# yangjames/Calico

Measured on AMD Instinct MI355X. Metric: LM iterations/sec on the 4-cam+IMU ~100k-observation problem, higher is better.
Workload: dtype f64

## Files before the change

### calico_amd/_capi.py

```python
import ctypes as C
import os

import numpy as np

OK, INVALID_ARGUMENT, FAILED_PRECONDITION, UNIMPLEMENTED, INTERNAL = 0, 3, 9, 12, 13
MANIFOLD_EUCLIDEAN, MANIFOLD_EIGEN_QUATERNION = 0, 1
SENSOR_CAMERA, SENSOR_GYROSCOPE, SENSOR_ACCELEROMETER = 0, 1, 2
CONVERGENCE, NO_CONVERGENCE, FAILURE = 0, 1, 2


class SolverOptions(C.Structure):
    _fields_ = [
        ("max_num_iterations", C.c_int32),
        ("num_threads", C.c_int32),
        ("minimizer_progress_to_stdout", C.c_int32),
        ("jacobi_scaling", C.c_int32),
        ("max_num_consecutive_invalid_steps", C.c_int32),
        ("sync_every", C.c_int32),
        ("function_tolerance", C.c_double),
        ("gradient_tolerance", C.c_double),
        ("parameter_tolerance", C.c_double),
        ("initial_trust_region_radius", C.c_double),
        ("max_trust_region_radius", C.c_double),
        ("min_trust_region_radius", C.c_double),
# ... 247 lines not shown
        ids = _i32(block_ids)
        per = np.broadcast_to(np.asarray(sizes, np.int64), (ids.size,))
        for i, n in zip(ids, per):
            known = self._sizes.get(int(i))
            if known is not None and known != int(n):
                raise ValueError("block %d has %d values, not %d" % (int(i), known, int(n)))
        total = int(per.sum())
        out = np.zeros(total)
        self._check(self.api.get_param_blocks(self.h, ids.size, _ip(ids), _dp(out)))
        return out

    def set_param_block(self, block_id, values):
        v = _f64(values).ravel()
        self._check(self.api.set_param_block(self.h, block_id, _dp(v)))

    def set_param_blocks(self, block_ids, values_concat):
        ids, v = _i32(block_ids), _f64(values_concat)
        self._check(self.api.set_param_blocks(self.h, ids.size, _ip(ids), _dp(v)))

    def set_spline(self, order, knots, basis, ctrl_block_ids):
        k, b, c = _f64(knots), _f64(basis), _i32(ctrl_block_ids)
        assert c.size == k.size - order
        self._check(self.api.problem_set_spline(self.h, order, k.size, _dp(k), _dp(b), _ip(c)))

    def add_rigid_body(self, q_block, t_block):
        out = C.c_int32(-1)
        self._check(self.api.problem_add_rigid_body(self.h, q_block, t_block, C.byref(out)))
        return out.value

    def add_sensor(self, kind, model, intr, q, t, lat, grav=-1, sigma=1.0, loss=0, loss_scale=1.0):
        out = C.c_int32(-1)
        self._check(self.api.problem_add_sensor(self.h, kind, model, intr, q, t, lat, grav, float(sigma), loss,
                                                float(loss_scale), C.byref(out)))
        return out.value

    def add_camera_residuals(self, sensor, pixels, stamps, body_ids, point_blocks):
        px, st, b, p = _f64(pixels), _f64(stamps), _i32(body_ids), _i32(point_blocks)
        self._check(self.api.problem_add_camera_residuals(self.h, sensor, st.size, _dp(px), _dp(st), _ip(b), _ip(p)))

    def add_imu_residuals(self, sensor, meas, stamps):
        m, st = _f64(meas), _f64(stamps)
        self._check(self.api.problem_add_imu_residuals(self.h, sensor, st.size, _dp(m), _dp(st)))

    def solve(self, options=None):
        o = options if options is not None else self.api.default_options()
        s = Summary()
        self._check(self.api.solve(self.h, C.byref(o), C.byref(s)))
        return s

    def iterations(self, max_rows=4096):
        buf = (Iteration * max_rows)()
        n = C.c_int32(0)
        self._check(self.api.get_iterations(self.h, buf, max_rows, C.byref(n)))
        return [buf[i] for i in range(n.value)]

    def residuals(self, sensor, n, dim, check=True):
        out = np.zeros((n, dim))
        valid = np.zeros(n, dtype=np.uint8)
        st = self.api.get_residuals(self.h, sensor, _dp(out), valid.ctypes.data_as(C.POINTER(C.c_uint8)))
        if check:
            self._check(st)
        return out, valid

    def project(self, sensor, n, dim):
        out = np.zeros((n, dim))
        valid = np.zeros(n, dtype=np.uint8)
        self._check(self.api.project(self.h, sensor, _dp(out), valid.ctypes.data_as(C.POINTER(C.c_uint8))))
        return out, valid

    def set_outlier_mask(self, sensor, is_outlier=None):
        if is_outlier is None:
            self._check(self.api.problem_set_outlier_mask(self.h, sensor, None))
        else:
            m = np.ascontiguousarray(is_outlier, dtype=np.uint8)
            self._check(self.api.problem_set_outlier_mask(self.h, sensor, m.ctypes.data_as(C.POINTER(C.c_uint8))))

    def mark_outliers(self, sensor, threshold):
        n = C.c_int64(0)
        self._check(self.api.mark_outliers(self.h, sensor, float(threshold), C.byref(n)))
        return n.value

    def residual_heatmap(self, sensor, image_width, image_height, num_rows=8, num_cols=12):
        rmse = np.zeros((num_rows, num_cols))
        count = np.zeros((num_rows, num_cols), dtype=np.int64)
        self._check(self.api.residual_heatmap(self.h, sensor, int(image_width), int(image_height), int(num_rows), int(num_cols),
                                              _dp(rmse), count.ctypes.data_as(C.POINTER(C.c_int64))))
        return rmse, count

    def inlier_mask(self, sensor, n, threshold):
        mask = np.zeros(n, dtype=np.uint8)
        self._check(self.api.get_inlier_mask(self.h, sensor, float(threshold),
                                             mask.ctypes.data_as(C.POINTER(C.c_uint8))))
        return mask

    def num_effective_parameters(self):
        n = C.c_int32(0)
        self._check(self.api.num_effective_parameters(self.h, C.byref(n)))
        return n.value

    def evaluate(self, want_jtj=True):
        n = self.num_effective_parameters()
        cost = C.c_double(0)
        g = np.zeros(n)
        H = np.zeros((n, n)) if want_jtj else None
        self._check(self.api.evaluate(self.h, C.byref(cost), _dp(g), _dp(H) if want_jtj else None))
        return cost.value, g, H

    def covariance_compute(self, min_relative_pivot=None):
        o = CovarianceOptions()
        self.api.default_covariance_options(C.byref(o))
        if min_relative_pivot is not None:
            o.min_relative_pivot = float(min_relative_pivot)
        self._check(self.api.covariance_compute(self.h, C.byref(o)))
        return self.covariance_info()

    def covariance_info(self):
        dim, nu, piv = C.c_int32(0), C.c_int32(0), C.c_double(0)
        self._check(self.api.covariance_info(self.h, C.byref(dim), C.byref(nu), C.byref(piv)))
        return dim.value, nu.value, piv.value

    def covariance_dense(self):
        dim = self.covariance_info()[0]
        out = np.zeros((dim, dim))
        self._check(self.api.covariance_get_dense(self.h, _dp(out)))
        return out

    def covariance(self, blocks, tangent=False, min_relative_pivot=None):
        self.covariance_compute(min_relative_pivot)
        res = {}
        for i, a in enumerate(blocks):
            for b in blocks[i:]:
                res[(a, b)] = self.covariance_block(a, b, tangent)
        return res

    def covariance_block(self, block_a, block_b, tangent=False, sizes=None):
        if sizes is None:
            def sz(b):
                n = self._sizes[b]
                return 3 if (tangent and n == 4 and self._manifolds.get(b) == MANIFOLD_EIGEN_QUATERNION) else n
            sizes = (sz(block_a), sz(block_b))
        out = np.zeros(sizes)
        self._check(self.api.covariance_get_block(self.h, int(block_a), int(block_b), int(bool(tangent)), _dp(out)))
        return out

    def set_allreduce(self, pyfunc):
        cb = ALLREDUCE_FN(pyfunc)
        self._keep.append(cb)
        self._check(self.api.problem_set_allreduce(self.h, cb, None))

    def finalize(self):
        self._check(self.api.problem_finalize(self.h))

    def plan_info(self):
        out = np.zeros(9, np.int32)
        self._check(self.api.debug_plan_info(self.h, out.ctypes.data_as(C.POINTER(C.c_int32)), 9))
        keys = ("fuse_expand", "frames", "items", "cells", "max_frames_per_cell", "max_items_per_cell", "tree_solver", "m",
                "all_control_points_observed")
        return dict(zip(keys, (int(v) for v in out)))

    def comm_init_rccl(self, unique_id, rank, world_size):
        buf = (C.c_uint8 * 128).from_buffer_copy(bytes(unique_id))
        self._check(self.api.comm_init_rccl(self.h, buf, int(rank), int(world_size)))

    def comm_info(self):
        r, w = C.c_int32(0), C.c_int32(0)
        nl, nt = C.c_int64(0), C.c_int64(0)
        self._check(self.api.comm_info(self.h, C.byref(r), C.byref(w), C.byref(nl), C.byref(nt)))
        return r.value, w.value, nl.value, nt.value

    def set_shard(self, rank, world_size):
        self._check(self.api.problem_set_shard(self.h, int(rank), int(world_size)))

    def set_stream(self, stream_ptr):
        self._check(self.api.problem_set_stream(self.h, C.c_void_p(stream_ptr)))

    def set_phase_timing(self, mask):
        self._check(self.api.set_phase_timing(self.h, int(mask)))

    def phase_time(self, phase):
        ms = C.c_double(0)
        n = C.c_int64(0)
        self._check(self.api.get_phase_time(self.h, phase, C.byref(ms), C.byref(n)))
        return ms.value, n.value


_HIP_LIB_NAME = "libcalico_hip.so"
_hip_api = None


def hip_library_path():
    other = os.environ.get("CALICO_HIP_LIB") if os.environ.get("CALICO_DEV") == "1" else None
    return other or os.path.join(os.path.dirname(os.path.abspath(__file__)), _HIP_LIB_NAME)


def load_hip():
    global _hip_api
    if _hip_api is None:
        path = hip_library_path()
        if not os.path.exists(path):
            raise RuntimeError("%s not found: run `python -c 'import __graft_entry__ as g; g.build()'` "
                               "(the HIP library is the only backend; there is no CPU fallback)" % path)
        _hip_api = CApi(C.CDLL(path), "calico_", has_device=True)
    return _hip_api
```

### calico_amd/csrc/calico_hip.cpp

```cpp
#include <hip/hip_runtime.h>
#include <rccl/rccl.h>
#include <dlfcn.h>
#include <link.h>

#include <algorithm>
#include <chrono>
#include <cmath>
#include <cstdio>
#include <cstdlib>
#include <cstring>
#include <limits>
#include <array>
#include <atomic>
#include <map>
#include <memory>
#include <mutex>
#include <string>
#include <unordered_map>
#include <vector>

#include "../../include/calico_hip.h"
#include "calico_hip_testing.h"
#include "problem_dev.hpp"
#include "shard.hpp"

namespace cal {

void launch_eval(const EvalArgs& a, bool jac, hipStream_t stream);
void launch_eval_frames(const EvalArgs& a, hipStream_t stream);
void launch_eval_jacobian(const EvalArgs& a, hipStream_t stream);
void launch_expand_cells(const EvalArgs& a, hipStream_t stream);
void launch_residual_heatmap(const double* res, const uint8_t* valid, const uint8_t* active, const double* px, const double* py,
                             int begin, int end, int width, int height, int num_rows, int num_cols, double* rmse, long long* count,
                             hipStream_t s);
void launch_inlier_mask(const double* res, uint8_t* valid_then_mask, const uint8_t* active, int begin, int end, int dim, double threshold,
                        hipStream_t s);
void launch_mark_outliers(const double* res, const uint8_t* valid, uint8_t* active, int begin, int end, int dim,
                          double threshold, int* n_marked, hipStream_t s);
hipError_t configure_eval_kernels(size_t max_lds_bytes);

void launch_gather(double* R, const double* src, const int* out_idx_thin, const int64_t* ptr_thin, const int* idx_thin,
                   int n_thin, int n_thin8, int n_thin4, int thin_per_lane, const int* out_idx_fat, const int64_t* ptr_fat, const int* idx_fat, int n_fat,
                   const double* cost_src, int n_cost, const LmState* st, int need_flag, size_t other_stride, hipStream_t s, const ControlTail* tail = nullptr);
void launch_gather_lists(const GatherStruct& gs, int n_out, int* cnt, int* out_idx, int64_t* ptr, int* idx, int zero_slot, long long* scratch,
                         hipStream_t s);
size_t gather_fixed_entries(int n_thin, int n_thin8, int n_thin4, int thin_per_lane);
void launch_gather_pack_fixed(const int64_t* ptr, const int* idx, int n_thin, int n_thin8, int n_thin4, int thin_per_lane, int zero_slot, int* out,
                              hipStream_t s);
void launch_post_eval(const SolveArgs& a, const double* x, const BlockDev* blocks, int n_blocks, const LmOptionsDev& o,
                      IterLog* log, int log_cap, int first, int jacobi, hipStream_t s);
size_t band_cholesky_lds_bytes(const SolveArgs& a);
size_t reduced_solve_lds_bytes(const SolveArgs& a);
size_t frame_lds_doubles(int Ps, int P1e, int n1);
size_t band_backsolve_lds_bytes(const SolveArgs& a);
hipError_t configure_solve_kernels(size_t band_lds, size_t reduced_lds, size_t back_lds);
void launch_solve(const SolveArgs& a, const LmOptionsDev& o, const double* x, double* x_cand, const BlockDev* blocks,
                  int n_blocks, bool dense_in_lds, hipStream_t s, bool with_post_eval, IterLog* log, int log_cap, int jacobi);
void launch_cost_reduce(const double* item_cost, int n_items, double* R2, const LmState* st, hipStream_t s);
void launch_control(LmState* st, const LmOptionsDev& o, double* R2, double* x, const double* x_cand, int n_amb,
                    IterLog* log, int log_cap, const double* item_cost, int n_items, const double* Rbase, size_t r_stride,
                    hipStream_t s, bool commit_by_copy = false);
void launch_init_state(LmState* st, double radius, double x_norm, hipStream_t s, const double* upd_ext = nullptr, int upd_ext_n = 0);
void launch_begin_solve(LmState* st, double radius, double x_norm, const double* upd_ext, int upd_ext_n, const ResultSink& sink, double* x,
                        double* x_cand, const double* h_x, int n_amb, hipStream_t s);
void launch_publish_results(const LmState* st, const IterLog* log, int log_rows, const double* x, int n_amb, LmState* h_state,
                            IterLog* h_log, double* h_x, hipStream_t s);
void launch_seed_x(double* x, const double* h_x, int n_amb, hipStream_t s);
void launch_debug_control_replay(LmState* st, const LmOptionsDev& o, const double* rho, const int* infinite, int n, double* R2,
                                 double* radius_out, int* accepted_out, double* cost_out, IterLog* log, int log_cap, hipStream_t s);
size_t bcr_level_lds_bytes();
size_t bcr_back_lds_bytes(int q_max, int m1p);
hipError_t configure_bcr_kernels(int q_max, int m1p);
void roll_table_row(int k, int lane, unsigned* out);
hipError_t configure_dense_block_solve();
hipError_t configure_reduced_block_step();
size_t dense_block_solve_lds_bytes();
void launch_bcr_level(const SolveArgs& a, const BcrArgs& b, int node0, int n_nodes, int level, int keep0, int n_keep, const LmOptionsDev& o,
                      const double* x, const BlockDev* blocks, int n_blocks, int with_post_eval, IterLog* log, int log_cap, int jacobi,
                      hipStream_t s, int schur_ks, int* fan_word, const BcrInlineNodes& inl);
void launch_bcr_schur(const SolveArgs& a, const BcrArgs& b, int ks, const LmOptionsDev& o, hipStream_t s);
void launch_bcr_back(const SolveArgs& a, const BcrArgs& b, int node0, int n_nodes, bool top, bool extras, bool border_rows, int q_max,
                     const double* x, double* x_cand, const BlockDev* blocks, int n_blocks, const BcrTopSeps& ts, hipStream_t s);

void launch_reduced_solve(const SolveArgs& a, bool reduced_in_lds, int ks, hipStream_t s);
bool dense_back_fusable(const SolveArgs& a, int ks, int q_max, bool border_rows);
size_t dense_back_lds_bytes(int q_max, int m1p);
hipError_t configure_dense_back_bytes(size_t lds);
void launch_dense_back(const SolveArgs& a, const BcrArgs& b, int ks, int node0, int n_nodes, int q_max, const double* x, double* x_cand,
                       const BlockDev* blocks, int n_blocks, const BcrTopSeps& ts, int* word, int seq, hipStream_t s);
int reduced_schur_slices(const SolveArgs& a);
void launch_band_reduction(const SolveArgs& a, const LmOptionsDev& o, const double* x, const BlockDev* blocks, int n_blocks, hipStream_t s,
                           bool with_post_eval, IterLog* log, int log_cap, int jacobi);
int covariance_max_dim();
int covariance_ld(int n);
bool covariance_in_lds(int n);
void launch_covariance(const double* Spart, int ks, int m, int mc, const double* Cdiag, const LmState* st, double* work, double* out,
                       double* info, hipStream_t s);
hipError_t configure_covariance_kernel();

}

using namespace cal;

namespace {

constexpr size_t kMaxLds = 160 * 1024;
constexpr int kLogCap = 4096;
constexpr int kNumPhases = 7;

struct RcclApi {
  void* lib = nullptr;
  ncclResult_t (*GetUniqueId)(ncclUniqueId*) = nullptr;
  ncclResult_t (*CommInitRank)(ncclComm_t*, int, ncclUniqueId, int) = nullptr;
  ncclResult_t (*CommDestroy)(ncclComm_t) = nullptr;
  ncclResult_t (*CommCount)(const ncclComm_t, int*) = nullptr;
  ncclResult_t (*AllReduce)(const void*, void*, size_t, ncclDataType_t, ncclRedOp_t, ncclComm_t, hipStream_t) = nullptr;
  const char* (*GetErrorString)(ncclResult_t) = nullptr;
  std::string error;
  bool ok() const { return lib != nullptr; }
};
RcclApi& rccl() {
  static RcclApi api = [] {
    RcclApi a;
    std::vector<std::string> names;
    if (const char* one = std::getenv("CALICO_RCCL_LIB")) names.push_back(one);
    else {
      names = {"librccl.so.1", "librccl.so"};
      for (const char* env : {"ROCM_PATH", "ROCM_HOME"})
        if (const char* r = std::getenv(env)) { names.push_back(std::string(r) + "/lib/librccl.so.1"); names.push_back(std::string(r) + "/lib/librccl.so"); }
      names.push_back("/opt/rocm/lib/librccl.so.1"); names.push_back("/opt/rocm/lib/librccl.so");
    }
    std::string why;
    for (const std::string& n : names) {
      a.lib = dlopen(n.c_str(), RTLD_NOW | RTLD_NOLOAD);
      if (a.lib) break;
    }
    for (const std::string& n : names) {
      if (a.lib) break;
      a.lib = dlopen(n.c_str(), RTLD_NOW | RTLD_LOCAL);
      if (a.lib) break;
      const char* e = dlerror();
      if (e) why = e;
    }
    if (!a.lib) { a.error = "librccl not found: " + why; return a; }
    auto sym = [&](const char* n) { void* f = dlsym(a.lib, n); if (!f && a.error.empty()) a.error = std::string("librccl lacks ") + n; return f; };
    a.GetUniqueId = reinterpret_cast<decltype(a.GetUniqueId)>(sym("ncclGetUniqueId"));
    a.CommInitRank = reinterpret_cast<decltype(a.CommInitRank)>(sym("ncclCommInitRank"));
    a.CommDestroy = reinterpret_cast<decltype(a.CommDestroy)>(sym("ncclCommDestroy"));
    a.CommCount = reinterpret_cast<decltype(a.CommCount)>(sym("ncclCommCount"));
    a.AllReduce = reinterpret_cast<decltype(a.AllReduce)>(sym("ncclAllReduce"));
    a.GetErrorString = reinterpret_cast<decltype(a.GetErrorString)>(sym("ncclGetErrorString"));
    if (!a.error.empty()) { dlclose(a.lib); a.lib = nullptr; }
    return a;
  }();
  return api;
}

struct HBlock {
  std::vector<double> v;
  int size = 0, manifold = 0;
  bool constant = false, used = false;
  int amb_off = 0;
  int tan = -1;
  int eff = -1;
  int tangent_size() const { return manifold == CALICO_MANIFOLD_EIGEN_QUATERNION ? 3 : size; }
};
struct HBody { int q, t; };
struct HSensor {
  int kind, model, K;
  int intr, q, t, lat, grav;
  double sigma, info;
  int loss; double loss_scale;
  std::vector<double> meas, stamps;
  std::vector<int> body, point, seg;
  std::vector<int64_t> sorted_pos;
  std::vector<uint8_t> active;
  int64_t n_active = -1;
  int64_t sorted_begin = 0, sorted_end = 0;
  int dim() const { return kind == CALICO_SENSOR_CAMERA ? 2 : 3; }
  int64_t n() const { return int64_t(stamps.size()); }
};

class DeviceArena {
 public:
  static DeviceArena& get() { static DeviceArena* a = new DeviceArena; return *a; }
  hipError_t alloc(void** out, size_t bytes) {
    if (!enabled_ || bytes > kSlab) return hipMalloc(out, bytes);
    bytes = (bytes + kAlign - 1) / kAlign * kAlign;
    std::lock_guard<std::mutex> g(mu_);
    int dev = 0; (void)hipGetDevice(&dev);
    for (int pass = 0; pass < 2; ++pass) {
      for (Slab& sl : slabs_) {
        if (sl.device != dev) continue;
        for (auto it = sl.free.begin(); it != sl.free.end(); ++it) {
          if (it->second < bytes) continue;
          const size_t off = it->first, len = it->second;
          sl.free.erase(it);
          if (len > bytes) sl.free.emplace(off + bytes, len - bytes);
          *out = sl.base + off;
// ... 34 lines not shown
      if (next != sl.free.begin()) {
        auto prev = std::prev(next);
        if (prev->first + prev->second == off) { off = prev->first; len += prev->second; sl.free.erase(prev); }
      }
      sl.free.emplace(off, len);
      return;
    }
  }
  struct Batch {
    explicit Batch(int device) : prev_(batch_device()) { if (DeviceArena::get().enabled_) { sync_device(device); batch_device() = device; } }
    ~Batch() { batch_device() = prev_; }
    Batch(const Batch&) = delete;
    Batch& operator=(const Batch&) = delete;
   private:
    int prev_;
  };
  size_t trim(int keep_per_device) {
    std::vector<Slab> drop;
    {
      std::lock_guard<std::mutex> g(mu_);
      std::map<int, int> kept;
      for (size_t i = 0; i < slabs_.size();) {
        Slab& sl = slabs_[i];
        const bool idle = sl.free.size() == 1 && sl.free.begin()->first == 0 && sl.free.begin()->second == sl.size;
        if (idle && kept[sl.device]++ >= keep_per_device) { drop.push_back(std::move(sl)); slabs_.erase(slabs_.begin() + long(i)); }
        else ++i;
      }
    }
    size_t bytes = 0;
    for (Slab& sl : drop) { (void)hipFree(sl.base); bytes += sl.size; }
    return bytes;
  }
  size_t slab_bytes() { std::lock_guard<std::mutex> g(mu_); size_t b = 0; for (const Slab& sl : slabs_) b += sl.size; return b; }
 private:
  static constexpr size_t kAlign = 4096, kSlab = size_t(64) << 20;
  struct Slab { char* base = nullptr; size_t size = 0; int device = 0; std::map<size_t, size_t> free; };
  DeviceArena() { enabled_ = env_flag("CALICO_ARENA", true); }
  static int& batch_device() { static thread_local int d = -1; return d; }
  static void sync_device(int device) {
    int cur = device;
    (void)hipGetDevice(&cur);
    if (cur != device) (void)hipSetDevice(device);
    (void)hipDeviceSynchronize();
    if (cur != device) (void)hipSetDevice(cur);
  }
  std::mutex mu_;
  std::vector<Slab> slabs_;
  std::unordered_map<void*, size_t> used_;
  bool enabled_ = true;
};

template <class T> struct DevBuf {
  T* p = nullptr; size_t n = 0;
  bool owner = true;
  DevBuf() = default;
  DevBuf(const DevBuf&) = delete;
  DevBuf& operator=(const DevBuf&) = delete;
  ~DevBuf() { release(); }
  void release() { if (p && owner) DeviceArena::get().release(p); p = nullptr; n = 0; owner = true; }
  void alias(const DevBuf& o) { release(); p = o.p; n = o.n; owner = false; }
  void take(DevBuf& o) { release(); p = o.p; n = o.n; owner = o.owner; o.p = nullptr; o.n = 0; o.owner = true; }
  void swap(DevBuf& o) { std::swap(p, o.p); std::swap(n, o.n); std::swap(owner, o.owner); }
  hipError_t alloc(size_t count) {
    if (count == 0) count = 1;
    if (count == n && p && owner) return hipSuccess;
    release();
    hipError_t e = DeviceArena::get().alloc(reinterpret_cast<void**>(&p), count * sizeof(T));
    if (e == hipSuccess) n = count;
    return e;
  }
  hipError_t upload(const std::vector<T>& h, hipStream_t s) {
    hipError_t e = alloc(h.size());
    if (e != hipSuccess || h.empty()) return e;
    return hipMemcpyAsync(p, h.data(), h.size() * sizeof(T), hipMemcpyHostToDevice, s);
  }
};

struct PhaseTimer {
  std::vector<hipEvent_t> pool;
  struct Rec { int phase; hipEvent_t a, b; };
  std::vector<Rec> pending;
  size_t next = 0;
  double ms[kNumPhases] = {0, 0, 0, 0, 0, 0};
  int64_t count[kNumPhases] = {0, 0, 0, 0, 0, 0};
  double ms_working[kNumPhases] = {0, 0, 0, 0, 0, 0};
  int64_t count_working[kNumPhases] = {0, 0, 0, 0, 0, 0};
  std::vector<float> samples[kNumPhases];
  hipEvent_t get() {
    if (next == pool.size()) { hipEvent_t e; (void)hipEventCreate(&e); pool.push_back(e); }
    return pool[next++];
  }
  int mask = 0;
  int every = 1;
  int64_t seen[kNumPhases] = {0, 0, 0, 0, 0, 0};
  bool open_rec = false;
  int nested = 0;
  void begin(int phase, hipStream_t s) {
    if (open_rec) { ++nested; return; }
    open_rec = (mask >> phase) & 1;
    if (open_rec && phase != 5 && every > 1) open_rec = (seen[phase]++ % every) == 0;
    if (!open_rec) return;
    Rec r; r.phase = phase; r.a = get(); r.b = nullptr; (void)hipEventRecord(r.a, s); pending.push_back(r);
  }
  void end(hipStream_t s) { if (nested) { --nested; return; } if (!open_rec) return; Rec& r = pending.back(); r.b = get(); (void)hipEventRecord(r.b, s); open_rec = false; }
  void resolve() {
    for (const Rec& r : pending) {
      float t = 0;
      if (r.b && hipEventElapsedTime(&t, r.a, r.b) == hipSuccess) { ms[r.phase] += t; count[r.phase]++; samples[r.phase].push_back(t); }
    }
    pending.clear(); next = 0;
    for (int ph = 0; ph < kNumPhases; ++ph) {
      float mx = 0; for (float t : samples[ph]) mx = std::max(mx, t);
      ms_working[ph] = 0; count_working[ph] = 0;
      for (float t : samples[ph]) if (t >= 0.25f * mx) { ms_working[ph] += t; count_working[ph]++; }
    }
  }
  void reset() { for (int i = 0; i < kNumPhases; ++i) { ms[i] = 0; count[i] = 0; seen[i] = 0; ms_working[i] = 0; count_working[i] = 0; samples[i].clear(); } }
  ~PhaseTimer() { for (hipEvent_t e : pool) (void)hipEventDestroy(e); }
};

}

struct BcrLevel { int node0, n_nodes, keep0, n_keep, q_max; };
struct PlanHost {
  bool speculative = true;
  size_t r_size = 0;
  int sep_s = 0, sep_n = 0;
  bool use_bcr = false, bcr_all_active = false;
  int bcr_N = 0, bcr_m1p = 16, bcr_root = -1, bcr_root_pend = 0, bcr_root_par = 0, bcr_br = 0, bcr_q_max = 1, bcr_slots = 1, bcr_q0 = 1;
  std::vector<BcrLevel> bcr_levels;
  std::vector<BcrNodeDev> h_bcr_nodes;
  std::vector<int> h_bcr_keep, h_cp_block;
  int border_extra() const { return use_bcr ? bcr_br : 6 * sep_n; }
  int n_cp = 0, m = 0, n_amb = 0, n_eff = 0, n_items = 0, n_items_all = 0, lds_cols = 0, row_pad = kRowPad;
  int64_t n_obs = 0;
  size_t partial_doubles = 0, partials_alloc = 0;
  std::vector<int> eff_to_tan;
  std::vector<BlockDev> h_blocks;
  std::vector<ItemDev> h_items, h_items_all, h_jac_items;
  std::vector<FrameItemDev> h_fitems;
  std::vector<CellDev> h_cells;
  int cell_chunk = 1, cell_rec_max = 1, row_cell_chunk = 1;
  int frame_lds_doubles = 0;
  int n_fitems = 0, n_jac_items = 0;
  bool fuse_expand = false;
  int pair_wave_lds_doubles = 0;
  int n_thin = 0, n_fat = 0;
  int n_thin8 = 0, n_thin4 = 0;
  int thin_per_lane = 6;
  bool gather_fixed = false;
  bool dense_in_lds = true;
  int gather_owner_block = 0;
  bool gs_lists_on_device = false;
};
struct PlanDev {
  DevBuf<double> d_knots, d_basis, d_stamp;
  DevBuf<int> d_ctrl_off, d_point_off, d_out_thin, d_idx_thin, d_idx_fixed, d_out_fat, d_idx_fat, d_prim_tab, d_bkeep, d_cp_block, d_gs_tab;
  DevBuf<int64_t> d_ptr_thin, d_ptr_fat;
  DevBuf<uint8_t> d_cp_active;
  DevBuf<SensorDev> d_sensors;
  DevBuf<LayoutDev> d_layouts;
  DevBuf<ItemDev> d_items, d_items_all, d_jac_items;
  DevBuf<FrameItemDev> d_fitems;
  DevBuf<CellDev> d_cells;
  DevBuf<BlockDev> d_blocks;
  DevBuf<BcrNodeDev> d_bnodes;
#define PLAN_DEV_BUFS(X) X(d_knots) X(d_basis) X(d_stamp) X(d_ctrl_off) X(d_point_off) X(d_out_thin) X(d_idx_thin) X(d_idx_fixed) X(d_out_fat) X(d_idx_fat) \
  X(d_prim_tab) X(d_bkeep) X(d_cp_block) X(d_gs_tab) X(d_ptr_thin) X(d_ptr_fat) X(d_cp_active) X(d_sensors) X(d_layouts) X(d_items) X(d_items_all)     \
  X(d_jac_items) X(d_fitems) X(d_cells) X(d_blocks) X(d_bnodes)
  void take_from(PlanDev& o) {
#define X(n) n.take(o.n);
    PLAN_DEV_BUFS(X)
#undef X
  }
  void alias_from(const PlanDev& o) {
#define X(n) n.alias(o.n);
    PLAN_DEV_BUFS(X)
#undef X
  }
};
struct Workspace {
  DevBuf<unsigned long long> d_wave_log;
  DevBuf<double> d_x, d_xc, d_m0, d_m1, d_m2, d_partials, d_R, d_R2, d_Lb, d_Linv, d_Y, d_S, d_Spart, d_Swork, d_zbuf, d_y, d_dadd, d_scale, d_res;
  DevBuf<double> d_bD, d_bG, d_bF, d_bpD, d_bpF, d_bM, d_bZA, d_bZB, d_bY, d_bysol, d_bzb, d_bupd;
  DevBuf<uint8_t> d_valid, d_active;
  DevBuf<int> d_counter;
  DevBuf<int> d_handoff;
  DevBuf<LmState> d_state;
  DevBuf<IterLog> d_log;
  int handoff_seq = 0;
  LmState* h_state = nullptr;
  int* h_progress = nullptr;
  int solve_epoch = 0;
  int* d_progress = nullptr;
  double* h_xpin = nullptr;
  size_t h_xpin_n = 0;
  IterLog* h_log = nullptr;
  bool ws_ready = false;
#define WS_BUFS(X) X(d_wave_log) X(d_x) X(d_xc) X(d_m0) X(d_m1) X(d_m2) X(d_partials) X(d_R) X(d_R2) X(d_Lb) X(d_Linv) X(d_Y) X(d_S) X(d_Spart)      \
  X(d_Swork) X(d_zbuf) X(d_y) X(d_dadd) X(d_scale) X(d_res) X(d_bD) X(d_bG) X(d_bF) X(d_bpD) X(d_bpF) X(d_bM) X(d_bZA) X(d_bZB) X(d_bY) X(d_bysol) \
  X(d_bzb) X(d_bupd) X(d_valid) X(d_active) X(d_counter) X(d_handoff) X(d_state) X(d_log)
  void swap_ws(Workspace& o) {
#define X(n) n.swap(o.n);
    WS_BUFS(X)
#undef X
    std::swap(handoff_seq, o.handoff_seq); std::swap(h_state, o.h_state); std::swap(h_progress, o.h_progress);
    std::swap(solve_epoch, o.solve_epoch); std::swap(d_progress, o.d_progress); std::swap(h_xpin, o.h_xpin);
    std::swap(h_xpin_n, o.h_xpin_n); std::swap(h_log, o.h_log); std::swap(ws_ready, o.ws_ready);
  }
  void free_pinned() {
    if (h_state) (void)hipHostFree(h_state);
    if (h_progress) (void)hipHostFree(h_progress);
    if (h_xpin) (void)hipHostFree(h_xpin);
    if (h_log) (void)hipHostFree(h_log);
    h_state = nullptr; h_progress = nullptr; d_progress = nullptr; h_xpin = nullptr; h_xpin_n = 0; h_log = nullptr;
  }
  Workspace() = default;
  Workspace(const Workspace&) = delete;
  Workspace& operator=(const Workspace&) = delete;
  ~Workspace() { free_pinned(); }
};

struct PlanEntry;

struct calico_problem : PlanHost, PlanDev, Workspace {
  int device = 0;
  hipStream_t stream = nullptr;
  bool own_stream = false;
  std::string error;
  std::vector<HBlock> blocks;
  std::vector<HBody> bodies;
  std::vector<HSensor> sensors;
  int order = 0;
  std::vector<double> knots, valid_knots, basis;
  std::vector<int> ctrl;
  bool dirty = true;
  calico_allreduce_fn allreduce = nullptr;
  void* allreduce_ctx = nullptr;
  ncclComm_t comm = nullptr;
  bool has_exchange() const { return allreduce != nullptr || comm != nullptr; }
  int rank = 0, world = 1;
  std::shared_ptr<PlanEntry> plan;

  std::vector<double> h_x;
  double* h_mpin = nullptr;
  size_t h_mpin_n = 0;
  bool active_dirty = true;
  bool any_tagged = false;
  bool xc_stale = true;
  struct ResCache { bool valid = false, predict = false; std::vector<double> x, r; std::vector<uint8_t> v; } res_cache;
  std::vector<calico_iteration> iterations;
  PhaseTimer timer;
  struct Covariance {
    DevBuf<LmState> st;
    DevBuf<double> scale, dadd, y, zbuf, work, out, info;
    bool valid = false;
    int dim = 0, n_unobserved = 0;
    double min_relative_pivot = 0.0;
    std::vector<double> sigma;
    struct Blk { int off, size, manifold; std::vector<double> v; };
    std::vector<Blk> blocks;
  } cov;

  int set_error(int code, const std::string& msg) { error = msg; return code; }
  int hip_error(hipError_t e, const char* what) {
    return set_error(CALICO_INTERNAL, std::string(what) + ": " + hipGetErrorString(e));
  }
};

#define HIP_TRY(p, expr)                                    \
  do {                                                      \
    hipError_t _e = (expr);                                 \
    if (_e != hipSuccess) return (p)->hip_error(_e, #expr); \
  } while (0)

namespace {

int spline_index(const calico_problem* p, double t) {
  const std::vector<double>& vk = p->valid_knots;
  if (t == vk.back()) return int(vk.size()) - 2;
  if (!(t < vk.back())) return -1;
  const int n = int(vk.size());
  if (t < vk.front()) return -1;
  const double dt = (vk.back() - vk.front()) / double(n - 1);
  int i = dt > 0.0 ? int((t - vk.front()) / dt) : 0;
  i = std::max(0, std::min(n - 2, i));
  while (i > 0 && t < vk[size_t(i)]) --i;
  while (i + 1 < n && !(t < vk[size_t(i) + 1])) ++i;
  return i;
}
int camera_num_params(int model) {
  switch (model) { case 1: return 8; case 2: return 11; case 3: return 7; case 4: return 5; case 5: return 4; case 6: return 4;
    case 7: return 5; default: return -1; }
}
int imu_num_params(int model) { return model == 1 ? 1 : (model == 2 ? 4 : (model == 3 ? 12 : -1)); }

struct PlanSwitches {
  bool band_solver = env_is("CALICO_SOLVER", "band");
  bool speculative = env_flag("CALICO_SPECULATIVE", true);
  bool band_split = env_flag("CALICO_BAND_SPLIT", true);
  bool fuse_expand = env_flag("CALICO_FUSE_EXPAND", true);
  bool gather_struct = env_flag("CALICO_GATHER_STRUCT", true);
  int bcr_leaf = env_int("CALICO_BCR_LEAF", 0, 1, kBcrMaxChain);
};

SolveArgs make_solve_args(calico_problem* p) {
  SolveArgs a;
  a.R = p->d_R.p; a.r_stride = p->speculative ? p->r_size : 0; a.Lb = p->d_Lb.p; a.Linv = p->d_Linv.p; a.Y = p->d_Y.p; a.S = p->d_S.p; a.Spart = p->d_Spart.p;
  a.Swork = p->d_Swork.p; a.y = p->d_y.p; a.zbuf = p->d_zbuf.p; a.dadd = p->d_dadd.p;
  a.scale = p->d_scale.p; a.cp_active = p->d_cp_active.p; a.st = p->d_state.p; a.n_cp = p->n_cp; a.k = p->order; a.mc = p->m; a.sep_s = p->sep_s; a.sep_n = p->sep_n; a.m = p->m + p->border_extra();
  static const int dbg = [] {
    const int v = env_int("CALICO_KERNEL_TIMING", 0, 0);
#ifndef CALICO_DEV_TIMING
    if (v) std::fprintf(stderr, "[calico] CALICO_KERNEL_TIMING is set, but this library was built without the kernels' development "
                                "instrumentation (rebuild with CALICO_DEV_TIMING=1 in the environment of __graft_entry__.build())\n");
#endif
    return v;
  }();
  a.debug = dbg;
  a.progress = nullptr;
  return a;
}

BcrArgs make_bcr_args(calico_problem* p) {
  BcrArgs b;
  b.D = p->d_bD.p; b.G = p->d_bG.p; b.F = p->d_bF.p; b.pendD = p->d_bpD.p; b.pendF = p->d_bpF.p; b.M = p->d_bM.p; b.ZA = p->d_bZA.p;
  b.ZB = p->d_bZB.p; b.Y = p->d_bY.p; b.ysol = p->d_bysol.p; b.zb = p->d_bzb.p; b.upd = p->d_bupd.p; b.nodes = p->d_bnodes.p; b.keep = p->d_bkeep.p;
  b.cp_block = p->d_cp_block.p; b.ctrl_off = p->d_ctrl_off.p; b.all_active = p->bcr_all_active ? 1 : 0; b.pad0 = 0; b.N = p->bcr_N; b.m1p = p->bcr_m1p; b.root = p->bcr_root; b.root_pend = p->bcr_root_pend;
  b.root_par = p->bcr_root_par; b.n_slots = p->bcr_slots;
  return b;
}

void build_bcr_plan(calico_problem* p, const PlanSwitches& sw) {
  const int N = (p->n_cp + kBcrCps - 1) / kBcrCps;
  p->bcr_N = N;
  auto levels_after = [](int n_sep) { int l = 0; while (n_sep > 1) { n_sep /= 2; ++l; } return l; };
  int q = 1;
  {
    double best = 1e300;
    for (int c = 1; c <= kBcrMaxChain; ++c) {
      const int n_sep = N > c ? N / (c + 1) : 0;
      const int L = 1 + levels_after(n_sep);
      double cost = 6.0 * L + 4.0 * (c + L - 1);
      const int per = 1 + p->bcr_m1p / 16, nodes = n_sep + 1;
      if (8 * ((nodes + 7) / 8) * per + 9 > 256) cost += 5.0;
      if (cost < best) { best = cost; q = c; }
    }
    if (sw.bcr_leaf > 0) q = sw.bcr_leaf;
  }
  p->bcr_levels.clear(); p->h_bcr_nodes.clear(); p->h_bcr_keep.clear();
  std::vector<int> alive(static_cast<size_t>(N), 0), mask(static_cast<size_t>(N), 0);
  for (int i = 0; i < N; ++i) alive[size_t(i)] = i;
  int level = 0, q_max_all = 1;
  while (!alive.empty() && (level == 0 || alive.size() > 1)) {
    const int chain = level == 0 ? q : 1;
    BcrLevel L;
    L.node0 = int(p->h_bcr_nodes.size()); L.keep0 = int(p->h_bcr_keep.size() / 2); L.q_max = 1;
    std::vector<int> kept, new_mask(size_t(N), 0);
    const size_t n = alive.size();
    size_t pos = 0;
    while (pos < n) {
      BcrNodeDev nd = {};
      nd.left = kept.empty() ? -1 : kept.back();
      nd.q = 0;
      nd.blk0 = alive[pos]; nd.pend = mask[size_t(alive[pos])];
      while (pos < n && nd.q < chain) { ++nd.q; ++pos; }
      nd.right = pos < n ? alive[pos] : -1;
      nd.slot = int(p->h_bcr_nodes.size());
      L.q_max = std::max(L.q_max, nd.q);
      if (nd.left >= 0) new_mask[size_t(nd.left)] |= 2;
      if (nd.right >= 0) new_mask[size_t(nd.right)] |= 1;
      p->h_bcr_nodes.push_back(nd);
      if (pos < n) { kept.push_back(alive[pos]); ++pos; }
    }
    for (int kb : kept)
      if (level == 0 || mask[size_t(kb)]) { p->h_bcr_keep.push_back(kb); p->h_bcr_keep.push_back(mask[size_t(kb)]); }
    L.n_nodes = int(p->h_bcr_nodes.size()) - L.node0;
    L.n_keep = int(p->h_bcr_keep.size() / 2) - L.keep0;
    q_max_all = std::max(q_max_all, L.q_max);
    p->bcr_levels.push_back(L);
    alive = kept; mask = new_mask;
    ++level;
  }
  p->bcr_root = alive.empty() ? -1 : alive[0];
  p->bcr_root_pend = alive.empty() ? 0 : mask[size_t(alive[0])];
  p->bcr_root_par = (level - 1) & 1;
  p->bcr_br = alive.empty() ? 0 : 6 * kBcrCps;
  p->bcr_q_max = q_max_all;
  p->bcr_q0 = q;
  p->bcr_slots = int(p->h_bcr_nodes.size()) + 1;
}

EvalArgs make_eval_args(calico_problem* p, const double* x, int apply_loss, bool want_res) {
  EvalArgs a;
  static const int dbg = env_int("CALICO_KERNEL_TIMING", 0, 0);
  a.debug = dbg;
  a.x = x; a.sensors = p->d_sensors.p; a.layouts = p->d_layouts.p; a.items = p->d_items.p;
  a.knots = p->d_knots.p; a.basis = p->d_basis.p; a.ctrl_off = p->d_ctrl_off.p;
  a.m0 = p->d_m0.p; a.m1 = p->d_m1.p; a.m2 = p->d_m2.p; a.stamp = p->d_stamp.p; a.point_off = p->d_point_off.p;
  a.partials = p->d_partials.p; a.item_cost = p->d_partials.p + p->partial_doubles;
  a.res_out = want_res ? p->d_res.p : nullptr; a.valid_out = want_res ? p->d_valid.p : nullptr;
  a.order = p->order; a.n_items = p->n_items; a.lds_cols = p->lds_cols; a.row_pad = p->row_pad; a.n_cells = int(p->h_cells.size()); a.cells = p->d_cells.p; a.prim_tab = p->d_prim_tab.p;
  a.cell_chunk = p->cell_chunk; a.cell_rec_max = p->cell_rec_max; a.project = 0; a.row_cell_chunk = p->row_cell_chunk; a.frame_lds_doubles = p->frame_lds_doubles; a.pad5 = 0; a.wave_log = p->d_wave_log.p; a.active = p->any_tagged ? p->d_active.p : nullptr; a.apply_loss = apply_loss;
  a.st = nullptr; a.need_flag = 0; a.cost_index_base = 0;
  a.fitems = p->d_fitems.p; a.n_fitems = p->n_fitems;
  a.hint_progress = nullptr; a.hint_seq = 0; a.hint_ftol = a.hint_ptol = 0.0;
  a.pair_mode = 0; a.wave_lds_doubles = 0;
  return a;
}

constexpr int kImuChunkItems = 21;

struct SetupTimer {
  std::chrono::steady_clock::time_point t = std::chrono::steady_clock::now();
  void section(const char* name) {
    static const bool on = env_flag("CALICO_SETUP_TIMING", false);
    if (!on) return;
    const auto now = std::chrono::steady_clock::now();
    std::fprintf(stderr, "[calico] finalize %-28s %8.3f ms\n", name, std::chrono::duration<double, std::milli>(now - t).count());
    t = now;
  }
};

int build_plan(calico_problem* p, const PlanSwitches& sw, SetupTimer& setup) {
  const int k = p->order;
  const int n_cp = int(p->ctrl.size());
  p->n_cp = n_cp;
  int off = 0;
  for (HBlock& b : p->blocks) { b.amb_off = off; off += b.size; b.used = false; b.tan = -1; b.eff = -1; }
  p->n_amb = off;
  std::vector<char> is_ctrl(p->blocks.size(), 0);
  for (int id : p->ctrl) is_ctrl[id] = 1;
  std::vector<uint8_t> cp_active(n_cp, 0);
  for (HSensor& s : p->sensors) {
    if (s.n() == 0) continue;
    p->blocks[s.intr].used = p->blocks[s.q].used = p->blocks[s.t].used = p->blocks[s.lat].used = true;
    if (s.kind == CALICO_SENSOR_ACCELEROMETER) p->blocks[s.grav].used = true;
    for (int64_t i = 0; i < s.n(); ++i) {
      for (int j = 0; j < k; ++j) cp_active[s.seg[i] + j] = 1;
      if (s.kind == CALICO_SENSOR_CAMERA) {
        p->blocks[s.point[i]].used = true;
        p->blocks[p->bodies[s.body[i]].q].used = p->blocks[p->bodies[s.body[i]].t].used = true;
      }
    }
  }
  for (int i = 0; i < n_cp; ++i) {
    HBlock& b = p->blocks[p->ctrl[i]];
    b.used = cp_active[i] != 0;
    if (b.constant && b.used) return p->set_error(CALICO_UNIMPLEMENTED, "constant control points are not supported");
    b.tan = 6 * i;
  }
  p->h_blocks.clear(); p->eff_to_tan.clear();
  int eff = 0;
  for (int i = 0; i < n_cp; ++i) {
    if (!cp_active[i]) continue;
// ... 258 lines not shown
        p->h_cells.push_back(c);
        it.rows_off = -2;
        it.partial_off = int64_t(poff);
        poff += size_t(tri_size(n1));
      } else if (hs.kind != CALICO_SENSOR_CAMERA && n1 <= 112) {
        it.partial_off = 0; it.rows_off = 0;
        if (p->h_cells.empty() || p->h_cells.back().prim_off >= 0 || p->h_cells.back().layout != it.layout ||
            p->h_cells.back().seg != it.seg) {
          CellDev c;
          c.layout = it.layout; c.seg = it.seg; c.frame_begin = int(p->h_jac_items.size()); c.frame_count = 0;
          c.partial_off = int64_t(poff); c.src_off = 0; c.n1 = n1; c.PE = hs.dim() * kImuChunkItems; c.prim_off = -1; c.pad0 = 0;
          poff += size_t(tri_size(n1));
          p->h_cells.push_back(c);
        }
        p->h_cells.back().frame_count += 1;
        p->h_cells.back().pad0 += hs.dim() * it.obs_count;
      } else {
        it.rows_off = -1;
        it.partial_off = int64_t(poff);
        poff += size_t(tri_size(n1));
      }
      p->h_jac_items.push_back(it);
    }
  }
  p->n_fitems = int(p->h_fitems.size());
  p->n_jac_items = int(p->h_jac_items.size());
  const size_t n_cost_slots = 2 * size_t(std::max(std::max(int(p->h_items.size()), int(p->h_items_all.size())), p->n_fitems + p->n_jac_items));
  const size_t comp_base = poff + n_cost_slots;
  p->cell_rec_max = 1;
  p->frame_lds_doubles = 0;
  for (FrameItemDev& f : p->h_fitems) {
    {
      const LayoutDev& L = layouts[size_t(f.layout)];
      const HSensor& hs = p->sensors[size_t(L.sensor)];
      const int P1 = 7 + (L.c_intr >= 0 ? hs.K : 0) + 3 * (L.c_q >= 0) + 3 * (L.c_t >= 0) + 3 * (L.c_bq >= 0) + 3 * (L.c_bt >= 0);
      const int Ps = 7 + (L.c_intr >= 0 ? hs.K : 0) + 3 * (L.c_bq >= 0);
      p->frame_lds_doubles = std::max(p->frame_lds_doubles, int(frame_lds_doubles(Ps, P1, L.ncols + 1)));
    }
    f.partial_off += int64_t(comp_base);
    p->cell_rec_max = std::max(p->cell_rec_max, int(frame_rec(layouts[size_t(f.layout)])));
  }
  p->cell_chunk = std::max(1, int((56 * 1024 / sizeof(double)) / size_t(p->cell_rec_max)));
  {
    int most = 1;
    for (const CellDev& c : p->h_cells) if (c.prim_off >= 0) most = std::max(most, c.frame_count);
    p->cell_chunk = std::min(p->cell_chunk, most);
  }
  std::vector<int> prim_tab;
  {
    std::vector<int> tab_off(layouts.size(), -1);
    for (CellDev& c : p->h_cells) {
      if (c.prim_off < 0) continue;
      const LayoutDev& L = layouts[size_t(c.layout)];
      const HSensor& hs = p->sensors[size_t(L.sensor)];
      int pc = 6;
      const int p_intr = pc; if (L.c_intr >= 0) pc += hs.K;
      const int p_q = pc; if (L.c_q >= 0) pc += 3;
      const int p_t = pc; if (L.c_t >= 0) pc += 3;
      const int p_bq = pc; if (L.c_bq >= 0) pc += 3;
      const int p_bt = pc; if (L.c_bt >= 0) pc += 3;
      const int p_r = pc, PT = pc + 1;
      if (tab_off[size_t(c.layout)] < 0) {
        tab_off[size_t(c.layout)] = int(prim_tab.size());
        std::vector<int> prim;
        for (int lc = 0; lc <= L.ncols; ++lc) {
          int pr;
          if (lc < 36) pr = lc % 6;
          else if (lc == L.c_lat) pr = PT;
          else if (lc == L.ncols) pr = p_r;
          else if (L.c_intr >= 0 && lc >= L.c_intr && lc < L.c_intr + hs.K) pr = p_intr + (lc - L.c_intr);
          else if (L.c_q >= 0 && lc >= L.c_q && lc < L.c_q + 3) pr = p_q + (lc - L.c_q);
          else if (L.c_t >= 0 && lc >= L.c_t && lc < L.c_t + 3) pr = p_t + (lc - L.c_t);
          else if (L.c_bq >= 0 && lc >= L.c_bq && lc < L.c_bq + 3) pr = p_bq + (lc - L.c_bq);
          else pr = p_bt + (lc - L.c_bt);
          prim.push_back(pr);
        }
        const int n1 = L.ncols + 1, PEc = PT + 1;
        for (int i = 0; i < n1; ++i)
          for (int j = i; j < n1; ++j) prim_tab.push_back(i | (j << 8) | ((prim[size_t(i)] * PEc + prim[size_t(j)]) << 16));
      }
      c.prim_off = tab_off[size_t(c.layout)]; c.pad0 = 0;
      c.n1 = L.ncols + 1; c.PE = PT + 1;
      c.src_off = c.frame_begin >= 0 ? p->h_fitems[size_t(c.frame_begin)].partial_off : 0;
    }
    for (FrameItemDev& fi : p->h_fitems) {
      const CellDev& c = p->h_cells[size_t(fi.cell)];
      fi.cell_frames = c.frame_count; fi.cell_prim_off = c.prim_off; fi.cell_partial_off = c.partial_off; fi.cell_src_off = c.src_off;
    }
  }
  for (HSensor& s : p->sensors) { s.sorted_begin = n_obs; s.sorted_end = 0; }
  for (int64_t q = 0; q < n_obs; ++q) {
    HSensor& s = p->sensors[keys[q].sensor];
    const int64_t i = keys[q].idx;
    s.sorted_pos[size_t(i)] = q;
    s.sorted_begin = std::min(s.sorted_begin, q); s.sorted_end = std::max(s.sorted_end, q + 1);
    st[q] = s.stamps[i];
    if (s.kind == CALICO_SENSOR_CAMERA) point_off[q] = p->blocks[s.point[i]].amb_off;
  }
  p->n_items = int(p->h_items.size());
  p->n_items_all = int(p->h_items_all.size());
  p->partial_doubles = poff;
  if (poff + 2 * size_t(std::max(p->n_items, p->n_fitems + p->n_jac_items)) >= size_t(0x7fffffff))
    return p->set_error(CALICO_UNIMPLEMENTED, "problem too large for 32-bit gather indices");
  {
    int jc = 4, jr = 2;
    for (const ItemDev& it : p->h_jac_items) {
      const LayoutDev& L = layouts[size_t(it.layout)];
      jc = std::max(jc, L.ncols + 1);
      jr = std::max(jr, p->sensors[size_t(L.sensor)].dim() * it.obs_count);
    }
    (void)max_cols;
    p->lds_cols = (jc + 15) & ~15;
    p->row_pad = (((jr + 3) & ~3) + 1) | 1;
  }
  if (size_t(p->lds_cols) * p->row_pad * sizeof(double) > kMaxLds)
    return p->set_error(CALICO_UNIMPLEMENTED, "too many Jacobian columns per residual block for the LDS staging area");
  size_t row_store = 0;
  {
    const size_t stride = (size_t(p->lds_cols) * p->row_pad + 1) & ~size_t(1);
    row_store = (comp_base + comp_off) & 1;
    for (size_t i = 0; i < p->h_jac_items.size(); ++i) {
      ItemDev& it = p->h_jac_items[i];
      if (it.rows_off < 0) continue;
      it.rows_off = int64_t(comp_base + comp_off + row_store);
      row_store += stride;
    }
    for (CellDev& c : p->h_cells)
      if (c.prim_off == -1) c.src_off = p->h_jac_items[size_t(c.frame_begin)].rows_off;
    p->row_cell_chunk = std::max(1, int((56 * 1024 / sizeof(double)) / std::max<size_t>(1, stride)));
    int most = 1;
    for (const CellDev& c : p->h_cells) if (c.prim_off == -1) most = std::max(most, c.frame_count);
    p->row_cell_chunk = std::min(p->row_cell_chunk, most);
  }
  setup.section("sort + work items");
  SolveArgs sa; sa.n_cp = n_cp; sa.k = k; sa.mc = m; sa.sep_s = p->sep_s; sa.sep_n = p->sep_n; sa.m = m + p->border_extra(); sa.debug = 0; sa.progress = nullptr;
  const size_t r_size = sa.r_size();
  if (r_size >= size_t(0x7fffffff)) return p->set_error(CALICO_UNIMPLEMENTED, "normal-equation buffer too large");
  struct Pair { int dst, src; };
  std::vector<Pair> pairs;
  const int n_cells = int(p->h_cells.size());
  const int n_part = n_cells + p->n_jac_items;
  bool gs_ok = sw.gather_struct && int(layouts.size()) * k <= 96 && int(layouts.size()) >= 1 && m >= 1 && n_cells > 0;
  for (int itn = n_cells; gs_ok && itn < n_part; ++itn) {
    const int64_t ro = p->h_jac_items[size_t(itn - n_cells)].rows_off;
    gs_ok = ro >= 0 || ro == -2;
  }
  const int64_t gs_n_out = int64_t(NS) * m + int64_t(n_cp) * k * 36 + NS;
  gs_ok = gs_ok && gs_n_out * 96 < int64_t(0x7fffffff);
  p->gs_lists_on_device = gs_ok;
  std::vector<int> gs_tab;
  GatherStruct gsd = {};
  if (gs_ok) {
    const int n_lay = int(layouts.size()), nsg = int(p->valid_knots.size()) - 1;
    gs_tab.assign(size_t(n_lay) * nsg + size_t(n_lay) * m + size_t(n_lay), -1);
    for (const CellDev& c : p->h_cells) gs_tab[size_t(c.layout) * nsg + size_t(c.seg)] = int(c.partial_off);
    for (int l = 0; l < n_lay; ++l) {
      const std::vector<int>& gmap = layout_gmap[size_t(l)];
      for (size_t q = 0; q < gmap.size(); ++q) gs_tab[size_t(n_lay) * nsg + size_t(l) * m + size_t(gmap[q] - NS)] = 6 * k + int(q);
      gs_tab[size_t(n_lay) * nsg + size_t(n_lay) * m + size_t(l)] = layouts[size_t(l)].ncols + 1;
    }
    gsd.n_lay = n_lay; gsd.nseg = nsg; gsd.n_cp = n_cp; gsd.k = k; gsd.m = m;
    {
      int d4 = k;
      while (d4 > 0 && (k - (d4 - 1)) * n_lay <= 24) --d4;
      gsd.d_split = d4;
    }
    gsd.off_g = sa.off_g(); gsd.off_B = sa.off_B(); gsd.off_E = sa.off_E();
  }
  pairs.reserve(gs_ok ? size_t(n_part) * 256 : poff / 2 + 4 * size_t(p->n_items));
  for (int itn = 0; itn < n_part; ++itn) {
    const bool is_cell = itn < n_cells;
    if (!is_cell && (p->h_jac_items[size_t(itn - n_cells)].rows_off >= 0 || p->h_jac_items[size_t(itn - n_cells)].rows_off == -2)) continue;
    const int it_layout = is_cell ? p->h_cells[size_t(itn)].layout : p->h_jac_items[size_t(itn - n_cells)].layout;
    const int it_seg = is_cell ? p->h_cells[size_t(itn)].seg : p->h_jac_items[size_t(itn - n_cells)].seg;
    const int64_t it_poff = is_cell ? p->h_cells[size_t(itn)].partial_off : p->h_jac_items[size_t(itn - n_cells)].partial_off;
    const LayoutDev& L = layouts[size_t(it_layout)];
    const std::vector<int>& gmap = layout_gmap[size_t(it_layout)];
    const int nc = L.ncols, n1 = nc + 1;
    auto tan_of = [&](int c) { return c < 6 * k ? 6 * (it_seg + c / 6) + c % 6 : gmap[size_t(c - 6 * k)]; };
    for (int i = gs_ok ? 6 * k : 0; i < nc; ++i) {
      const int ti = tan_of(i);
      pairs.push_back({int(sa.off_g()) + ti, int(it_poff) + tri_off(i, nc, n1)});
      for (int j = i; j < nc; ++j) {
        const int tj = tan_of(j);
        const int src = int(it_poff) + tri_off(i, j, n1);
        if (ti < NS && tj < NS) {
          const int a = ti / 6, b = tj / 6;
          pairs.push_back({int(sa.off_B()) + (a * k + (b - a)) * 36 + (ti % 6) * 6 + (tj % 6), src});
          if (a == b && ti != tj) pairs.push_back({int(sa.off_B()) + (a * k) * 36 + (tj % 6) * 6 + (ti % 6), src});
        } else if (ti < NS) {
          pairs.push_back({int(sa.off_E() + size_t(ti) * m + (tj - NS)), src});
        } else {
          const int a = ti - NS, b = tj - NS;
          pairs.push_back({int(sa.off_C() + size_t(a) * m + b), src});
          if (a != b) pairs.push_back({int(sa.off_C() + size_t(b) * m + a), src});
        }
      }
    }
  }
  std::vector<int> out_thin, idx_thin, out_fat, idx_fat;
  std::vector<int64_t> ptr_thin(1, 0), ptr_fat(1, 0);
  {
    std::vector<int64_t> start(r_size + 1, 0);
    for (const Pair& pr : pairs) ++start[size_t(pr.dst) + 1];
    for (size_t d = 0; d < r_size; ++d) start[d + 1] += start[d];
    std::vector<int> sorted_src(pairs.size());
    {
      std::vector<int64_t> fill(start.begin(), start.end() - 1);
      for (const Pair& pr : pairs) sorted_src[size_t(fill[size_t(pr.dst)]++)] = pr.src;
    }
    int thin_cap = 48;
    if (gs_ok) thin_cap = int(layouts.size()) * k <= 48 ? 48 : 96;
    else {
      size_t n_mid = 0;
      for (size_t d = 0; d < r_size; ++d) { const int64_t c = start[d + 1] - start[d]; if (c > 48 && c <= 96) ++n_mid; }
      if (n_mid > 0) thin_cap = 96;
    }
    p->thin_per_lane = thin_cap / 8;
    size_t n_thin_src = 0, n_fat_src = 0;
    for (size_t d = 0; d < r_size; ++d) {
      const int64_t c = start[d + 1] - start[d];
      if (gs_ok || c > thin_cap) n_fat_src += size_t(c); else n_thin_src += size_t(c);
    }
    idx_thin.reserve(n_thin_src); idx_fat.reserve(n_fat_src);
    for (size_t d = 0; d < r_size; ++d) {
      const int64_t q0 = start[d], q1 = start[d + 1];
      if (q1 == q0) continue;
      const bool fat = gs_ok || (q1 - q0) > thin_cap;
      std::vector<int>& out = fat ? out_fat : out_thin;
      std::vector<int>& idx = fat ? idx_fat : idx_thin;
      std::vector<int64_t>& ptr = fat ? ptr_fat : ptr_thin;
      out.push_back(int(d));
      idx.insert(idx.end(), sorted_src.begin() + q0, sorted_src.begin() + q1);
      ptr.push_back(int64_t(idx.size()));
    }
  }
  p->n_thin = int(out_thin.size()); p->n_fat = int(out_fat.size());
  p->n_thin8 = p->n_thin; p->n_thin4 = p->n_thin;
  p->gather_owner_block = 0;
  setup.section("gather lists");
  hipStream_t s = p->stream;
  std::vector<int> ctrl_off(n_cp);
  for (int i = 0; i < n_cp; ++i) ctrl_off[i] = p->blocks[p->ctrl[i]].amb_off;
  {
    auto fill = [&](auto& it) {
      it.L = layouts[size_t(it.layout)];
      it.S = sd[size_t(it.L.sensor)];
      for (int i = 0; i < 8; ++i) it.ctrl_off[i] = (i < k && it.seg + i < n_cp) ? ctrl_off[size_t(it.seg + i)] : 0;
    };
    for (ItemDev& it : p->h_items) fill(it);
    for (ItemDev& it : p->h_items_all) fill(it);
    for (ItemDev& it : p->h_jac_items) fill(it);
    for (FrameItemDev& it : p->h_fitems) fill(it);
  }
  HIP_TRY(p, p->d_knots.upload(p->knots, s)); HIP_TRY(p, p->d_basis.upload(p->basis, s));
  HIP_TRY(p, p->d_ctrl_off.upload(ctrl_off, s));
  HIP_TRY(p, p->d_stamp.upload(st, s)); HIP_TRY(p, p->d_point_off.upload(point_off, s));
  HIP_TRY(p, p->d_sensors.upload(sd, s)); HIP_TRY(p, p->d_layouts.upload(layouts, s));
  HIP_TRY(p, p->d_items.upload(p->h_items, s)); HIP_TRY(p, p->d_items_all.upload(p->h_items_all, s));
  HIP_TRY(p, p->d_jac_items.upload(p->h_jac_items, s)); HIP_TRY(p, p->d_fitems.upload(p->h_fitems, s));
  HIP_TRY(p, p->d_blocks.upload(p->h_blocks, s));
  HIP_TRY(p, p->d_cp_active.upload(cp_active, s));
  DevBuf<int> d_cnt;
  DevBuf<long long> d_scan;
  if (comp_base + comp_off + row_store + 2 >= size_t(0x7fffffff)) return p->set_error(CALICO_UNIMPLEMENTED, "problem too large for 32-bit gather indices");
  const int zero_slot = int(comp_base + comp_off + row_store);
  if (gs_ok) {
    HIP_TRY(p, p->d_gs_tab.upload(gs_tab, s));
    gsd.tab = p->d_gs_tab.p;
    const int per_out = int(layouts.size()) * k;
    HIP_TRY(p, p->d_out_thin.alloc(size_t(gs_n_out))); HIP_TRY(p, p->d_ptr_thin.alloc(size_t(gs_n_out) + 1));
    HIP_TRY(p, p->d_idx_thin.alloc(size_t(gs_n_out) * per_out)); HIP_TRY(p, d_cnt.alloc(size_t(gs_n_out)));
    HIP_TRY(p, d_scan.alloc(size_t(gs_n_out) / 1024 + 2));
    launch_gather_lists(gsd, int(gs_n_out), d_cnt.p, p->d_out_thin.p, p->d_ptr_thin.p, p->d_idx_thin.p, zero_slot, d_scan.p, s);
    p->n_thin = int(gs_n_out);
    bool one_layout = k <= 8;
    for (int tc = 0; one_layout && tc < m; ++tc) {
      int holders = 0;
      for (int l = 0; l < gsd.n_lay; ++l) holders += gs_tab[size_t(gsd.n_lay) * gsd.nseg + size_t(l) * m + size_t(tc)] >= 0 ? 1 : 0;
      one_layout = holders <= 1;
    }
    const int n_border0 = NS + n_cp * k * 36;
    p->n_thin4 = one_layout ? n_border0 : p->n_thin;
    const int d4 = gsd.d_split;
    p->n_thin8 = one_layout ? std::min(n_border0, NS + d4 * n_cp * 36) : p->n_thin;
  } else {
    HIP_TRY(p, p->d_out_thin.upload(out_thin, s)); HIP_TRY(p, p->d_idx_thin.upload(idx_thin, s));
    HIP_TRY(p, p->d_ptr_thin.upload(ptr_thin, s));
  }
  HIP_TRY(p, p->d_out_fat.upload(out_fat, s)); HIP_TRY(p, p->d_idx_fat.upload(idx_fat, s));
  HIP_TRY(p, p->d_ptr_fat.upload(ptr_fat, s));
  p->gather_fixed = p->n_thin > 0 && gs_ok;
  if (p->gather_fixed) {
    HIP_TRY(p, p->d_idx_fixed.alloc(gather_fixed_entries(p->n_thin, p->n_thin8, p->n_thin4, p->thin_per_lane) + 8));
    launch_gather_pack_fixed(p->d_ptr_thin.p, p->d_idx_thin.p, p->n_thin, p->n_thin8, p->n_thin4, p->thin_per_lane, zero_slot, p->d_idx_fixed.p, s);
  }
  HIP_TRY(p, p->d_cells.upload(p->h_cells, s)); HIP_TRY(p, p->d_prim_tab.upload(prim_tab, s));
  p->partials_alloc = comp_base + comp_off + row_store + 2;
  p->r_size = r_size;
  p->speculative = sw.speculative;
  {
    sa = make_solve_args(p);
    if (band_cholesky_lds_bytes(sa) > kMaxLds) return p->set_error(CALICO_UNIMPLEMENTED, "spline order too high for the banded factorisation window");
    p->dense_in_lds = reduced_solve_lds_bytes(sa) <= kMaxLds - 1024;
    if (band_backsolve_lds_bytes(sa) > kMaxLds) return p->set_error(CALICO_UNIMPLEMENTED, "trajectory too long for the back-substitution window");
  }
  if (p->use_bcr) {
    HIP_TRY(p, p->d_bnodes.upload(p->h_bcr_nodes, s)); HIP_TRY(p, p->d_bkeep.upload(p->h_bcr_keep, s));
    p->h_cp_block.assign(size_t(n_cp), -1);
    for (size_t bi = 0; bi < p->h_blocks.size(); ++bi)
      if (p->h_blocks[bi].tan_off < NS) p->h_cp_block[size_t(p->h_blocks[bi].tan_off / 6)] = int(bi);
    HIP_TRY(p, p->d_cp_block.upload(p->h_cp_block, s));
    if (bcr_level_lds_bytes() > kMaxLds || bcr_back_lds_bytes(p->bcr_q_max, p->bcr_m1p) > kMaxLds)
      return p->set_error(CALICO_UNIMPLEMENTED, "tree solver workspace exceeds the LDS");
  }
  HIP_TRY(p, hipStreamSynchronize(s));
  setup.section("structure uploads");
  return CALICO_OK;
}

struct PlanKey {
  uint64_t h1 = 0, h2 = 0; size_t n_blocks = 0, n_obs = 0; int device = 0;
  bool operator==(const PlanKey& o) const { return h1 == o.h1 && h2 == o.h2 && n_blocks == o.n_blocks && n_obs == o.n_obs && device == o.device; }
};
}
struct PlanEntry {
  PlanKey key;
  PlanHost host;
  PlanDev dev;
  struct BlockMeta { int amb_off, tan, eff; bool used; };
  std::vector<BlockMeta> block_meta;
  struct SensorMeta { std::vector<int64_t> sorted_pos; int64_t sorted_begin, sorted_end; };
  std::vector<SensorMeta> sensor_meta;
  std::vector<std::unique_ptr<Workspace>> pool;
  uint64_t last_use = 0;
};
namespace {
struct PlanCache {
  std::mutex mu;
  std::vector<std::shared_ptr<PlanEntry>> entries;
  uint64_t tick = 0;
  int64_t hits = 0, misses = 0;
  static constexpr size_t kMaxEntries = 8, kMaxPool = 2;
};
PlanCache& plan_cache() { static PlanCache* c = new PlanCache; return *c; }
bool plan_cache_enabled() {
  static const bool on = env_flag("CALICO_PLAN_CACHE", true);
  return on;
}
struct Hasher {
  uint64_t a = 0x9E3779B97F4A7C15ull, b = 0xC2B2AE3D27D4EB4Full;
  void word(uint64_t w) {
    a = (a ^ w) * 0xff51afd7ed558ccdull; a ^= a >> 32;
    b = (b + w) * 0xc4ceb9fe1a85ec53ull; b ^= b >> 29;
  }
  void bytes(const void* p, size_t n) {
    const unsigned char* c = static_cast<const unsigned char*>(p);
    size_t i = 0;
    if (n >= 256) {
      uint64_t l0 = 0x243F6A8885A308D3ull, l1 = 0x13198A2E03707344ull, l2 = 0xA4093822299F31D0ull, l3 = 0x082EFA98EC4E6C89ull;
      for (; i + 32 <= n; i += 32) {
        uint64_t w[4];
        std::memcpy(w, c + i, 32);
        l0 = (l0 ^ w[0]) * 0xff51afd7ed558ccdull; l0 ^= l0 >> 32;
        l1 = (l1 ^ w[1]) * 0xc4ceb9fe1a85ec53ull; l1 ^= l1 >> 29;
        l2 = (l2 ^ w[2]) * 0x9E3779B97F4A7C15ull; l2 ^= l2 >> 31;
        l3 = (l3 ^ w[3]) * 0xD6E8FEB86659FD93ull; l3 ^= l3 >> 30;
      }
      word(l0); word(l1); word(l2); word(l3);
    }
    for (; i + 8 <= n; i += 8) { uint64_t w; std::memcpy(&w, c + i, 8); word(w); }
    if (i < n) { uint64_t w = 0; std::memcpy(&w, c + i, n - i); word(w ^ (uint64_t(n - i) << 56)); }
  }
  template <class T> void vec(const std::vector<T>& v) { word(v.size()); bytes(v.data(), v.size() * sizeof(T)); }
  void dbl(double d) { uint64_t w; std::memcpy(&w, &d, 8); word(w); }
};
PlanKey structure_key(const calico_problem* p, const PlanSwitches& sw) {
  Hasher h;
  h.word(uint64_t(p->order)); h.vec(p->knots); h.vec(p->basis); h.vec(p->ctrl);
  h.word(uint64_t(p->rank)); h.word(uint64_t(p->world));
  h.word(p->blocks.size());
  for (const HBlock& b : p->blocks) h.word(uint64_t(b.size) | (uint64_t(b.manifold) << 32) | (uint64_t(b.constant) << 40));
  h.word(p->bodies.size());
  for (const HBody& b : p->bodies) h.word(uint64_t(uint32_t(b.q)) | (uint64_t(uint32_t(b.t)) << 32));
  h.word(p->sensors.size());
  size_t n_obs = 0;
  for (const HSensor& s : p->sensors) {
    h.word(uint64_t(s.kind) | (uint64_t(s.model) << 8) | (uint64_t(s.K) << 16) | (uint64_t(s.loss) << 32));
    h.word(uint64_t(uint32_t(s.intr)) | (uint64_t(uint32_t(s.q)) << 32)); h.word(uint64_t(uint32_t(s.t)) | (uint64_t(uint32_t(s.lat)) << 32));
    h.word(uint64_t(uint32_t(s.grav)));
    h.dbl(s.sigma); h.dbl(s.info); h.dbl(s.loss_scale);
    h.vec(s.stamps); h.vec(s.body); h.vec(s.point);
    n_obs += s.stamps.size();
  }
  h.word(uint64_t(sw.band_solver) | (uint64_t(sw.speculative) << 1) | (uint64_t(sw.band_split) << 2) | (uint64_t(sw.fuse_expand) << 3) |
         (uint64_t(sw.gather_struct) << 4) | (uint64_t(sw.bcr_leaf) << 8));
  PlanKey k; k.h1 = h.a; k.h2 = h.b; k.n_blocks = p->blocks.size(); k.n_obs = n_obs; k.device = p->device;
  return k;
}

void adopt_plan(calico_problem* p, const std::shared_ptr<PlanEntry>& e) {
  static_cast<PlanHost&>(*p) = e->host;
  static_cast<PlanDev&>(*p).alias_from(e->dev);
  for (size_t i = 0; i < p->blocks.size(); ++i) {
    const PlanEntry::BlockMeta& bm = e->block_meta[i];
    p->blocks[i].amb_off = bm.amb_off; p->blocks[i].tan = bm.tan; p->blocks[i].eff = bm.eff; p->blocks[i].used = bm.used;
  }
  for (size_t i = 0; i < p->sensors.size(); ++i) {
    p->sensors[i].sorted_pos = e->sensor_meta[i].sorted_pos;
    p->sensors[i].sorted_begin = e->sensor_meta[i].sorted_begin; p->sensors[i].sorted_end = e->sensor_meta[i].sorted_end;
  }
  p->plan = e;
}

int prepare_workspace(calico_problem* p) {
  hipStream_t s = p->stream;
  if (p->plan) {
    std::unique_ptr<Workspace> w;
    {
      std::lock_guard<std::mutex> lock(plan_cache().mu);
      if (!p->plan->pool.empty()) { w = std::move(p->plan->pool.back()); p->plan->pool.pop_back(); }
    }
    if (w) { static_cast<Workspace&>(*p).swap_ws(*w); p->active_dirty = true; p->xc_stale = true; return CALICO_OK; }
  }
  const int n_cp = p->n_cp, m = p->m, k = p->order, NS = 6 * n_cp;
  const int64_t n_obs = p->n_obs;
  const size_t r_size = p->r_size;
  HIP_TRY(p, p->d_x.alloc(size_t(p->n_amb))); HIP_TRY(p, p->d_xc.alloc(size_t(p->n_amb)));
  HIP_TRY(p, p->d_m0.alloc(size_t(n_obs))); HIP_TRY(p, p->d_m1.alloc(size_t(n_obs))); HIP_TRY(p, p->d_m2.alloc(size_t(n_obs)));
  HIP_TRY(p, p->d_partials.alloc(p->partials_alloc));
  HIP_TRY(p, hipMemsetAsync(p->d_partials.p + (p->partials_alloc - 2), 0, 2 * sizeof(double), s));
  if (env_int("CALICO_KERNEL_TIMING", 0, 0) >= 3) HIP_TRY(p, p->d_wave_log.alloc(2 * size_t(p->n_jac_items + p->n_fitems) + 8));
  HIP_TRY(p, p->d_R.alloc(2 * r_size)); HIP_TRY(p, hipMemsetAsync(p->d_R.p, 0, 2 * r_size * sizeof(double), s));
  HIP_TRY(p, p->d_R2.alloc(2));
  const int NT = 6 * n_cp + m;
  const int mw = m + p->border_extra();
  HIP_TRY(p, p->d_Lb.alloc(size_t(NS) * 6 * k)); HIP_TRY(p, p->d_Linv.alloc(size_t(n_cp) * 36));
  HIP_TRY(p, p->d_Y.alloc(size_t(NS) * (mw + 1)));
  HIP_TRY(p, p->d_S.alloc(size_t(mw + 1) * (mw + 1)));
  HIP_TRY(p, p->d_y.alloc(size_t(NT) + p->border_extra() + 64)); HIP_TRY(p, p->d_zbuf.alloc(size_t(NS) + 64)); HIP_TRY(p, p->d_dadd.alloc(NT)); HIP_TRY(p, p->d_scale.alloc(2 * size_t(NT)));
  HIP_TRY(p, p->d_res.alloc(size_t(n_obs) * 3)); HIP_TRY(p, p->d_valid.alloc(size_t(n_obs)));
  HIP_TRY(p, p->d_active.alloc(size_t(n_obs))); HIP_TRY(p, p->d_counter.alloc(1));
  p->active_dirty = true; p->xc_stale = true;
  HIP_TRY(p, p->d_state.alloc(1)); HIP_TRY(p, p->d_log.alloc(kLogCap));
  if (!p->h_state) {
    HIP_TRY(p, hipHostMalloc(reinterpret_cast<void**>(&p->h_state), sizeof(LmState), hipHostMallocMapped | hipHostMallocCoherent));
    std::memset(p->h_state, 0, sizeof(LmState));
  }
  if (!p->h_log) HIP_TRY(p, hipHostMalloc(reinterpret_cast<void**>(&p->h_log), size_t(kLogCap) * sizeof(IterLog), hipHostMallocMapped | hipHostMallocCoherent));
  if (p->h_xpin_n < size_t(p->n_amb)) {
    if (p->h_xpin) (void)hipHostFree(p->h_xpin);
    p->h_xpin = nullptr; p->h_xpin_n = 0;
    HIP_TRY(p, hipHostMalloc(reinterpret_cast<void**>(&p->h_xpin), std::max<size_t>(1, size_t(p->n_amb)) * sizeof(double), hipHostMallocMapped | hipHostMallocCoherent));
    p->h_xpin_n = size_t(p->n_amb);
  }
  if (!p->h_progress) {
    HIP_TRY(p, hipHostMalloc(reinterpret_cast<void**>(&p->h_progress), 64, hipHostMallocMapped | hipHostMallocCoherent));
    HIP_TRY(p, hipHostGetDevicePointer(reinterpret_cast<void**>(&p->d_progress), p->h_progress, 0));
    std::memset(p->h_progress, 0, 64);
  }
  const SolveArgs sa = make_solve_args(p);
  const size_t reduced_lds = reduced_solve_lds_bytes(sa);
  HIP_TRY(p, p->d_Spart.alloc(size_t(mw + 1 <= 128 ? 8 : 4) * size_t(mw + 1) * (mw + 1) + 64));
  HIP_TRY(p, p->d_Swork.alloc(std::max<size_t>(reduced_lds / sizeof(double) + 8, size_t(mw + 1) * 16 * 13 + 8)));
  if (p->use_bcr) {
    const size_t N = size_t(p->bcr_N), bb = size_t(kBcrBP) * kBcrBP, fb = size_t(kBcrBP) * p->bcr_m1p;
    HIP_TRY(p, p->d_bD.alloc(N * bb)); HIP_TRY(p, p->d_bG.alloc(2 * N * bb)); HIP_TRY(p, p->d_bF.alloc(N * fb));
    HIP_TRY(p, p->d_bpD.alloc(4 * N * bb)); HIP_TRY(p, p->d_bpF.alloc(4 * N * fb));
    HIP_TRY(p, p->d_bM.alloc(N * bb)); HIP_TRY(p, p->d_bZA.alloc(N * bb)); HIP_TRY(p, p->d_bZB.alloc(N * bb));
    HIP_TRY(p, p->d_bY.alloc(N * fb)); HIP_TRY(p, p->d_bysol.alloc(N * kBcrBP)); HIP_TRY(p, p->d_bzb.alloc(N * kBcrBP)); HIP_TRY(p, p->d_bupd.alloc(size_t(p->bcr_slots) * 4));
    HIP_TRY(p, hipMemsetAsync(p->d_bY.p, 0, N * fb * sizeof(double), s));
    HIP_TRY(p, hipMemsetAsync(p->d_bG.p, 0, 2 * N * bb * sizeof(double), s));
    HIP_TRY(p, hipMemsetAsync(p->d_bpD.p, 0, 4 * N * bb * sizeof(double), s)); HIP_TRY(p, hipMemsetAsync(p->d_bpF.p, 0, 4 * N * fb * sizeof(double), s));
    HIP_TRY(p, hipMemsetAsync(p->d_bupd.p, 0, size_t(p->bcr_slots) * 4 * sizeof(double), s));
    HIP_TRY(p, p->d_handoff.alloc(8)); HIP_TRY(p, hipMemsetAsync(p->d_handoff.p, 0, 8 * sizeof(int), s));
    p->handoff_seq = 0;
  }
  p->ws_ready = true;
  return CALICO_OK;
}

struct PinnedPool {
  std::mutex mu;
  std::vector<std::pair<double*, size_t>> idle;
  double* acquire(size_t n, size_t* cap) {
    {
      std::lock_guard<std::mutex> lock(mu);
      for (size_t i = 0; i < idle.size(); ++i)
        if (idle[i].second >= n) { double* q = idle[i].first; *cap = idle[i].second; idle.erase(idle.begin() + long(i)); return q; }
    }
    double* q = nullptr;
    const size_t c = n + n / 4;
    if (hipHostMalloc(reinterpret_cast<void**>(&q), c * sizeof(double), hipHostMallocDefault) != hipSuccess) return nullptr;
    *cap = c;
    return q;
  }
  void release(double* q, size_t cap) {
    if (!q) return;
    std::lock_guard<std::mutex> lock(mu);
    if (idle.size() < 2) { idle.emplace_back(q, cap); return; }
    size_t small = 0;
    for (size_t i = 1; i < idle.size(); ++i) if (idle[i].second < idle[small].second) small = i;
    if (idle[small].second < cap) { (void)hipHostFree(idle[small].first); idle[small] = {q, cap}; }
    else (void)hipHostFree(q);
  }
};
PinnedPool& pinned_pool() { static PinnedPool* pp = new PinnedPool(); return *pp; }

int upload_values(calico_problem* p) {
  hipStream_t s = p->stream;
  const size_t n = size_t(std::max<int64_t>(p->n_obs, 1));
  if (p->h_mpin && p->h_mpin_n < 3 * n) { pinned_pool().release(p->h_mpin, p->h_mpin_n); p->h_mpin = nullptr; p->h_mpin_n = 0; }
  if (!p->h_mpin) {
    p->h_mpin = pinned_pool().acquire(3 * n, &p->h_mpin_n);
    if (!p->h_mpin) return p->set_error(CALICO_INTERNAL, "hipHostMalloc (measurement staging) failed");
  }
  double* m0 = p->h_mpin; double* m1 = m0 + n; double* m2 = m1 + n;
  for (const HSensor& sn : p->sensors) {
    const int dim = sn.dim();
    const int64_t ns = sn.n();
    const double* me = sn.meas.data();
    const int64_t* sp = sn.sorted_pos.data();
    if (dim == 2) for (int64_t i = 0; i < ns; ++i) { const size_t q = size_t(sp[i]); m0[q] = me[2 * i]; m1[q] = me[2 * i + 1]; m2[q] = 0.0; }
    else for (int64_t i = 0; i < ns; ++i) { const size_t q = size_t(sp[i]); m0[q] = me[3 * i]; m1[q] = me[3 * i + 1]; m2[q] = me[3 * i + 2]; }
  }
  if (p->n_obs > 0) {
    HIP_TRY(p, hipMemcpyAsync(p->d_m0.p, m0, size_t(p->n_obs) * sizeof(double), hipMemcpyHostToDevice, s));
    HIP_TRY(p, hipMemcpyAsync(p->d_m1.p, m1, size_t(p->n_obs) * sizeof(double), hipMemcpyHostToDevice, s));
    HIP_TRY(p, hipMemcpyAsync(p->d_m2.p, m2, size_t(p->n_obs) * sizeof(double), hipMemcpyHostToDevice, s));
  }
  p->h_x.assign(size_t(p->n_amb), 0.0);
  for (const HBlock& b : p->blocks) std::copy(b.v.begin(), b.v.end(), p->h_x.begin() + b.amb_off);
  if (p->n_amb > 0) {
    HIP_TRY(p, hipMemcpyAsync(p->d_x.p, p->h_x.data(), p->h_x.size() * sizeof(double), hipMemcpyHostToDevice, s));
    HIP_TRY(p, hipMemcpyAsync(p->d_xc.p, p->h_x.data(), p->h_x.size() * sizeof(double), hipMemcpyHostToDevice, s));
  }
  return CALICO_OK;
}

int configure_kernels(calico_problem* p) {
  const SolveArgs sa = make_solve_args(p);
  const size_t reduced_lds = reduced_solve_lds_bytes(sa);
  const bool db_fits = p->use_bcr && std::max(dense_block_solve_lds_bytes(), bcr_back_lds_bytes(std::min(p->bcr_q_max, 4), p->bcr_m1p)) + 1024 <= kMaxLds;
  const std::array<size_t, 8> want = {size_t(p->lds_cols) * p->row_pad * sizeof(double), band_cholesky_lds_bytes(sa),
                                      p->dense_in_lds ? reduced_lds : 0, band_backsolve_lds_bytes(sa), size_t(p->use_bcr ? 1 : 0),
                                      size_t(p->use_bcr ? p->bcr_q_max : 0), size_t(p->use_bcr ? p->bcr_m1p : 0),
                                      db_fits ? dense_back_lds_bytes(std::min(p->bcr_q_max, 4), p->bcr_m1p) : 0};
  static std::mutex mu;
  static std::map<int, std::array<size_t, 8>> allowed;
// ... 7 lines not shown
  HIP_TRY(p, configure_dense_block_solve());
  HIP_TRY(p, configure_reduced_block_step());
  if (nw[4]) HIP_TRY(p, configure_bcr_kernels(int(nw[5]), int(nw[6])));
  if (nw[7]) HIP_TRY(p, configure_dense_back_bytes(nw[7]));
  cur = nw;
  return CALICO_OK;
}

int finalize(calico_problem* p) {
  if (!p->dirty) return CALICO_OK;
  p->res_cache.valid = false;
  p->cov.valid = false;
  if (p->order <= 0) return p->set_error(CALICO_FAILED_PRECONDITION, "spline not set");
  if (p->order > 8) return p->set_error(CALICO_UNIMPLEMENTED, "spline order > 8 is not supported by the HIP kernels");
  HIP_TRY(p, hipSetDevice(p->device));
  const PlanSwitches sw{};
  SetupTimer setup;
  const bool use_cache = plan_cache_enabled();
  PlanKey key;
  std::shared_ptr<PlanEntry> hit;
  if (use_cache) {
    key = structure_key(p, sw);
    PlanCache& c = plan_cache();
    std::lock_guard<std::mutex> lock(c.mu);
    for (const std::shared_ptr<PlanEntry>& e : c.entries) if (e->key == key) { hit = e; break; }
    if (hit) { hit->last_use = ++c.tick; ++c.hits; } else ++c.misses;
  }
  setup.section("structure key + look-up");
  if (hit && p->plan == hit && p->ws_ready) {
  } else {
    if (p->plan && p->ws_ready) {
      HIP_TRY(p, hipStreamSynchronize(p->stream));
      auto w = std::make_unique<Workspace>();
      w->swap_ws(static_cast<Workspace&>(*p));
      std::lock_guard<std::mutex> lock(plan_cache().mu);
      if (p->plan->pool.size() < PlanCache::kMaxPool) p->plan->pool.push_back(std::move(w));
    }
    p->plan.reset();
    p->ws_ready = false;
    if (hit) adopt_plan(p, hit);
    else {
      const int rc = build_plan(p, sw, setup);
      if (rc != CALICO_OK) return rc;
      if (use_cache) {
        auto e = std::make_shared<PlanEntry>();
        e->key = key;
        e->host = static_cast<const PlanHost&>(*p);
        e->block_meta.resize(p->blocks.size());
        for (size_t i = 0; i < p->blocks.size(); ++i) e->block_meta[i] = {p->blocks[i].amb_off, p->blocks[i].tan, p->blocks[i].eff, p->blocks[i].used};
        e->sensor_meta.resize(p->sensors.size());
        for (size_t i = 0; i < p->sensors.size(); ++i)
          e->sensor_meta[i] = {p->sensors[i].sorted_pos, p->sensors[i].sorted_begin, p->sensors[i].sorted_end};
        e->dev.take_from(static_cast<PlanDev&>(*p));
        static_cast<PlanDev&>(*p).alias_from(e->dev);
        p->plan = e;
        PlanCache& c = plan_cache();
        std::shared_ptr<PlanEntry> evicted;
        {
          std::lock_guard<std::mutex> lock(c.mu);
          e->last_use = ++c.tick;
          if (c.entries.size() >= PlanCache::kMaxEntries) {
            size_t old = 0;
            for (size_t i = 1; i < c.entries.size(); ++i) if (c.entries[i]->last_use < c.entries[old]->last_use) old = i;
            evicted = std::move(c.entries[old]);
            c.entries.erase(c.entries.begin() + long(old));
          }
          c.entries.push_back(e);
        }
        if (evicted && evicted.use_count() == 1) {
          DeviceArena::Batch batch(evicted->key.device);
          evicted.reset();
        }
      }
    }
    setup.section(hit ? "plan adopted" : "plan cached");
    const int rc = prepare_workspace(p);
    if (rc != CALICO_OK) return rc;
    setup.section("workspace");
  }
  int rc = upload_values(p);
  if (rc != CALICO_OK) return rc;
  rc = configure_kernels(p);
  if (rc != CALICO_OK) return rc;
  HIP_TRY(p, hipStreamSynchronize(p->stream));
  pinned_pool().release(p->h_mpin, p->h_mpin_n); p->h_mpin = nullptr; p->h_mpin_n = 0;
  setup.section("values + kernel attributes");
  p->dirty = false;
  return CALICO_OK;
}

int upload_x(calico_problem* p, bool seed = true) {
  if (p->active_dirty) {
    std::vector<uint8_t> act(size_t(std::max<int64_t>(p->n_obs, 1)), 1);
    bool tagged = false;
    for (const HSensor& s : p->sensors)
      for (int64_t i = 0; i < s.n(); ++i) { act[size_t(s.sorted_pos[size_t(i)])] = s.active[size_t(i)]; tagged = tagged || !s.active[size_t(i)]; }
    p->any_tagged = tagged;
    HIP_TRY(p, hipMemcpyAsync(p->d_active.p, act.data(), size_t(p->n_obs), hipMemcpyHostToDevice, p->stream));
    HIP_TRY(p, hipStreamSynchronize(p->stream));
    p->active_dirty = false;
  }
  for (const HBlock& b : p->blocks) std::copy(b.v.begin(), b.v.end(), p->h_x.begin() + b.amb_off);
  std::copy(p->h_x.begin(), p->h_x.end(), p->h_xpin);
  if (!seed) return CALICO_OK;
  launch_seed_x(p->d_x.p, p->h_xpin, int(p->h_x.size()), p->stream);
  if (p->xc_stale) {
    HIP_TRY(p, hipMemcpyAsync(p->d_xc.p, p->h_xpin, p->h_x.size() * sizeof(double), hipMemcpyHostToDevice, p->stream));
    p->xc_stale = false;
  }
  return CALICO_OK;
}

int do_allreduce(calico_problem* p, double* buf, int64_t n) {
  if (p->comm) {
    const ncclResult_t r = rccl().AllReduce(buf, buf, size_t(n), ncclDouble, ncclSum, p->comm, p->stream);
    if (r != ncclSuccess) return p->set_error(CALICO_INTERNAL, std::string("ncclAllReduce: ") + rccl().GetErrorString(r));
    return CALICO_OK;
  }
  if (!p->allreduce) return CALICO_OK;
  const int st = p->allreduce(p->allreduce_ctx, buf, n, p->stream);
  if (st != 0) return p->set_error(CALICO_INTERNAL, "all-reduce callback failed");
  return CALICO_OK;
}

static bool end_hint_available(const calico_problem* p) { return p->order == 6 && p->n_fitems > 0; }
int enqueue_jacobian_eval(calico_problem* p, const LmState* st, int need_flag, const double* x_at = nullptr, bool spec = false,
                          const ControlTail* tail = nullptr, bool end_hint = false) {
  p->timer.begin(0, p->stream);
  EvalArgs ea = make_eval_args(p, x_at ? x_at : p->d_x.p, 1, false);
  ea.st = st; ea.need_flag = need_flag;
  if (end_hint && tail && st && end_hint_available(p)) {
    ea.hint_progress = tail->progress; ea.hint_seq = tail->seq;
    ea.hint_ftol = tail->o.function_tolerance; ea.hint_ptol = tail->o.parameter_tolerance;
  }
  ea.items = p->d_jac_items.p; ea.n_items = p->n_jac_items; ea.cost_index_base = p->n_fitems;
  if (p->fuse_expand) { ea.pair_mode = 1; ea.wave_lds_doubles = p->pair_wave_lds_doubles; }
  (void)hipGetLastError();
  if (p->order == 6 && p->n_fitems > 0) {
    launch_eval_jacobian(ea, p->stream);
    HIP_TRY(p, hipGetLastError());
  } else {
    launch_eval_frames(ea, p->stream);
    HIP_TRY(p, hipGetLastError());
    launch_eval(ea, true, p->stream);
    HIP_TRY(p, hipGetLastError());
  }
  p->timer.end(p->stream);
  p->timer.begin(1, p->stream);
  double* target = p->d_R.p + ((spec && p->h_state && !p->h_state->rcur) ? p->r_size : 0);
  if (p->has_exchange() && p->world > 1) {
    HIP_TRY(p, hipMemsetAsync(target, 0, p->r_size * sizeof(double), p->stream));
  }
  if (!p->fuse_expand) launch_expand_cells(ea, p->stream);
  launch_gather(p->d_R.p, p->d_partials.p, p->d_out_thin.p, p->gather_fixed ? nullptr : p->d_ptr_thin.p, p->gather_fixed ? p->d_idx_fixed.p : p->d_idx_thin.p, p->n_thin, p->n_thin8, p->n_thin4, p->thin_per_lane, p->d_out_fat.p,
                p->d_ptr_fat.p, p->d_idx_fat.p, p->n_fat, p->d_partials.p + p->partial_doubles, p->n_fitems + p->n_jac_items, st, need_flag,
                spec ? p->r_size : 0, p->stream, tail);
  p->timer.end(p->stream);
  if (!p->has_exchange()) return CALICO_OK;
  return do_allreduce(p, target, int64_t(p->r_size));
}

void enqueue_linear_solve(calico_problem* p, const SolveArgs& sa, const LmOptionsDev& o, int with_post_eval, int jacobi, bool reduce_only = false) {
  hipStream_t s = p->stream;
  const int n_blocks = int(p->h_blocks.size());
  if (reduce_only && !p->use_bcr) {
    launch_band_reduction(sa, o, p->d_x.p, p->d_blocks.p, n_blocks, s, with_post_eval == 1, p->d_log.p, kLogCap, jacobi);
    return;
  }
  if (!p->use_bcr) {
    launch_solve(sa, o, p->d_x.p, p->d_xc.p, p->d_blocks.p, n_blocks, p->dense_in_lds, s, with_post_eval == 1, p->d_log.p, kLogCap, jacobi);
    return;
  }
  const BcrArgs b = make_bcr_args(p);
  const int L = int(p->bcr_levels.size());
  const int ks = reduced_schur_slices(sa);
  const BcrLevel& last = p->bcr_levels[size_t(L - 1)];
  bool schur_rides = L >= 2 && last.n_nodes >= 1 && last.n_nodes <= 2 && p->bcr_root >= 0;
  for (int i = 0; schur_rides && i < last.n_nodes; ++i) schur_rides = p->h_bcr_nodes[size_t(last.node0 + i)].q == 1;
  int* const fan_word = p->d_handoff.p + 4;
  const bool inline_nodes = env_flag("CALICO_INLINE_NODES", true);
  for (int l = 0; l < L; ++l) {
    const BcrLevel& lv = p->bcr_levels[size_t(l)];
    BcrInlineNodes inl = {};
    if (inline_nodes) {
      if (l == 0) inl.q_regular = p->bcr_q0;
      else if (lv.n_nodes <= 4) { inl.n = lv.n_nodes; for (int i = 0; i < lv.n_nodes; ++i) inl.nd[i] = p->h_bcr_nodes[size_t(lv.node0 + i)]; }
    }
    launch_bcr_level(sa, b, lv.node0, lv.n_nodes, l, lv.keep0, lv.n_keep, o, p->d_x.p, p->d_blocks.p, n_blocks, l == 0 ? with_post_eval : 0,
                     p->d_log.p, kLogCap, jacobi, s, schur_rides && l == L - 1 ? ks : 0, schur_rides ? fan_word : nullptr, inl);
  }
  if (!schur_rides) launch_bcr_schur(sa, b, ks, o, s);
  if (reduce_only) return;
  BcrTopSeps ts = {};
  if (L >= 2) {
    const BcrLevel& tl = p->bcr_levels[size_t(L - 1)];
    bool ok = tl.n_nodes <= 2 && p->bcr_levels[size_t(L - 2)].q_max <= 4;
    for (int i = 0; ok && i < tl.n_nodes; ++i) {
      const BcrNodeDev& nd = p->h_bcr_nodes[size_t(tl.node0 + i)];
      ok = nd.q == 1 && (nd.left < 0 || nd.left == p->bcr_root) && (nd.right < 0 || nd.right == p->bcr_root);
      ts.blk[i] = nd.blk0; ts.left[i] = nd.left; ts.right[i] = nd.right;
    }
    ts.n = ok ? tl.n_nodes : 0;
  }
  const int l_first = ts.n > 0 ? L - 2 : L - 1;
  const BcrLevel& lf = p->bcr_levels[size_t(l_first)];
  const bool fused = l_first == 0 && dense_back_fusable(sa, ks, lf.q_max, l_first > 0) &&
                     std::max(dense_block_solve_lds_bytes(), bcr_back_lds_bytes(lf.q_max, p->bcr_m1p)) + 1024 <= kMaxLds;
  p->timer.begin(6, s);
  if (fused) {
    p->handoff_seq = p->handoff_seq % 0x3fffffff + 1;
    launch_dense_back(sa, b, ks, lf.node0, lf.n_nodes, lf.q_max, p->d_x.p, p->d_xc.p, p->d_blocks.p, n_blocks, ts, p->d_handoff.p, p->handoff_seq, s);
  } else {
    launch_reduced_solve(sa, p->dense_in_lds, ks, s);
  }
  p->timer.end(s);
  for (int l = L - 1; l >= 0; --l) {
    const BcrLevel& lv = p->bcr_levels[size_t(l)];
    if (ts.n > 0 && l == L - 1) continue;
    const bool first = l == L - 1 || (ts.n > 0 && l == L - 2);
    if (first && fused) continue;
    const BcrTopSeps none = {};
    launch_bcr_back(sa, b, lv.node0, lv.n_nodes, first, first, l > 0, lv.q_max, p->d_x.p, p->d_xc.p, p->d_blocks.p, n_blocks,
                    first ? ts : none, s);
  }
  static const bool check = env_flag("CALICO_CHECK_FINITE", false);
  if (check) {
    (void)hipStreamSynchronize(s);
    const hipError_t le = hipGetLastError();
    if (le != hipSuccess) std::fprintf(stderr, "[calico] launch error after the tree solve: %s\n", hipGetErrorString(le));
    auto scan = [&](const char* name, const double* d, size_t n) {
      std::vector<double> h(n);
      (void)hipMemcpy(h.data(), d, n * sizeof(double), hipMemcpyDeviceToHost);
      size_t bad = 0, first = 0;
      for (size_t i = 0; i < n; ++i) if (!std::isfinite(h[i])) { if (!bad) first = i; ++bad; }
      if (bad) std::fprintf(stderr, "[calico] %s: %zu of %zu non-finite, first at %zu\n", name, bad, n, first);
    };
    const size_t N = size_t(p->bcr_N), bb = size_t(kBcrBP) * kBcrBP, fb = size_t(kBcrBP) * p->bcr_m1p, m1 = size_t(sa.m) + 1;
    scan("R", p->d_R.p, 2 * p->r_size); scan("D", b.D, N * bb); scan("F", b.F, N * fb); scan("M", b.M, N * bb); scan("ZA", b.ZA, N * bb);
    scan("ZB", b.ZB, N * bb); scan("Y", b.Y, N * fb); scan("Spart", sa.Spart, size_t(ks) * m1 * m1); scan("y", sa.y, size_t(sa.NT()) + p->border_extra());
    scan("dadd", sa.dadd, size_t(sa.NT())); scan("scale", sa.scale, size_t(sa.NT()));
    scan("zb", b.zb, N * kBcrBP); scan("ysol", b.ysol, N * kBcrBP); scan("x", p->d_x.p, size_t(p->n_amb)); scan("x_cand", p->d_xc.p, size_t(p->n_amb));
    {
      std::vector<double> h(N * kBcrBP);
      (void)hipMemcpy(h.data(), b.ysol, h.size() * sizeof(double), hipMemcpyDeviceToHost);
      std::string okb;
      for (size_t I = 0; I < N; ++I) { bool ok = true; for (int r = 0; r < kBcrBP; ++r) ok = ok && std::isfinite(h[I * kBcrBP + r]); okb += ok ? '.' : 'X'; }
      std::fprintf(stderr, "[calico] ysol by superblock (X = non-finite): %s  root %d levels %zu\n", okb.c_str(), p->bcr_root, p->bcr_levels.size());
    }
  }
}

int read_state(calico_problem* p) {
  HIP_TRY(p, hipMemcpyAsync(p->h_state, p->d_state.p, sizeof(LmState), hipMemcpyDeviceToHost, p->stream));
  HIP_TRY(p, hipStreamSynchronize(p->stream));
  p->timer.resolve();
  return CALICO_OK;
}

void fill_counts(calico_problem* p, calico_summary* sm) {
  int nrb = 0, nr = 0;
  for (HSensor& s : p->sensors) {
    if (s.n_active < 0) { int64_t c = 0; for (uint8_t a : s.active) c += a ? 1 : 0; s.n_active = c; }
    const int64_t na = s.n_active;
    nrb += int(na); nr += int(na) * s.dim();
  }
  sm->num_residual_blocks = nrb; sm->num_residuals = nr;
  sm->num_residual_blocks_reduced = nrb; sm->num_residuals_reduced = nr;
  sm->num_parameter_blocks = int(p->blocks.size());
  int np = 0, ne = 0, npr = 0;
  for (const HBlock& b : p->blocks) { np += b.size; ne += b.tangent_size(); }
  sm->num_parameters = np; sm->num_effective_parameters = ne;
  sm->num_parameter_blocks_reduced = int(p->h_blocks.size());
  for (const BlockDev& b : p->h_blocks) npr += b.size;
  sm->num_parameters_reduced = npr;
  sm->num_effective_parameters_reduced = p->n_eff;
}

const char* reason_message(int reason) {
  switch (reason) {
    case 1: return "Maximum number of iterations reached.";
    case 2: return "Gradient tolerance reached.";
    case 3: return "Minimum trust region radius reached.";
    case 4: return "Parameter tolerance reached.";
    case 5: return "Function tolerance reached.";
    case 10: return "Initial residual and Jacobian evaluation failed.";
    case 11: return "Residual and Jacobian evaluation failed.";
    case 12: return "Number of consecutive invalid steps more than Solver::Options::max_num_consecutive_invalid_steps.";
    default: return "";
  }
}

}

namespace {
struct StreamPool {
  std::mutex mu;
  std::map<int, std::vector<hipStream_t>> idle;
  static constexpr size_t kMaxIdle = 4;
};
StreamPool& stream_pool() { static StreamPool* sp = new StreamPool(); return *sp; }
}

extern "C" {

int32_t calico_problem_create(calico_problem** out, int32_t device) {
  if (!out) return CALICO_INVALID_ARGUMENT;
  *out = nullptr;
  int count = 0;
  if (hipGetDeviceCount(&count) != hipSuccess || count <= 0 || device < 0 || device >= count) return CALICO_INTERNAL;
// ... 371 lines not shown
    rc = read_state(p);
    if (rc != CALICO_OK) return rc;
  }
  const bool spec = p->speculative;
  const bool multi = p->has_exchange();
  const bool async = !multi || (spec && env_flag("CALICO_MULTIRANK_ASYNC", true));
  const int batch = async ? std::max(1, opt->sync_every) : 1;
  int batch_now = batch;
  while (!streaming && !p->h_state->terminated) {
    batch_now = batch;
    {
      const LmState& hs = *p->h_state;
      const double tol = opt->function_tolerance * hs.x_cost;
      if (batch > 1 && hs.last_cost_change > 0.0 && hs.prev_cost_change > hs.last_cost_change && tol > 0.0) {
        const double r = hs.last_cost_change / hs.prev_cost_change;
        const double left = hs.last_cost_change <= tol ? 0.0 : std::ceil(std::log(tol / hs.last_cost_change) / std::log(r));
        batch_now = int(std::max(1.0, std::min(double(batch), left + 1.0)));
      }
    }
    for (int b = 0; b < batch_now; ++b) {
      const bool ride = spec && async && b > 0;
      p->timer.begin(2, s);
      enqueue_linear_solve(p, sa, o, ride, opt->jacobi_scaling);
      p->timer.end(s);
      if (spec) {
        rc = enqueue_jacobian_eval(p, p->d_state.p, 0, p->d_xc.p, true);
        if (rc != CALICO_OK) return rc;
        p->timer.begin(4, s);
        launch_control(p->d_state.p, o, p->d_R2.p, p->d_x.p, p->d_xc.p, p->n_amb, p->d_log.p, kLogCap, nullptr, 0, p->d_R.p,
                       p->r_size, s, multi && async);
        if (!async || b == batch_now - 1)
          launch_post_eval(sa, p->d_x.p, p->d_blocks.p, n_blocks, o, p->d_log.p, kLogCap, 0, opt->jacobi_scaling, s);
        p->timer.end(s);
        if (!async) {
          rc = read_state(p);
          if (rc != CALICO_OK) return rc;
          if (p->h_state->terminated) break;
        }
        continue;
      }
      p->timer.begin(3, s);
      {
        EvalArgs ea = make_eval_args(p, p->d_xc.p, 1, false);
        ea.st = p->d_state.p;
        launch_eval(ea, false, s);
      }
      const bool fuse_cost = !p->has_exchange();
      if (!fuse_cost) launch_cost_reduce(p->d_partials.p + p->partial_doubles, p->n_items, p->d_R2.p, p->d_state.p, s);
      p->timer.end(s);
      rc = do_allreduce(p, p->d_R2.p, 2);
      if (rc != CALICO_OK) return rc;
      p->timer.begin(4, s);
      launch_control(p->d_state.p, o, p->d_R2.p, p->d_x.p, p->d_xc.p, p->n_amb, p->d_log.p, kLogCap,
                     fuse_cost ? p->d_partials.p + p->partial_doubles : nullptr, p->n_items, nullptr, 0, s);
      p->timer.end(s);
      if (!async) {
        rc = read_state(p);
        if (rc != CALICO_OK) return rc;
        if (p->h_state->terminated || !p->h_state->need_jacobian) continue;
      }
      rc = enqueue_jacobian_eval(p, p->d_state.p, async ? 1 : 0);
      if (rc != CALICO_OK) return rc;
      p->timer.begin(4, s);
      launch_post_eval(sa, p->d_x.p, p->d_blocks.p, n_blocks, o, p->d_log.p, kLogCap, 0, opt->jacobi_scaling, s);
      p->timer.end(s);
    }
    rc = read_state(p);
    if (rc != CALICO_OK) return rc;
  }
  mark(3);
  if (!streaming) launch_publish_results(p->d_state.p, p->d_log.p, log_rows, p->d_x.p, int(p->h_x.size()), p->h_state, p->h_log, p->h_xpin, s);
  if (!streaming) HIP_TRY(p, hipStreamSynchronize(s));
  sm->num_jacobian_evaluations = p->h_state->n_jac_evals;
  sm->num_cost_evaluations = p->h_state->n_cost_evals;
  const double t_solve = std::chrono::duration<double>(std::chrono::steady_clock::now() - t_loop).count();
  const LmState st = *p->h_state;
  std::copy(p->h_xpin, p->h_xpin + p->h_x.size(), p->h_x.begin());
  for (HBlock& b : p->blocks) std::copy(p->h_x.begin() + b.amb_off, p->h_x.begin() + b.amb_off + b.size, b.v.begin());
  const std::vector<IterLog> log(p->h_log, p->h_log + std::max(0, std::min(st.n_log, log_rows)));
  for (const IterLog& r : log) {
    calico_iteration it;
    it.iteration = r.iteration; it.step_is_valid = r.step_is_valid; it.step_is_successful = r.step_is_successful; it.reserved = 0;
    it.cost = r.cost; it.cost_change = r.cost_change; it.gradient_max_norm = r.gradient_max_norm; it.step_norm = r.step_norm;
    it.relative_decrease = r.relative_decrease; it.trust_region_radius = r.trust_region_radius;
    p->iterations.push_back(it);
    if (opt->minimizer_progress_to_stdout) {
      if (r.iteration == 0) std::printf("iter      cost      cost_change  |gradient|   |step|    tr_ratio  tr_radius\n");
      std::printf("%4d % 8e   % 3.2e   % 3.2e  % 3.2e  % 3.2e % 3.2e\n", r.iteration, r.cost, r.cost_change, r.gradient_max_norm,
                  r.step_norm, r.relative_decrease, r.trust_region_radius);
    }
  }
  if (p->d_wave_log.p && p->d_wave_log.n > 1) {
    std::vector<unsigned long long> wl(p->d_wave_log.n);
    HIP_TRY(p, hipMemcpy(wl.data(), p->d_wave_log.p, wl.size() * sizeof(unsigned long long), hipMemcpyDeviceToHost));
    for (size_t i = 0; i + 1 < wl.size(); i += 2)
      std::fprintf(stderr, "WAVE %zu %s t0 %llu t1 %llu\n", i / 2, int(i / 2) < ((p->n_jac_items + 1) & ~1) ? "item" : "frame", wl[i], wl[i + 1]);
  }
  sm->termination_type = st.termination_type;
  sm->num_successful_steps = st.num_successful; sm->num_unsuccessful_steps = st.num_unsuccessful;
  sm->num_iterations = st.last_logged_iteration;
  sm->initial_cost = st.initial_cost;
  sm->final_cost = st.termination_type == CALICO_FAILURE ? 0.0 : std::min(st.initial_cost, st.min_cost);
  std::snprintf(sm->message, sizeof(sm->message), "%s", reason_message(st.termination_reason));
  sm->solve_time_in_seconds = t_solve;
  sm->total_time_in_seconds = std::chrono::duration<double>(std::chrono::steady_clock::now() - t_start).count();
  if (solve_timing) {
    mark(4);
    std::fprintf(stderr, "solve host us: since last return %.1f | prep %.1f | begin launch %.1f | first evaluation enqueued %.1f | loop %.1f | results %.1f"
                 " | iterations: device %d, enqueued %d (ahead of the device %d, behind a finished iteration %d), reason %d\n",
                 std::chrono::duration<double, std::micro>(t_start - t_last_return).count(), t_mark[0], t_mark[1] - t_mark[0],
                 t_mark[2] - t_mark[1], t_mark[3] - t_mark[2], t_mark[4] - t_mark[3], st.iteration, dbg_enq, dbg_go, dbg_wait,
                 st.termination_reason);
    t_last_return = std::chrono::steady_clock::now();
  }
  return CALICO_OK;
}

int32_t calico_debug_lm_control_replay(int32_t device, int32_t n, const double* rho, const int32_t* infinite,
                                       const calico_solver_options* opt, double* radius_out, int32_t* accepted_out,
                                       double* cost_column_out) {
  if (n <= 0 || n > kLogCap - 2 || !rho || !infinite || !opt || !radius_out || !accepted_out || !cost_column_out)
    return CALICO_INVALID_ARGUMENT;
  if (hipSetDevice(device) != hipSuccess) return CALICO_INTERNAL;
  DevBuf<double> d_rho, d_R2, d_rad, d_cost;
  DevBuf<int> d_inf, d_acc;
  DevBuf<LmState> d_st;
  DevBuf<IterLog> d_log;
  std::vector<double> h_rho(rho, rho + n);
  std::vector<int> h_inf(infinite, infinite + n);
  if (d_rho.upload(h_rho, nullptr) != hipSuccess || d_inf.upload(h_inf, nullptr) != hipSuccess || d_R2.alloc(2) != hipSuccess ||
      d_rad.alloc(size_t(n)) != hipSuccess || d_cost.alloc(size_t(n)) != hipSuccess || d_acc.alloc(size_t(n)) != hipSuccess ||
      d_st.alloc(1) != hipSuccess || d_log.alloc(kLogCap) != hipSuccess)
    return CALICO_INTERNAL;
  LmOptionsDev o;
  o.max_num_iterations = 1 << 30; o.max_num_consecutive_invalid_steps = opt->max_num_consecutive_invalid_steps;
  o.function_tolerance = 0.0; o.gradient_tolerance = 0.0; o.parameter_tolerance = 0.0;
  o.max_radius = opt->max_trust_region_radius; o.min_radius = opt->min_trust_region_radius;
  o.min_relative_decrease = opt->min_relative_decrease; o.min_lm_diagonal = opt->min_lm_diagonal; o.max_lm_diagonal = opt->max_lm_diagonal;
  launch_init_state(d_st.p, opt->initial_trust_region_radius, 1.0, nullptr);
  launch_debug_control_replay(d_st.p, o, d_rho.p, d_inf.p, n, d_R2.p, d_rad.p, d_acc.p, d_cost.p, d_log.p, kLogCap, nullptr);
  if (hipMemcpy(radius_out, d_rad.p, size_t(n) * sizeof(double), hipMemcpyDeviceToHost) != hipSuccess ||
      hipMemcpy(accepted_out, d_acc.p, size_t(n) * sizeof(int), hipMemcpyDeviceToHost) != hipSuccess ||
      hipMemcpy(cost_column_out, d_cost.p, size_t(n) * sizeof(double), hipMemcpyDeviceToHost) != hipSuccess)
    return CALICO_INTERNAL;
  return CALICO_OK;
}

int32_t calico_debug_roll_table(int32_t spline_order, int32_t lane, uint32_t* out48) {
  if (!out48 || spline_order < 1 || spline_order > 6 || lane < 0 || lane > 63) return CALICO_INVALID_ARGUMENT;
  cal::roll_table_row(spline_order, lane, out48);
  return CALICO_OK;
}

int32_t calico_debug_plan_info(calico_problem* p, int32_t* out, int32_t n) {
  if (!p || !out || n < 0 || n > 9) return CALICO_INVALID_ARGUMENT;
  int rc = finalize(p);
  if (rc != CALICO_OK) return rc;
  int max_frames = 0, max_items = 0, run = 0, prev_layout = -1, prev_seg = -1;
  for (const CellDev& c : p->h_cells) if (c.prim_off >= 0) max_frames = std::max(max_frames, c.frame_count);
  for (const ItemDev& it : p->h_jac_items) {
    run = (it.layout == prev_layout && it.seg == prev_seg) ? run + 1 : 1;
    prev_layout = it.layout; prev_seg = it.seg;
    max_items = std::max(max_items, run);
  }
  const int v[9] = {p->fuse_expand ? 1 : 0, p->n_fitems, p->n_jac_items, int(p->h_cells.size()), max_frames, max_items,
                    p->use_bcr ? 1 : 0, p->m, p->bcr_all_active ? 1 : 0};
  for (int i = 0; i < n; ++i) out[i] = v[i];
  return CALICO_OK;
}

int32_t calico_get_iterations(calico_problem* p, calico_iteration* out, int32_t max_rows, int32_t* n_out) {
  if (!p || !out || !n_out) return CALICO_INVALID_ARGUMENT;
  const int n = std::min<int>(max_rows, int(p->iterations.size()));
  for (int i = 0; i < n; ++i) out[i] = p->iterations[size_t(i)];
  *n_out = n;
  return CALICO_OK;
}

static int32_t residuals_or_prediction(calico_problem* p, int32_t sid, double* out, uint8_t* valid, bool predict) {
  if (!p) return CALICO_INVALID_ARGUMENT;
  if (sid < 0 || sid >= int(p->sensors.size())) return p->set_error(CALICO_INVALID_ARGUMENT, "bad sensor id");
  if (p->sensors[size_t(sid)].n() == 0) return CALICO_OK;
  if (!out) return p->set_error(CALICO_INVALID_ARGUMENT, "null output buffer");
  int rc = finalize(p);
  if (rc != CALICO_OK) return rc;
  HIP_TRY(p, hipSetDevice(p->device));
  calico_problem::ResCache& rc_ = p->res_cache;
  std::vector<double> xnow(size_t(p->n_amb), 0.0);
  for (const HBlock& b : p->blocks) std::copy(b.v.begin(), b.v.end(), xnow.begin() + b.amb_off);
  if (!(rc_.valid && rc_.predict == predict && !p->active_dirty && rc_.x == xnow)) {
    rc_.valid = false;
    rc = upload_x(p);
    if (rc != CALICO_OK) return rc;
    {
      EvalArgs ea = make_eval_args(p, p->d_x.p, 0, true);
      ea.items = p->d_items_all.p; ea.n_items = p->n_items_all;
      ea.project = predict ? 1 : 0;
      launch_eval(ea, false, p->stream);
    }
    rc_.r.resize(size_t(p->n_obs) * 3);
    rc_.v.resize(size_t(p->n_obs));
    HIP_TRY(p, hipMemcpyAsync(rc_.r.data(), p->d_res.p, rc_.r.size() * sizeof(double), hipMemcpyDeviceToHost, p->stream));
    HIP_TRY(p, hipMemcpyAsync(rc_.v.data(), p->d_valid.p, rc_.v.size(), hipMemcpyDeviceToHost, p->stream));
    HIP_TRY(p, hipStreamSynchronize(p->stream));
    rc_.x.swap(xnow); rc_.predict = predict; rc_.valid = true;
  }
  const std::vector<double>& r = rc_.r;
  const std::vector<uint8_t>& v = rc_.v;
  const HSensor& s = p->sensors[sid];
  const int dim = s.dim();
  bool all = true;
  for (int64_t i = 0; i < s.n(); ++i) {
    const int64_t q = s.sorted_pos[size_t(i)];
    for (int c = 0; c < dim; ++c) out[i * dim + c] = v[size_t(q)] ? r[size_t(q) * 3 + c] : 0.0;
    if (valid) valid[i] = v[size_t(q)];
    if (!v[size_t(q)] && s.active[size_t(i)]) all = false;
  }
  if (predict) return CALICO_OK;
  return all ? CALICO_OK : p->set_error(CALICO_INTERNAL, "Failed to update residual");
}

int32_t calico_get_residuals(calico_problem* p, int32_t sid, double* out, uint8_t* valid) {
  return residuals_or_prediction(p, sid, out, valid, false);
}

int32_t calico_project(calico_problem* p, int32_t sid, double* out, uint8_t* valid) {
  return residuals_or_prediction(p, sid, out, valid, true);
}

int32_t calico_get_inlier_mask(calico_problem* p, int32_t sid, double threshold, uint8_t* mask) {
  if (!p) return CALICO_INVALID_ARGUMENT;
  if (sid < 0 || sid >= int(p->sensors.size()) || !mask) return p->set_error(CALICO_INVALID_ARGUMENT, "bad sensor id");
  int rc = finalize(p);
  if (rc != CALICO_OK) return rc;
  HIP_TRY(p, hipSetDevice(p->device));
  rc = upload_x(p);
  if (rc != CALICO_OK) return rc;
  const HSensor& s = p->sensors[sid];
  if (s.n() == 0) return CALICO_OK;
  {
    EvalArgs ea = make_eval_args(p, p->d_x.p, 0, true);
    ea.items = p->d_items_all.p; ea.n_items = p->n_items_all;
    launch_eval(ea, false, p->stream);
  }
  launch_inlier_mask(p->d_res.p, p->d_valid.p, p->d_active.p, int(s.sorted_begin), int(s.sorted_end), s.dim(), threshold, p->stream);
  const int64_t nrange = std::max<int64_t>(0, s.sorted_end - s.sorted_begin);
  std::vector<uint8_t> m(size_t(std::max<int64_t>(nrange, 1)));
  if (nrange > 0) HIP_TRY(p, hipMemcpyAsync(m.data(), p->d_valid.p + s.sorted_begin, size_t(nrange), hipMemcpyDeviceToHost, p->stream));
  HIP_TRY(p, hipStreamSynchronize(p->stream));
  for (int64_t i = 0; i < s.n(); ++i) mask[i] = m[size_t(s.sorted_pos[size_t(i)] - s.sorted_begin)];
  return CALICO_OK;
}

int32_t calico_problem_set_outlier_mask(calico_problem* p, int32_t sid, const uint8_t* is_outlier) {
  if (!p) return CALICO_INVALID_ARGUMENT;
  if (sid < 0 || sid >= int(p->sensors.size())) return p->set_error(CALICO_INVALID_ARGUMENT, "bad sensor id");
  HSensor& s = p->sensors[sid];
  for (int64_t i = 0; i < s.n(); ++i) s.active[size_t(i)] = (is_outlier && is_outlier[i]) ? 0 : 1;
  s.n_active = -1;
  p->active_dirty = true;
  p->res_cache.valid = false;
  return CALICO_OK;
}

int32_t calico_mark_outliers(calico_problem* p, int32_t sid, double threshold, int64_t* n_marked) {
  if (!p) return CALICO_INVALID_ARGUMENT;
  if (sid < 0 || sid >= int(p->sensors.size())) return p->set_error(CALICO_INVALID_ARGUMENT, "bad sensor id");
  int rc = finalize(p);
  if (rc != CALICO_OK) return rc;
  HIP_TRY(p, hipSetDevice(p->device));
  rc = upload_x(p);
  if (rc != CALICO_OK) return rc;
  HSensor& s = p->sensors[sid];
  {
    EvalArgs ea = make_eval_args(p, p->d_x.p, 0, true);
    ea.items = p->d_items_all.p; ea.n_items = p->n_items_all;
    launch_eval(ea, false, p->stream);
  }
  HIP_TRY(p, hipMemsetAsync(p->d_counter.p, 0, sizeof(int), p->stream));
  launch_mark_outliers(p->d_res.p, p->d_valid.p, p->d_active.p, int(s.sorted_begin), int(s.sorted_end), s.dim(), threshold,
                       p->d_counter.p, p->stream);
  const int64_t nrange = std::max<int64_t>(0, s.sorted_end - s.sorted_begin);
  std::vector<uint8_t> act(size_t(std::max<int64_t>(nrange, 1)));
  int marked = 0;
  if (nrange > 0) HIP_TRY(p, hipMemcpyAsync(act.data(), p->d_active.p + s.sorted_begin, size_t(nrange), hipMemcpyDeviceToHost, p->stream));
  HIP_TRY(p, hipMemcpyAsync(&marked, p->d_counter.p, sizeof(int), hipMemcpyDeviceToHost, p->stream));
  HIP_TRY(p, hipStreamSynchronize(p->stream));
  for (int64_t i = 0; i < s.n(); ++i) s.active[size_t(i)] = act[size_t(s.sorted_pos[size_t(i)] - s.sorted_begin)];
  s.n_active = -1;
  p->res_cache.valid = false;
  if (marked > 0) p->any_tagged = true;
  if (n_marked) *n_marked = marked;
  return CALICO_OK;
}

int32_t calico_residual_heatmap(calico_problem* p, int32_t sid, int32_t image_width, int32_t image_height, int32_t num_rows,
                                int32_t num_cols, double* rmse_out, int64_t* count_out) {
  if (!p) return CALICO_INVALID_ARGUMENT;
  if (sid < 0 || sid >= int(p->sensors.size())) return p->set_error(CALICO_INVALID_ARGUMENT, "bad sensor id");
  if (p->sensors[size_t(sid)].kind != CALICO_SENSOR_CAMERA) return p->set_error(CALICO_INVALID_ARGUMENT, "not a camera");
  if (image_width <= 0 || image_height <= 0 || num_rows <= 0 || num_cols <= 0 || !rmse_out || !count_out)
    return p->set_error(CALICO_INVALID_ARGUMENT, "bad heat-map dimensions");
  int rc = finalize(p);
  if (rc != CALICO_OK) return rc;
  HIP_TRY(p, hipSetDevice(p->device));
  rc = upload_x(p);
  if (rc != CALICO_OK) return rc;
  const HSensor& s = p->sensors[size_t(sid)];
  {
    EvalArgs ea = make_eval_args(p, p->d_x.p, 0, true);
    ea.items = p->d_items_all.p; ea.n_items = p->n_items_all;
    launch_eval(ea, false, p->stream);
  }
  const size_t nb = size_t(num_rows) * num_cols;
  DevBuf<double> d_rmse; DevBuf<long long> d_cnt;
  HIP_TRY(p, d_rmse.alloc(nb)); HIP_TRY(p, d_cnt.alloc(nb));
  launch_residual_heatmap(p->d_res.p, p->d_valid.p, p->d_active.p, p->d_m0.p, p->d_m1.p, int(std::min(s.sorted_begin, s.sorted_end)),
                          int(s.sorted_end), image_width, image_height, num_rows, num_cols, d_rmse.p, d_cnt.p, p->stream);
  std::vector<long long> cnt(nb);
// ... 319 lines not shown
```

### calico_amd/csrc/calico_hip_testing.h

```cpp
#ifndef CALICO_HIP_TESTING_H_
#define CALICO_HIP_TESTING_H_

#include "../../include/calico_hip.h"

#ifdef __cplusplus
extern "C" {
#endif

int32_t calico_debug_lm_control_replay(int32_t device, int32_t n, const double* rho, const int32_t* infinite,
                                       const calico_solver_options* options, double* radius_out, int32_t* accepted_out,
                                       double* cost_column_out);

int32_t calico_debug_plan_info(calico_problem* problem, int32_t* out, int32_t n);

int32_t calico_debug_roll_table(int32_t spline_order, int32_t lane, uint32_t* out48);

#ifdef __cplusplus
}
#endif
#endif
```

### calico_amd/csrc/problem_dev.hpp

```cpp
#pragma once
#include <stddef.h>
#include <stdint.h>
#include <climits>
#include <cstdlib>
#include <cstring>

#ifdef CALICO_DEV_TIMING
#define CAL_DEV_TIMING(expr) (expr)
#else
#define CAL_DEV_TIMING(expr) false
#endif

namespace cal {

inline bool env_flag(const char* name, bool def) {
  const char* e = std::getenv(name);
  return e ? std::atoi(e) != 0 : def;
}
inline int env_int(const char* name, int def, int lo, int hi = INT_MAX) {
  const char* e = std::getenv(name);
  if (!e) return def;
  const int v = std::atoi(e);
  return v < lo ? lo : (v > hi ? hi : v);
}
inline bool env_is(const char* name, const char* value) {
  const char* e = std::getenv(name);
  return e && std::strcmp(e, value) == 0;
}

constexpr int kRowsPerItem = 128;
constexpr int kRowPad = 129;
constexpr size_t kCellsMaxLds = 158 * 1024;
constexpr size_t cells_launch_lds_bytes(size_t wave_lds_doubles) { return (2 * wave_lds_doubles + 2) * sizeof(double); }

struct SensorDev {
  int kind, model, K, loss;
  int intr_off, q_off, t_off, lat_off, grav_off;
  int pad0;
  double info, loss_scale;
};

struct LayoutDev {
  int sensor, ncols;
  int c_intr, c_q, c_t, c_lat, c_bq, c_bt, c_grav;
  int bq_off, bt_off;
  int c_pt;
};

struct ItemDev {
  int layout, seg, obs_begin, obs_count;
  int64_t partial_off;
  int64_t rows_off;
  LayoutDev L;
  SensorDev S;
  int ctrl_off[8];
};

struct FrameItemDev {
  int layout, seg, obs_begin, obs_count;
  double stamp;
  int64_t partial_off;
  LayoutDev L;
  SensorDev S;
  int ctrl_off[8];
  int cell, cell_frames, cell_prim_off, cell_pad;
  int64_t cell_partial_off, cell_src_off;
};

struct CellDev {
  int layout, seg, frame_begin, frame_count;
  int64_t partial_off;
  int64_t src_off;
  int n1, PE;
  int prim_off, pad0;
};

struct EvalArgs {
  const double* x;
  const SensorDev* sensors;
  const LayoutDev* layouts;
  const ItemDev* items;
  const double* knots;
  const double* basis;
  const int* ctrl_off;
  const double* m0; const double* m1; const double* m2; const double* stamp;
  const int* point_off;
  double* partials;
  double* item_cost;
  double* res_out;
  uint8_t* valid_out;
  int order, n_items, lds_cols, apply_loss;
  const struct LmState* st;
  int need_flag, cost_index_base;
  const FrameItemDev* fitems;
  int n_fitems, debug;
  int row_pad, n_cells;
  const CellDev* cells;
  const int* prim_tab;
  int cell_chunk, cell_rec_max;
  int project, row_cell_chunk;
  const uint8_t* active;
  int frame_lds_doubles, pad5;
  unsigned long long* wave_log;
  int* hint_progress;
  int hint_seq;
  double hint_ftol, hint_ptol;
  int pair_mode;
  int wave_lds_doubles;
};

struct IterLog;
struct LmState;
struct ResultSink {
  LmState* state; IterLog* log; double* x;
  const IterLog* src_log; const double* src_x;
  int rows, n_amb, epoch, pad;
};

struct LmState {
  double radius, decrease_factor;
  double x_cost, candidate_cost, model_cost_change;
  double x_norm, cand_norm, step_norm, gradient_max_norm, gradient_norm;
  double relative_decrease, cost_change;
  double prev_cost_change;
  double last_cost_change;
  double initial_cost, min_cost;
  int iteration;
  int need_jacobian;
  int terminated, termination_type, termination_reason;
  int step_valid, step_successful, chol_failed;
  int num_consecutive_invalid, num_successful, num_unsuccessful;
  int invalid_eval;
  int n_log, n_jac_evals, n_cost_evals;
  int rcur;
  int rfill;
  double upd_mcc[2], upd_sn[2], upd_cn[2];
  int upd_bad[2], upd_parts;
  int commit_pending;
  const double* upd_ext;
  int upd_ext_n;
  int last_logged_iteration;
  int published;
  ResultSink sink;
};

struct LmOptionsDev {
  int max_num_iterations, max_num_consecutive_invalid_steps;
  double function_tolerance, gradient_tolerance, parameter_tolerance;
  double max_radius, min_radius, min_relative_decrease, min_lm_diagonal, max_lm_diagonal;
};

struct IterLog {
  int iteration, step_is_valid, step_is_successful, reserved;
  double cost, cost_change, gradient_max_norm, step_norm, relative_decrease, trust_region_radius;
};

struct BlockDev {
  int amb_off, size, manifold, tan_off;
};

struct GatherStruct {
  const int* tab;
  int n_lay, nseg, n_cp, k, m;
  int d_split;
  unsigned long long off_g, off_B, off_E;
};

struct ControlTail {
  int enabled, n_amb, log_cap, seq;
  LmOptionsDev o;
  double* x;
  const double* x_cand;
  IterLog* log;
  const double* Rbase;
  size_t r_stride;
  int* progress;
  int owner_block;
};

#if defined(__HIPCC__)
#define CAL_HD __host__ __device__
#else
#define CAL_HD
#endif
CAL_HD inline int tri_off(int i, int j, int n1) { return i * n1 - ((i * (i - 1)) >> 1) + (j - i); }
CAL_HD inline int tri_size(int n1) { return (n1 * (n1 + 1)) >> 1; }

struct SolveArgs {
  const double* R;
  size_t r_stride;
  double* Lb;
  double* Linv;
  double* Y;
  double* S;
  double* Spart;
  double* Swork;
  double* y;
  double* zbuf;
  double* dadd;
  double* scale;
  const uint8_t* cp_active;
  LmState* st;
  int n_cp, k;
  int m;
  int mc;
  int sep_s, sep_n;
  int debug;
  int* progress;
  CAL_HD int n_s() const { return 6 * n_cp; }
  CAL_HD int W() const { return 6 * k; }
  CAL_HD int NT() const { return 6 * n_cp + mc; }
  CAL_HD size_t off_g() const { return 2; }
  CAL_HD size_t off_B() const { return 2 + size_t(NT()); }
  CAL_HD size_t off_E() const { return off_B() + size_t(n_cp) * k * 36; }
  CAL_HD size_t off_C() const { return off_E() + size_t(n_s()) * mc; }
  CAL_HD size_t r_size() const { return off_C() + size_t(mc) * mc; }
  CAL_HD bool in_sep(int tangent_row) const { return sep_n > 0 && tangent_row >= 6 * sep_s && tangent_row < 6 * (sep_s + sep_n); }
  CAL_HD int seg_begin(int seg) const { return seg == 0 ? 0 : sep_s + sep_n; }
  CAL_HD int seg_end(int seg) const { return sep_n > 0 && seg == 0 ? sep_s : n_cp; }
  CAL_HD int n_seg() const { return sep_n > 0 ? 2 : 1; }
  CAL_HD int border_tangent(int b) const { return b < mc ? n_s() + b : 6 * sep_s + (b - mc); }
  CAL_HD int y_index(int j) const { return in_sep(j) ? n_s() + mc + (j - 6 * sep_s) : j; }
};

constexpr int kBcrCps = 5;
constexpr int kBcrBP = 32;
constexpr int kBcrMaxChain = 8;
constexpr int kBcrFS = 16;

struct BcrNodeDev {
  int q;
  int left, right;
  int slot;
  int blk0;
  int pend;
};

struct BcrInlineNodes {
  int q_regular, n;
  BcrNodeDev nd[4];
};

struct BcrTopSeps {
  int n;
  int blk[2], left[2], right[2];
};

struct BcrArgs {
  double* D;
  double* G;
  double* F;
  double* pendD;
  double* pendF;
  double* M;
  double* ZA;
  double* ZB;
  double* Y;
  double* ysol;
  double* zb;
  double* upd;
  const BcrNodeDev* nodes;
  const int* keep;
  const int* cp_block;
  const int* ctrl_off;
  int all_active, pad0;
  int N, m1p;
  int root, root_pend, root_par;
  int n_slots;
};

template <class T> __device__ __forceinline__ const T* vector_ptr(const T* p) { asm volatile("" : "+v"(p)); return p; }
__device__ __forceinline__ int uniform(int v) { return __builtin_amdgcn_readfirstlane(v); }
__device__ __forceinline__ double uniform(double v) {
  return __hiloint2double(__builtin_amdgcn_readfirstlane(__double2hiint(v)), __builtin_amdgcn_readfirstlane(__double2loint(v)));
}

template <int CTRL> __device__ __forceinline__ double dpp_mov(double v) {
  int lo = __double2loint(v), hi = __double2hiint(v);
  lo = __builtin_amdgcn_update_dpp(0, lo, CTRL, 0xf, 0xf, false);
  hi = __builtin_amdgcn_update_dpp(0, hi, CTRL, 0xf, 0xf, false);
  return __hiloint2double(hi, lo);
}
__device__ __forceinline__ double row4_sum(double v) { v += dpp_mov<0xB1>(v); v += dpp_mov<0x4E>(v); return v; }
__device__ __forceinline__ double row8_sum(double v) { v = row4_sum(v); v += dpp_mov<0x141>(v); return v; }
__device__ __forceinline__ double row16_sum(double v) { v = row8_sum(v); v += dpp_mov<0x140>(v); return v; }
__device__ __forceinline__ double other_half(double v) {
  const int lo = __double2loint(v), hi = __double2hiint(v);
  const auto a = __builtin_amdgcn_permlane32_swap(lo, lo, false, false);
  const auto b = __builtin_amdgcn_permlane32_swap(hi, hi, false, false);
  const bool up = (threadIdx.x & 32) != 0;
  return __hiloint2double(up ? b[0] : b[1], up ? a[0] : a[1]);
}
__device__ __forceinline__ double other_row(double v) {
  const int lo = __double2loint(v), hi = __double2hiint(v);
  const auto a = __builtin_amdgcn_permlane16_swap(lo, lo, false, false);
  const auto b = __builtin_amdgcn_permlane16_swap(hi, hi, false, false);
  const bool odd = (threadIdx.x & 16) != 0;
  return __hiloint2double(odd ? b[0] : b[1], odd ? a[0] : a[1]);
}
__device__ __forceinline__ double wave_sum(double v) { v = row16_sum(v); v += other_half(v); v += other_row(v); return v; }

}
```

### calico_amd/csrc/solve_kernels.hip

```cpp
#include <hip/hip_runtime.h>

#include <algorithm>

#include "problem_dev.hpp"
#include "solve_dev.hpp"

namespace cal {

struct ControlStage { double u0, u1, u2, u3; double xc[4]; const double* c01; };
DEVI void control_prefetch(const LmState* st, const double* x_cand, int n_amb, LmState* s_st, ControlStage& pf);
DEVI void control_body(LmState* st, const LmOptionsDev& o, double* R2, double* x, const double* x_cand, int n_amb, IterLog* log,
                       int log_cap, const double* __restrict__ item_cost, int n_items, const double* Rbase, size_t r_stride,
                       int no_swap, int* progress, int seq, LmState* s_st, const ControlStage* staged = nullptr);
DEVI void publish(int* word, int value);
struct StructOut { int a, b, r, c, tc, rhs; size_t dst; };
DEVI StructOut struct_output(const GatherStruct& gs, int o) {
  const int NS = 6 * gs.n_cp, n_e = NS * gs.m, n_b = gs.n_cp * gs.k * 36;
  StructOut q;
  q.tc = -1; q.rhs = 0; q.c = 0;
  if (o < NS) {
    const int ti = o;
    q.a = q.b = ti / 6; q.r = ti % 6; q.rhs = 1;
    q.dst = size_t(gs.off_g) + size_t(ti);
  } else if (o < NS + n_b) {
    const int e = o - NS, ds = gs.d_split, n_a = gs.n_cp * ds * 36;
    int bd, d;
    if (e < n_a) { bd = e / 36; q.a = bd / ds; d = bd - q.a * ds; }
    else { const int dr = gs.k - ds; bd = (e - n_a) / 36; q.a = bd / dr; d = ds + (bd - q.a * dr); }
    const int w = e - 36 * (e / 36);
    q.b = q.a + d;
    q.r = w / 6; q.c = w % 6;
    q.dst = size_t(gs.off_B) + size_t(q.a * gs.k + d) * 36 + size_t(w);
  } else {
    const int e = o - NS - n_b, ti = e / gs.m;
    q.tc = e - ti * gs.m;
    q.a = q.b = ti / 6; q.r = ti % 6;
    q.dst = size_t(gs.off_E) + size_t(e);
  }
  return q;
}
template <class F>
DEVI int struct_sources(const GatherStruct& gs, const StructOut& q, F f) {
  const int n_lay = gs.n_lay, nseg = gs.nseg, m = gs.m, k = gs.k;
  const int* poff = gs.tab;
  const int* inv = gs.tab + n_lay * nseg;
  const int* n1s = inv + n_lay * m;
  if (q.b >= gs.n_cp) return 0;
  const int lo = max(0, q.b - (k - 1)), hi = min(q.a, nseg - 1);
  int n = 0;
  for (int l = 0; l < n_lay; ++l) {
    const int n1 = n1s[l];
    const int jc = q.tc >= 0 ? inv[l * m + q.tc] : 0;
    if (jc < 0) continue;
    for (int sg = lo; sg <= hi; ++sg) {
      const int po = poff[l * nseg + sg];
      if (po < 0) continue;
      int i = 6 * (q.a - sg) + q.r, j;
      if (q.tc >= 0) j = jc;
      else if (q.rhs) j = n1 - 1;
      else { j = 6 * (q.b - sg) + q.c; if (q.a == q.b && i > j) { const int t = i; i = j; j = t; } }
      f(po + tri_off(i, j, n1));
      ++n;
    }
  }
  return n;
}
__global__ __launch_bounds__(256) void gather_lists_count_kernel(GatherStruct gs, int n_out, int* __restrict__ cnt, int* __restrict__ out_idx) {
  const int o = blockIdx.x * 256 + threadIdx.x;
  if (o >= n_out) return;
  const StructOut q = struct_output(gs, o);
  const int n = struct_sources(gs, q, [](int) {});
  cnt[o] = n > 0 ? n : 1;
  out_idx[o] = int(q.dst);
}
constexpr int kScanBlock = 1024;
__global__ __launch_bounds__(256) void gather_lists_block_sums_kernel(const int* __restrict__ cnt, int n, long long* __restrict__ bsum) {
  __shared__ long long sw[4];
  const int base = blockIdx.x * kScanBlock, tid = threadIdx.x;
  long long s = 0;
#pragma unroll
  for (int u = 0; u < 4; ++u) { const int i = base + tid + 256 * u; s += i < n ? cnt[i] : 0; }
#pragma unroll
  for (int off = 32; off > 0; off >>= 1) s += __shfl_xor(s, off, 64);
  if ((tid & 63) == 0) sw[tid >> 6] = s;
  __syncthreads();
  if (tid == 0) bsum[blockIdx.x] = (sw[0] + sw[1]) + (sw[2] + sw[3]);
}
__global__ __launch_bounds__(1024) void gather_lists_scan_sums_kernel(long long* __restrict__ bsum, int nb, int64_t* __restrict__ ptr_total) {
  __shared__ long long part[1024];
  const int tid = threadIdx.x;
  long long carry = 0;
  for (int b0 = 0; b0 < nb; b0 += 1024) {
    const int b = b0 + tid;
    const long long v = b < nb ? bsum[b] : 0;
    part[tid] = v;
    __syncthreads();
    for (int off = 1; off < 1024; off <<= 1) {
      const long long w = tid >= off ? part[tid - off] : 0;
      __syncthreads();
      part[tid] += w;
      __syncthreads();
    }
    if (b < nb) bsum[b] = carry + part[tid] - v;
    const long long total = part[1023];
    __syncthreads();
    carry += total;
  }
  if (tid == 0) *ptr_total = carry;
}
__global__ __launch_bounds__(256) void gather_lists_block_scan_kernel(const int* __restrict__ cnt, int n, const long long* __restrict__ boff,
                                                                      int64_t* __restrict__ ptr) {
  __shared__ long long sw[4];
  const int base = blockIdx.x * kScanBlock, tid = threadIdx.x, lane = tid & 63, wave = tid >> 6;
  int c[4];
#pragma unroll
  for (int u = 0; u < 4; ++u) { const int i = base + 4 * tid + u; c[u] = i < n ? cnt[i] : 0; }
  const long long mine = (long long)c[0] + c[1] + c[2] + c[3];
  long long incl = mine;
#pragma unroll
  for (int off = 1; off < 64; off <<= 1) { const long long w = __shfl_up(incl, off, 64); if (lane >= off) incl += w; }
  if (lane == 63) sw[wave] = incl;
  __syncthreads();
  long long wave_off = 0;
#pragma unroll
  for (int w = 0; w < 4; ++w) wave_off += w < wave ? sw[w] : 0;
  long long run = boff[blockIdx.x] + wave_off + (incl - mine);
#pragma unroll
  for (int u = 0; u < 4; ++u) { const int i = base + 4 * tid + u; if (i < n) ptr[i] = run; run += c[u]; }
}
__global__ __launch_bounds__(256) void gather_lists_fill_kernel(GatherStruct gs, int n_out, const int64_t* __restrict__ ptr, int* __restrict__ idx,
                                                                int zero_slot) {
  const int o = blockIdx.x * 256 + threadIdx.x;
  if (o >= n_out) return;
  const StructOut q = struct_output(gs, o);
  int64_t w = ptr[o];
  const int n = struct_sources(gs, q, [&](int srci) { idx[w++] = srci; });
  if (n == 0) idx[w] = zero_slot;
}
void launch_gather_lists(const GatherStruct& gs, int n_out, int* cnt, int* out_idx, int64_t* ptr, int* idx, int zero_slot, long long* scratch,
                         hipStream_t s) {
  hipLaunchKernelGGL(gather_lists_count_kernel, dim3((n_out + 255) / 256), dim3(256), 0, s, gs, n_out, cnt, out_idx);
  const int nb = (n_out + kScanBlock - 1) / kScanBlock;
  hipLaunchKernelGGL(gather_lists_block_sums_kernel, dim3(nb), dim3(256), 0, s, cnt, n_out, scratch);
  hipLaunchKernelGGL(gather_lists_scan_sums_kernel, dim3(1), dim3(1024), 0, s, scratch, nb, ptr + n_out);
  hipLaunchKernelGGL(gather_lists_block_scan_kernel, dim3(nb), dim3(256), 0, s, cnt, n_out, scratch, ptr);
  hipLaunchKernelGGL(gather_lists_fill_kernel, dim3((n_out + 255) / 256), dim3(256), 0, s, gs, n_out, ptr, idx, zero_slot);
}

template <int U, bool FIXED>
__global__ __launch_bounds__(256) void gather_kernel(double* __restrict__ R, const double* __restrict__ src,
                                                     const int* __restrict__ out_thin, const int64_t* __restrict__ ptr_thin,
                                                     const int* __restrict__ idx_thin, int n_thin, int n_thin8, int n_thin4,
                                                     const int* __restrict__ out_fat, const int64_t* __restrict__ ptr_fat,
                                                     const int* __restrict__ idx_fat, int n_fat, int nb_fat,
                                                     const double* __restrict__ cost_src, int n_cost,
                                                     const LmState* st, int need_flag, size_t other_stride, ControlTail tail) {
  int64_t pre_q0 = 0, pre_q1 = 0;
  const int nb_thin8 = (n_thin8 + 31) / 32, nb_thin4 = (n_thin4 - n_thin8 + 63) / 64;
  int o_thin = 0;
  int cls = 8;
  int tb_map = 0;
  bool idle = false;
  if (int(blockIdx.x) - 1 >= nb_fat) {
    const int pb = int(blockIdx.x) - ((1 + nb_fat + 7) & ~7);
    const int nb_thin1 = (n_thin - n_thin4 + 255) / 256;
    const int nbp8 = (nb_thin8 + 7) & ~7, nbp4 = (nb_thin4 + 7) & ~7;
    int pbc = pb, nbc = nb_thin8, base_l = 0;
    if (pb >= nbp8 + nbp4) { pbc = pb - nbp8 - nbp4; nbc = nb_thin1; base_l = nb_thin8 + nb_thin4; }
    else if (pb >= nbp8) { pbc = pb - nbp8; nbc = nb_thin4; base_l = nb_thin8; }
    const int j = (pbc & 7) * ((nbc + 7) >> 3) + (pbc >> 3);
    idle = pb < 0 || j >= nbc;
    tb_map = base_l + (idle ? 0 : j);
  }
  {
    const int bidp = int(blockIdx.x) - 1;
    if (bidp >= nb_fat && n_thin > 0) {
      const int tb = tb_map;
      int oc;
      if (tb < nb_thin8) { o_thin = (tb * int(blockDim.x) + int(threadIdx.x)) >> 3; oc = o_thin < n_thin8 ? o_thin : n_thin8 - 1; }
      else if (tb < nb_thin8 + nb_thin4) {
        cls = 4; o_thin = n_thin8 + (((tb - nb_thin8) * int(blockDim.x) + int(threadIdx.x)) >> 2); oc = o_thin < n_thin4 ? o_thin : n_thin4 - 1;
      } else {
        cls = 1; o_thin = n_thin4 + (tb - nb_thin8 - nb_thin4) * int(blockDim.x) + int(threadIdx.x); oc = o_thin < n_thin ? o_thin : n_thin - 1;
      }
      if (!FIXED) { pre_q0 = ptr_thin[oc]; pre_q1 = ptr_thin[oc + 1]; }
    }
  }
  const size_t fbase4 = size_t(n_thin8) * (8 * U), fbase1 = fbase4 + size_t(n_thin4 - n_thin8) * 24;
  int fid[U > 8 ? U : 8];
  if (FIXED && int(blockIdx.x) - 1 >= nb_fat && n_thin > 0) {
    if (cls == 1) {
      const int oc = o_thin < n_thin ? o_thin : n_thin - 1;
#pragma unroll
      for (int u = 0; u < 8; ++u) fid[u] = idx_thin[fbase1 + size_t(oc - n_thin4) * 8 + u];
    } else if (cls == 4) {
      const int oc = o_thin < n_thin4 ? o_thin : n_thin4 - 1, sub = int(threadIdx.x) & 3;
#pragma unroll
      for (int u = 0; u < 6; ++u) fid[u] = idx_thin[fbase4 + size_t(oc - n_thin8) * 24 + sub + 4 * u];
    } else {
      const int oc = o_thin < n_thin8 ? o_thin : n_thin8 - 1, sub = int(threadIdx.x) & 7;
#pragma unroll
      for (int u = 0; u < U; ++u) fid[u] = idx_thin[size_t(oc) * (8 * U) + sub + 8 * u];
    }
  }
  if (st && (st->terminated || (need_flag && !st->need_jacobian))) {
    if (tail.enabled && tail.progress && st->terminated && blockIdx.x == 0 && threadIdx.x == 0) publish_progress(tail.progress, st, tail.seq);
    return;
  }
  if (idle) return;
  __shared__ LmState s_st;
  __shared__ double s_c01[2];
  ControlStage pf;
  const bool owner = blockIdx.x == 0;
  if (owner && tail.enabled) { control_prefetch(st, tail.x_cand, tail.n_amb, &s_st, pf); pf.c01 = s_c01; }
  if (other_stride && st && st->rfill) R += other_stride;
  if (owner) {
    const int tid = threadIdx.x;
    double c = 0.0, v = 0.0;
    for (int i = tid; i < n_cost; i += 256 * 4) {
      double cc[4], vv[4];
#pragma unroll
      for (int u = 0; u < 4; ++u) { const int j = min(i + 256 * u, n_cost - 1); cc[u] = cost_src[2 * j]; vv[u] = cost_src[2 * j + 1]; }
#pragma unroll
      for (int u = 0; u < 4; ++u) if (i + 256 * u < n_cost) { c += cc[u]; v += vv[u]; }
    }
    c = wave_sum(c); v = wave_sum(v);
    __shared__ double s_w[2][4];
    if ((tid & 63) == 0) { s_w[0][tid >> 6] = c; s_w[1][tid >> 6] = v; }
    __syncthreads();
    if (tid == 0) {
      const double ct = ((s_w[0][0] + s_w[0][1]) + s_w[0][2]) + s_w[0][3], vt = ((s_w[1][0] + s_w[1][1]) + s_w[1][2]) + s_w[1][3];
      R[0] = ct; R[1] = vt; s_c01[0] = ct; s_c01[1] = vt;
    }
    if (tail.enabled) {
      __syncthreads();
      control_body(const_cast<LmState*>(st), tail.o, nullptr, tail.x, tail.x_cand, tail.n_amb, tail.log, tail.log_cap, nullptr, 0,
                   tail.Rbase, tail.r_stride, 0, tail.progress, tail.seq, &s_st, &pf);
    }
    return;
  }
  const int bid = int(blockIdx.x) - 1;
  if (bid < nb_fat) {
    const int wave_raw = (bid * blockDim.x + threadIdx.x) >> 6;
    const int lane = threadIdx.x & 63;
    const bool live = wave_raw < n_fat;
    const int wave = live ? wave_raw : n_fat - 1;
    const int64_t q0 = ptr_fat[wave], q1 = ptr_fat[wave + 1];
    double s = 0.0;
    for (int64_t qb = q0; qb < q1; qb += 256) {
      int id[4];
#pragma unroll
      for (int u = 0; u < 4; ++u) { const int64_t q = qb + lane + 64 * u; id[u] = idx_fat[q < q1 ? q : q1 - 1]; }
      double v[4];
#pragma unroll
      for (int u = 0; u < 4; ++u) v[u] = src[id[u]];
#pragma unroll
      for (int u = 0; u < 4; ++u) s += qb + lane + 64 * u < q1 ? v[u] : 0.0;
    }
    s = wave_sum(s);
    if (live && lane == 0) R[out_fat[wave]] = s;
  } else {
    if (FIXED) {
      if (cls == 1) {
        const int o = o_thin;
        const int dst = out_thin[o < n_thin ? o : n_thin - 1];
        double v[8];
#pragma unroll
        for (int u = 0; u < 8; ++u) v[u] = src[fid[u]];
        double s = 0.0;
#pragma unroll
        for (int u = 0; u < 8; ++u) s += v[u];
        if (o < n_thin) R[dst] = s;
        return;
      }
      if (cls == 4) {
        const int o = o_thin, sub = int(threadIdx.x) & 3;
        double v[6];
#pragma unroll
        for (int u = 0; u < 6; ++u) v[u] = src[fid[u]];
        double s = 0.0;
#pragma unroll
        for (int u = 0; u < 6; ++u) s += v[u];
        s = row4_sum(s);
        if (o < n_thin4 && sub == 0) R[out_thin[o]] = s;
        return;
      }
      const int o = o_thin, sub = int(threadIdx.x) & 7;
      double v[U];
#pragma unroll
      for (int u = 0; u < U; ++u) v[u] = src[fid[u]];
      double s = 0.0, s2 = 0.0;
#pragma unroll
      for (int u = 0; u < 6; ++u) s += v[u];
#pragma unroll
      for (int u = 6; u < U; ++u) s2 += v[u];
      s += s2;
      s = row8_sum(s);
      if (o < n_thin8 && sub == 0) R[out_thin[o]] = s;
      return;
    }
    if (cls == 1) {
      const int o = o_thin;
      const int64_t q0 = pre_q0, q1 = pre_q1;
      int id[8];
#pragma unroll
      for (int u = 0; u < 8; ++u) { const int64_t q = q0 + u; id[u] = idx_thin[q < q1 ? q : q1 - 1]; }
      const int dst = out_thin[o < n_thin ? o : n_thin - 1];
      double v[8];
#pragma unroll
      for (int u = 0; u < 8; ++u) v[u] = src[id[u]];
      double s = 0.0;
#pragma unroll
      for (int u = 0; u < 8; ++u) s += q0 + u < q1 ? v[u] : 0.0;
      if (o < n_thin) R[dst] = s;
      return;
    }
    if (cls == 4) {
      const int o = o_thin, sub = int(threadIdx.x) & 3;
      const int64_t q0 = pre_q0, q1 = pre_q1;
      int id[6];
#pragma unroll
      for (int u = 0; u < 6; ++u) { const int64_t q = q0 + sub + 4 * u; id[u] = idx_thin[q < q1 ? q : q1 - 1]; }
      double v[6];
#pragma unroll
      for (int u = 0; u < 6; ++u) v[u] = src[id[u]];
      double s = 0.0;
#pragma unroll
      for (int u = 0; u < 6; ++u) s += q0 + sub + 4 * u < q1 ? v[u] : 0.0;
      s = row4_sum(s);
      if (o < n_thin4 && sub == 0) R[out_thin[o]] = s;
      return;
    }
    const int o = o_thin, sub = int(threadIdx.x) & 7;
    const bool live = o < n_thin8;
    const int64_t q0 = pre_q0, q1 = pre_q1;
    int id[6];
#pragma unroll
    for (int u = 0; u < 6; ++u) { const int64_t q = q0 + sub + 8 * u; id[u] = idx_thin[q < q1 ? q : q1 - 1]; }
    double v[6];
#pragma unroll
    for (int u = 0; u < 6; ++u) v[u] = src[id[u]];
    double s2 = 0.0;
    if constexpr (U > 6) {
      if (q1 - q0 > 48) {
        int id2[U - 6];
#pragma unroll
        for (int u = 6; u < U; ++u) { const int64_t q = q0 + sub + 8 * u; id2[u - 6] = idx_thin[q < q1 ? q : q1 - 1]; }
        double v2[U - 6];
#pragma unroll
        for (int u = 6; u < U; ++u) v2[u - 6] = src[id2[u - 6]];
#pragma unroll
        for (int u = 6; u < U; ++u) s2 += q0 + sub + 8 * u < q1 ? v2[u - 6] : 0.0;
      }
    }
    double s = 0.0;
#pragma unroll
    for (int u = 0; u < 6; ++u) s += q0 + sub + 8 * u < q1 ? v[u] : 0.0;
    s += s2;
    s = row8_sum(s);
    if (live && sub == 0) R[out_thin[o]] = s;
  }
}

__global__ __launch_bounds__(256) void post_eval_kernel(SolveArgs a, const double* __restrict__ x,
                                                        const BlockDev* __restrict__ blocks, int n_blocks,
                                                        LmOptionsDev o, IterLog* log, int log_cap, int first,
                                                        int jacobi_scaling) {
  if (threadIdx.x == 0 && a.st->commit_pending) a.st->commit_pending = 0;
  post_eval_body(a, x, blocks, n_blocks, o, log, log_cap, first, jacobi_scaling);
}

__global__ __launch_bounds__(256) void prepare_kernel(SolveArgs a, LmOptionsDev o, int with_post, const double* __restrict__ x,
                                                      const BlockDev* __restrict__ blocks, int n_blocks, IterLog* log, int log_cap,
                                                      int jacobi_scaling) {
  const LmState* st = a.st;
  if (st->terminated) return;
  if (with_post && blockIdx.x == gridDim.x - 1) {
    if (threadIdx.x == 0 && a.st->commit_pending) a.st->commit_pending = 0;
    post_eval_body(a, x, blocks, n_blocks, o, log, log_cap, 0, jacobi_scaling);
    return;
  }
  const size_t n_prep_blocks = gridDim.x - (with_post ? 1 : 0);
  use_current_R(a);
  const int n_s = a.n_s(), W = a.W(), m = a.m, mc = a.mc, m1 = a.m + 1;
  const double radius = st->radius;
  const size_t nL = size_t(a.n_cp) * W * 6, nY = size_t(n_s) * m1, nS = size_t(m1) * m1;
  const size_t total = nL + nY + nS;
  auto hss = [&](int r, int c) { return r >= c ? band_entry(a, r, c) : band_entry(a, c, r); };
  auto band_act = [&](int J) { return a.cp_active[J] != 0 && !a.in_sep(6 * J); };
  for (size_t i = size_t(blockIdx.x) * blockDim.x + threadIdx.x; i < total; i += n_prep_blocks * blockDim.x) {
    if (i < nL) {
      const int J = int(i / (size_t(W) * 6)), rem = int(i % (size_t(W) * 6));
      const int r = rem / 6, cc = rem % 6;
      const int col = 6 * J + cc, row = 6 * J + r;
      const bool act = band_act(J);
      double v = 0.0;
      if (row < n_s) v = hss(row, col);
      if (row == col) {
        if (!act) { v = 1.0; if (!a.in_sep(col)) a.dadd[col] = 0.0; }
        else {
          const double s = a.scale[col];
          const double d = fmin(fmax(v * s * s, o.min_lm_diagonal), o.max_lm_diagonal) / (radius * s * s);
          a.dadd[col] = d; v += d;
        }
      } else if (!act || (row < n_s && !band_act(row / 6))) v = 0.0;
      a.Lb[i] = v;
    } else if (i < nL + nY) {
      const size_t q = i - nL;
      const int c = int(q / m1), j = int(q % m1);
      double v = 0.0;
      if (band_act(c / 6)) {
        if (j < mc) v = a.R[a.off_E() + size_t(c) * mc + j];
        else if (j < m) v = hss(c, 6 * a.sep_s + (j - mc));
        else v = a.R[a.off_g() + c];
      }
      a.Y[q] = v;
    } else {
      const size_t q = i - nL - nY;
      const int r = int(q / m1), cc = int(q % m1);
      double v = 0.0;
      if (r < m && cc < m) {
        if (r < mc && cc < mc) v = a.R[a.off_C() + size_t(r) * mc + cc];
        else if (r >= mc && cc >= mc) v = hss(6 * a.sep_s + (r - mc), 6 * a.sep_s + (cc - mc));
        else {
          const int t = 6 * a.sep_s + ((r >= mc ? r : cc) - mc), j = r >= mc ? cc : r;
          v = a.R[a.off_E() + size_t(t) * mc + j];
        }
        if (r == cc) {
          const int tj = a.border_tangent(r);
          const double s = a.scale[tj];
          const double d = fmin(fmax(v * s * s, o.min_lm_diagonal), o.max_lm_diagonal) / (radius * s * s);
          a.dadd[tj] = d; v += d;
        }
      } else if (r == m && cc < m) v = a.R[a.off_g() + a.border_tangent(cc)];
      else if (r < m && cc == m) v = a.R[a.off_g() + a.border_tangent(r)];
      a.S[q] = v;
    }
  }
}

constexpr int kSlotPad = 16;

DEVI void chol6(const double* A, double L[6][6], double dinv[6], double* dmin) {
  double a[6][6];
#pragma unroll
  for (int i = 0; i < 6; ++i)
#pragma unroll
    for (int k = 0; k <= i; ++k) a[i][k] = A[i * 6 + k];
#pragma unroll
  for (int j = 0; j < 6; ++j) {
    const double d = a[j][j];
    *dmin = fmin(*dmin, d);
    const double inv = rsqrt_nr(d);
    L[j][j] = d * inv; dinv[j] = inv;
#pragma unroll
    for (int i = j + 1; i < 6; ++i) L[i][j] = a[i][j] * inv;
#pragma unroll
    for (int i = j + 1; i < 6; ++i)
#pragma unroll
      for (int k = j + 1; k <= i; ++k) a[i][k] -= L[i][j] * L[k][j];
  }
}

__global__ __launch_bounds__(256) __attribute__((amdgpu_waves_per_eu(2))) void band_cholesky_kernel(SolveArgs a, int bs ) {
  LmState* st = a.st;
  if (st->terminated) return;
  extern __shared__ double lds[];
  const int jb = a.seg_begin(blockIdx.y);
  const int k = a.k, W = 6 * k, ncp = a.seg_end(blockIdx.y) - jb, m1 = a.m + 1;
  if (ncp <= 0) return;
  double* const Lb0 = a.Lb + size_t(jb) * W * 6;
  double* const Y0 = a.Y + size_t(6 * jb) * m1;
  double* const Linv0 = a.Linv + size_t(jb) * 36;
  const int j0 = blockIdx.x * bs;
  const int nb = max(1, min(bs, m1 - j0));
  const int nband = W * 6;
  const int SLP = nband + bs * 6;
  const int ZERO = SLP, DUMP = SLP + 8, LINV = SLP + kSlotPad;
  const int SL = SLP + kSlotPad + 40;
  const int NSL = k + 2;
  const int tid = threadIdx.x, lane = tid & 63, wave = tid >> 6;
  const int lc16 = lane & 15, lk = lane >> 4;
  const int nelem = nband + nb * 6;
  constexpr int NE = 3;
  double* Xbuf = lds + NSL * SL;
  double* Lpiv = Xbuf + 2 * SL;
  double* W3 = Lpiv + 144;
  for (int i = tid; i < (NSL + 2) * SL + 224; i += 256) lds[i] = 0.0;
  int l_off[NE], wb_l[NE];
  bool wb_piv[NE];
  const double* g_base[NE];
  double* wb_base[NE];
  size_t g_stride[NE], wb_stride[NE];
  const int stid = tid >= 64 && tid < 192 ? tid - 64 : 0;
#pragma unroll
  for (int u = 0; u < NE; ++u) {
    const int e = stid + 128 * u;
    auto describe = [&](int ee, int* lo, size_t* goff, size_t* stride, bool* isy) {
      if (ee < nband) { *lo = ee; *goff = size_t(ee); *stride = size_t(nband); *isy = false; }
      else { const int q = ee - nband; const int c = q / nb, j = q % nb; *lo = nband + j * 6 + c; *goff = size_t(c) * m1 + j0 + j; *stride = size_t(6) * m1; *isy = true; }
    };
    size_t goff; bool isy;
    describe(e < nelem ? e : 0, &l_off[u], &goff, &g_stride[u], &isy);
    if (e >= nelem) l_off[u] = DUMP;
    g_base[u] = (isy ? Y0 : Lb0) + goff;
    const int ew = blockIdx.x == 0 ? e % nelem : nband + e % (nb * 6);
    describe(ew, &wb_l[u], &goff, &wb_stride[u], &isy);
    wb_base[u] = (isy ? Y0 : Lb0) + goff;
    wb_piv[u] = ew < 36;
  }
  auto gload = [&](int J, double regs[NE]) {
    const int Jc = J < ncp ? J : ncp - 1;
#pragma unroll
    for (int u = 0; u < NE; ++u) regs[u] = g_base[u][size_t(Jc) * g_stride[u]];
// ... 683 lines not shown
      st->invalid_eval = ev_invalid > 0.0;
      if (st->step_norm <= o.parameter_tolerance * (st->x_norm + o.parameter_tolerance)) {
        st->terminated = 1; st->termination_type = 0; st->termination_reason = 4;
      } else {
        st->cost_change = st->x_cost - candidate_cost;
        if (fabs(st->cost_change) <= o.function_tolerance * st->x_cost) {
          st->terminated = 1; st->termination_type = 0; st->termination_reason = 5;
        } else {
          st->relative_decrease = (candidate_cost >= 1.7976931348623157e308)
                                      ? -1.7976931348623157e308
                                      : (st->x_cost - candidate_cost) / st->model_cost_change;
          if (st->relative_decrease > o.min_relative_decrease) {
            s_accept = 1;
            st->step_successful = 1;
            st->prev_cost_change = st->last_cost_change; st->last_cost_change = st->cost_change;
            st->need_jacobian = 1;
            if (r_stride) { if (no_swap) st->commit_pending = 1; else st->rcur ^= 1; }
            st->x_norm = cand_norm;
            const double t = 2.0 * st->relative_decrease - 1.0;
            st->radius = st->radius / fmax(1.0 / 3.0, 1.0 - t * t * t);
            st->radius = fmin(o.max_radius, st->radius);
            st->decrease_factor = 2.0;
          } else {
            st->radius = st->radius / st->decrease_factor;
            st->decrease_factor *= 2.0;
            log_and_finalize(st, o, log, log_cap);
          }
        }
      }
    }
  }
  __syncthreads();
  {
    constexpr int n_int = int(sizeof(LmState) / sizeof(int));
    for (int i = tid; i < n_int; i += 256) reinterpret_cast<int*>(st_g)[i] = reinterpret_cast<const int*>(st)[i];
  }
  if (s_accept) {
#pragma unroll
    for (int k = 0; k < 4; ++k) if (tid + 256 * k < n_amb) x[tid + 256 * k] = pf.xc[k];
    for (int i = tid + 1024; i < n_amb; i += 256) x[i] = x_cand[i];
  }
  if (st->terminated) {
    __syncthreads();
    publish_results_block(st_g, tid, 256);
    __syncthreads();
    if (tid == 0) st_g->published = 1;
  }
  if (progress && tid == 0) publish_progress(progress, st, seq);
}
__global__ __launch_bounds__(256) void lm_control_kernel(LmState* st, LmOptionsDev o, double* R2, double* x,
                                                         const double* x_cand, int n_amb, IterLog* log, int log_cap,
                                                         const double* __restrict__ item_cost, int n_items,
                                                         const double* Rbase, size_t r_stride, int no_swap, int* progress,
                                                         int seq) {
  __shared__ LmState s_st;
  control_body(st, o, R2, x, x_cand, n_amb, log, log_cap, item_cost, n_items, Rbase, r_stride, no_swap, progress, seq, &s_st);
}

__global__ __launch_bounds__(256) void commit_kernel(const LmState* st, double* R, size_t n) {
  if (!st->commit_pending) return;
  for (size_t i = size_t(blockIdx.x) * 256 + threadIdx.x; i < n; i += size_t(gridDim.x) * 256) R[i] = R[n + i];
}

__global__ __launch_bounds__(256) void debug_control_replay_kernel(LmState* st, LmOptionsDev o, const double* rho, const int* infinite,
                                                                    int n, double* R2, double* radius_out, int* accepted_out,
                                                                    double* cost_out, IterLog* log, int log_cap) {
  __shared__ LmState s_st;
  for (int i = 0; i < n; ++i) {
    if (threadIdx.x == 0) {
      st->terminated = 0; st->x_cost = 1.0; st->x_norm = 1.0; st->chol_failed = 0;
      st->upd_parts = 1; st->upd_mcc[0] = 1.0; st->upd_sn[0] = 1.0; st->upd_cn[0] = 1.0; st->upd_bad[0] = 0;
      R2[0] = 1.0 - rho[i]; R2[1] = infinite[i] ? 1.0 : 0.0;
    }
    __syncthreads();
    control_body(st, o, R2, nullptr, nullptr, 0, log, log_cap, nullptr, 0, nullptr, 0, 0, nullptr, 0, &s_st);
    __syncthreads();
    if (threadIdx.x == 0) {
      radius_out[i] = st->radius; accepted_out[i] = st->step_successful;
      cost_out[i] = st->step_successful ? st->candidate_cost : log[st->n_log - 1].cost;
    }
    __syncthreads();
  }
}
void launch_debug_control_replay(LmState* st, const LmOptionsDev& o, const double* rho, const int* infinite, int n, double* R2,
                                 double* radius_out, int* accepted_out, double* cost_out, IterLog* log, int log_cap, hipStream_t s) {
  hipLaunchKernelGGL(debug_control_replay_kernel, dim3(1), dim3(256), 0, s, st, o, rho, infinite, n, R2, radius_out, accepted_out, cost_out,
                     log, log_cap);
}

__global__ __launch_bounds__(256) void publish_results_kernel(const LmState* st, const IterLog* log, int log_rows, const double* x, int n_amb,
                                                              LmState* h_state, IterLog* h_log, double* h_x) {
  const int tid = threadIdx.x;
  const int n_state = int(sizeof(LmState) / sizeof(int)), n_row = int(sizeof(IterLog) / sizeof(int));
  const int rows = min(max(st->n_log, 0), log_rows);
  for (int i = tid; i < n_state; i += 256) reinterpret_cast<int*>(h_state)[i] = reinterpret_cast<const int*>(st)[i];
  for (int i = tid; i < rows * n_row; i += 256) reinterpret_cast<int*>(h_log)[i] = reinterpret_cast<const int*>(log)[i];
  for (int i = tid; i < n_amb; i += 256) h_x[i] = x[i];
}
void launch_publish_results(const LmState* st, const IterLog* log, int log_rows, const double* x, int n_amb, LmState* h_state,
                            IterLog* h_log, double* h_x, hipStream_t s) {
  hipLaunchKernelGGL(publish_results_kernel, dim3(1), dim3(256), 0, s, st, log, log_rows, x, n_amb, h_state, h_log, h_x);
}
__global__ __launch_bounds__(256) void seed_x_kernel(double* x, const double* h_x, int n_amb) {
  for (int i = threadIdx.x + blockIdx.x * 256; i < n_amb; i += 256 * gridDim.x) x[i] = h_x[i];
}
void launch_seed_x(double* x, const double* h_x, int n_amb, hipStream_t s) {
  hipLaunchKernelGGL(seed_x_kernel, dim3(4), dim3(256), 0, s, x, h_x, n_amb);
}

__global__ __launch_bounds__(256) void begin_solve_kernel(LmState* st, double radius, double x_norm, const double* upd_ext, int upd_ext_n,
                                                          ResultSink sink, double* x, double* x_cand, const double* h_x, int n_amb) {
  for (int i = threadIdx.x + blockIdx.x * 256; i < n_amb; i += 256 * gridDim.x) {
    const double v = h_x[i];
    x[i] = v;
    if (x_cand) x_cand[i] = v;
  }
  if (blockIdx.x == 0 && threadIdx.x == 0) {
    LmState s = {};
    s.upd_ext = upd_ext; s.upd_ext_n = upd_ext_n; s.upd_parts = 1;
    s.radius = radius; s.decrease_factor = 2.0; s.x_norm = x_norm; s.need_jacobian = 1; s.rfill = 1;
    s.min_cost = 1.7976931348623157e308;
    s.sink = sink;
    *st = s;
  }
}
void launch_begin_solve(LmState* st, double radius, double x_norm, const double* upd_ext, int upd_ext_n, const ResultSink& sink, double* x,
                        double* x_cand, const double* h_x, int n_amb, hipStream_t s) {
  hipLaunchKernelGGL(begin_solve_kernel, dim3(4), dim3(256), 0, s, st, radius, x_norm, upd_ext, upd_ext_n, sink, x, x_cand, h_x, n_amb);
}

__global__ void init_state_kernel(LmState* st, double radius, double x_norm, const double* upd_ext, int upd_ext_n) {
  LmState s = {};
  s.upd_ext = upd_ext; s.upd_ext_n = upd_ext_n; s.upd_parts = 1;
  s.radius = radius; s.decrease_factor = 2.0; s.x_norm = x_norm; s.need_jacobian = 1; s.rfill = 1;
  s.min_cost = 1.7976931348623157e308;
  *st = s;
}

void launch_gather(double* R, const double* src, const int* out_idx_thin, const int64_t* ptr_thin, const int* idx_thin,
                   int n_thin, int n_thin8, int n_thin4, int thin_per_lane, const int* out_idx_fat, const int64_t* ptr_fat, const int* idx_fat, int n_fat,
                   const double* cost_src, int n_cost,
                   const LmState* st, int need_flag, size_t other_stride, hipStream_t s, const ControlTail* tail) {
  const int nb_fat = (n_fat + 3) / 4;
  const int nb8 = (n_thin8 + 31) / 32, nb4 = (n_thin4 - n_thin8 + 63) / 64, nb1 = (n_thin - n_thin4 + 255) / 256;
  const int n_blocks = ((1 + nb_fat + 7) & ~7) + ((nb8 + 7) & ~7) + ((nb4 + 7) & ~7) + ((nb1 + 7) & ~7);
  ControlTail t;
  if (tail) t = *tail; else { t = ControlTail(); t.enabled = 0; }
#define LAUNCH_GATHER(UU, FX) hipLaunchKernelGGL((gather_kernel<UU, FX>), dim3(n_blocks), dim3(256), 0, s, R, src, out_idx_thin, ptr_thin, idx_thin, n_thin, n_thin8, n_thin4, \
                       out_idx_fat, ptr_fat, idx_fat, n_fat, nb_fat, cost_src, n_cost, st, need_flag, other_stride, t)
  if (thin_per_lane <= 6) { if (ptr_thin) LAUNCH_GATHER(6, false); else LAUNCH_GATHER(6, true); }
  else { if (ptr_thin) LAUNCH_GATHER(12, false); else LAUNCH_GATHER(12, true); }
#undef LAUNCH_GATHER
}
__global__ __launch_bounds__(256) void gather_pack_fixed_kernel(const int64_t* __restrict__ ptr, const int* __restrict__ idx, int n_thin, int n_thin8,
                                                               int n_thin4, int s8, int zero_slot, int* __restrict__ out) {
  const int o = int(blockIdx.x) * 256 + int(threadIdx.x);
  if (o >= n_thin) return;
  const size_t base4 = size_t(n_thin8) * s8, base1 = base4 + size_t(n_thin4 - n_thin8) * 24;
  const int stride = o < n_thin8 ? s8 : (o < n_thin4 ? 24 : 8);
  const size_t base = o < n_thin8 ? size_t(o) * s8 : (o < n_thin4 ? base4 + size_t(o - n_thin8) * 24 : base1 + size_t(o - n_thin4) * 8);
  const int64_t q0 = ptr[o], q1 = ptr[o + 1];
  for (int k = 0; k < stride; ++k) out[base + k] = q0 + k < q1 ? idx[q0 + k] : zero_slot;
}
size_t gather_fixed_entries(int n_thin, int n_thin8, int n_thin4, int thin_per_lane) {
  return size_t(n_thin8) * (8 * thin_per_lane) + size_t(n_thin4 - n_thin8) * 24 + size_t(n_thin - n_thin4) * 8;
}
void launch_gather_pack_fixed(const int64_t* ptr, const int* idx, int n_thin, int n_thin8, int n_thin4, int thin_per_lane, int zero_slot, int* out,
                              hipStream_t s) {
  if (n_thin <= 0) return;
  hipLaunchKernelGGL(gather_pack_fixed_kernel, dim3((n_thin + 255) / 256), dim3(256), 0, s, ptr, idx, n_thin, n_thin8, n_thin4, 8 * thin_per_lane, zero_slot, out);
}
void launch_post_eval(const SolveArgs& a, const double* x, const BlockDev* blocks, int n_blocks, const LmOptionsDev& o,
                      IterLog* log, int log_cap, int first, int jacobi, hipStream_t s) {
  hipLaunchKernelGGL(post_eval_kernel, dim3(1), dim3(256), 0, s, a, x, blocks, n_blocks, o, log, log_cap, first, jacobi);
}
constexpr int kBorderSlice = 16;
size_t band_cholesky_lds_bytes(const SolveArgs& a) {
  return (size_t(a.k + 4) * (a.W() * 6 + kBorderSlice * 6 + 16 + 40) + 224) * sizeof(double);
}
size_t reduced_solve_lds_bytes(const SolveArgs& a) {
  const int m1 = a.m + 1;
  return (size_t(m1) * (m1 | 1) + m1) * sizeof(double);
}
size_t band_backsolve_lds_bytes(const SolveArgs&) { return 0; }
hipError_t configure_solve_kernels(size_t band_lds, size_t reduced_lds, size_t back_lds) {
  hipError_t e = hipFuncSetAttribute(reinterpret_cast<const void*>(&band_cholesky_kernel),
                                     hipFuncAttributeMaxDynamicSharedMemorySize, int(band_lds));
  if (e != hipSuccess) return e;
  if (reduced_lds) {
    e = hipFuncSetAttribute(reinterpret_cast<const void*>(&reduced_solve_kernel),
                            hipFuncAttributeMaxDynamicSharedMemorySize, int(reduced_lds));
    if (e != hipSuccess) return e;
  }
  (void)hipFuncSetAttribute(reinterpret_cast<const void*>(&reduced_solve_panel_kernel<1>), hipFuncAttributeMaxDynamicSharedMemorySize, 150 * 1024);
  for (const void* f : {reinterpret_cast<const void*>(&band_backsolve_kernel<2>), reinterpret_cast<const void*>(&band_backsolve_kernel<3>),
                        reinterpret_cast<const void*>(&band_backsolve_kernel<4>), reinterpret_cast<const void*>(&band_backsolve_kernel<5>),
                        reinterpret_cast<const void*>(&band_backsolve_kernel<6>), reinterpret_cast<const void*>(&band_backsolve_kernel<7>),
                        reinterpret_cast<const void*>(&band_backsolve_kernel<8>)}) {
    e = hipFuncSetAttribute(f, hipFuncAttributeMaxDynamicSharedMemorySize, int(back_lds));
    if (e != hipSuccess) return e;
  }
  return hipSuccess;
}
static bool reduced_is_blocked(const SolveArgs& a) { return a.m + 1 > 128 && a.m <= kBlockedMaxM; }
int reduced_schur_slices(const SolveArgs& a) {
  if (!(a.m + 1 <= 128 || reduced_is_blocked(a))) return 1;
  if (a.m + 1 <= 128) {
    if (a.n_cp >= 1280) return 8;
    if (a.n_cp >= 640) return 4;
    if (a.n_cp < 160) return 1;
  }
  if (a.n_cp < 320) return 1;
  return kSchurSlices;
}
void launch_dense_block_solve(const SolveArgs& a, int ks, hipStream_t s, int t0 = 0, int outer_back = 0);
void launch_reduced_block_step(const SolveArgs& a, int j, int nsl, int n_wg, hipStream_t s);
void launch_reduced_solve(const SolveArgs& a, bool reduced_in_lds, int ks, hipStream_t s) {
  const int m1 = a.m + 1;
  if (m1 <= 128 && a.m >= 1) {
    launch_dense_block_solve(a, ks, s);
  } else if (m1 <= 128) {
    const size_t lds = (size_t(m1) * ((16 * ((m1 + 15) / 16)) | 1) + m1 + 32 + 128 + 256) * sizeof(double);
    hipLaunchKernelGGL(reduced_solve_panel_kernel<1>, dim3(1), dim3(256), lds, s, a, 0, ks);
  } else if (reduced_is_blocked(a)) {
    const int steps = (m1 - 128 + kRB - 1) / kRB, t0 = kRB * steps;
    for (int j = 0; j < steps; ++j) {
      const int rows = m1 - kRB * (j + 1), T = rows > 0 ? (rows + 63) / 64 : 0;
      launch_reduced_block_step(a, j, j == 0 ? ks : 1, T > 0 ? T * (T + 1) / 2 : 1, s);
    }
    launch_dense_block_solve(a, 1, s, t0, 1);
  } else {
    hipLaunchKernelGGL(reduced_solve_kernel, dim3(1), dim3(256), reduced_in_lds ? reduced_solve_lds_bytes(a) : 0, s, a,
                       reduced_in_lds ? 1 : 0);
  }
}
void launch_band_reduction(const SolveArgs& a, const LmOptionsDev& o, const double* x, const BlockDev* blocks, int n_blocks, hipStream_t s,
                           bool with_post_eval, IterLog* log, int log_cap, int jacobi) {
  const int m1 = a.m + 1;
  const size_t total = size_t(a.n_cp) * a.W() * 6 + size_t(a.n_s()) * m1 + size_t(m1) * m1;
  const int pb = int((total + 255) / 256);
  hipLaunchKernelGGL(prepare_kernel, dim3((pb < 2048 ? pb : 2048) + (with_post_eval ? 1 : 0)), dim3(256), 0, s, a, o, with_post_eval ? 1 : 0,
                     x, blocks, n_blocks, log, log_cap, jacobi);
  const int nwg = (m1 + kBorderSlice - 1) / kBorderSlice;
  hipLaunchKernelGGL(band_cholesky_kernel, dim3(nwg, a.n_seg()), dim3(256), band_cholesky_lds_bytes(a), s, a, kBorderSlice);
  const int nt = (m1 + 15) / 16;
  const int ks = reduced_schur_slices(a);
  hipLaunchKernelGGL(schur_kernel, dim3(nt * (nt + 1) / 2 * ks), dim3(256), 0, s, a, ks);
}
void launch_solve(const SolveArgs& a, const LmOptionsDev& o, const double* x, double* x_cand, const BlockDev* blocks,
                  int n_blocks, bool reduced_in_lds, hipStream_t s, bool with_post_eval, IterLog* log, int log_cap, int jacobi) {
  launch_band_reduction(a, o, x, blocks, n_blocks, s, with_post_eval, log, log_cap, jacobi);
  const int ks = reduced_schur_slices(a);
  launch_reduced_solve(a, reduced_in_lds, ks, s);
  hipLaunchKernelGGL(border_matvec_kernel, dim3((a.n_s() + 3) / 4), dim3(256), 0, s, a);
  {
    const size_t bl = band_backsolve_lds_bytes(a);
    switch (a.k) {
      case 2: hipLaunchKernelGGL(band_backsolve_kernel<2>, dim3(a.n_seg()), dim3(256), bl, s, a, x, x_cand, blocks, n_blocks); break;
      case 3: hipLaunchKernelGGL(band_backsolve_kernel<3>, dim3(a.n_seg()), dim3(256), bl, s, a, x, x_cand, blocks, n_blocks); break;
      case 4: hipLaunchKernelGGL(band_backsolve_kernel<4>, dim3(a.n_seg()), dim3(256), bl, s, a, x, x_cand, blocks, n_blocks); break;
      case 5: hipLaunchKernelGGL(band_backsolve_kernel<5>, dim3(a.n_seg()), dim3(256), bl, s, a, x, x_cand, blocks, n_blocks); break;
      case 6: hipLaunchKernelGGL(band_backsolve_kernel<6>, dim3(a.n_seg()), dim3(256), bl, s, a, x, x_cand, blocks, n_blocks); break;
      case 7: hipLaunchKernelGGL(band_backsolve_kernel<7>, dim3(a.n_seg()), dim3(256), bl, s, a, x, x_cand, blocks, n_blocks); break;
      default: hipLaunchKernelGGL(band_backsolve_kernel<8>, dim3(a.n_seg()), dim3(256), bl, s, a, x, x_cand, blocks, n_blocks); break;
    }
  }
}
void launch_cost_reduce(const double* item_cost, int n_items, double* R2, const LmState* st, hipStream_t s) {
  hipLaunchKernelGGL(cost_reduce_kernel, dim3(1), dim3(256), 0, s, item_cost, n_items, R2, st);
}
void launch_control(LmState* st, const LmOptionsDev& o, double* R2, double* x, const double* x_cand, int n_amb,
                    IterLog* log, int log_cap, const double* item_cost, int n_items, const double* Rbase, size_t r_stride,
                    hipStream_t s, bool commit_by_copy) {
  hipLaunchKernelGGL(lm_control_kernel, dim3(1), dim3(256), 0, s, st, o, R2, x, x_cand, n_amb, log, log_cap, item_cost, n_items,
                     Rbase, r_stride, commit_by_copy ? 1 : 0, nullptr, 0);
  if (commit_by_copy && r_stride)
    hipLaunchKernelGGL(commit_kernel, dim3(unsigned(std::min<size_t>(512, (r_stride + 255) / 256))), dim3(256), 0, s, st,
                       const_cast<double*>(Rbase), r_stride);
}
void launch_init_state(LmState* st, double radius, double x_norm, hipStream_t s, const double* upd_ext, int upd_ext_n) {
  hipLaunchKernelGGL(init_state_kernel, dim3(1), dim3(1), 0, s, st, radius, x_norm, upd_ext, upd_ext_n);
}

}
```

Baseline: 10270.

## Compute gather source indices on the fly from structured tables instead of index lists

Adds a structured gather kernel that derives each output's source partial offsets from compact per-layout/segment tables staged in LDS, replacing the precomputed per-output index lists and packed fixed-index arrays. It is meant to cut the global-memory traffic of reading large index arrays in the per-iteration normal-equation gather. It also adds ownership and full-segment tables for fast paths. The cost is extra integer arithmetic per lane, LDS usage, and more complex index logic. The old list path stays available behind an environment flag.

```diff
diff --git a/calico_amd/_capi.py b/calico_amd/_capi.py
--- a/calico_amd/_capi.py
+++ b/calico_amd/_capi.py
@@ -423,10 +423,10 @@
         self._check(self.api.problem_finalize(self.h))
 
     def plan_info(self):
-        out = np.zeros(9, np.int32)
-        self._check(self.api.debug_plan_info(self.h, out.ctypes.data_as(C.POINTER(C.c_int32)), 9))
+        out = np.zeros(10, np.int32)
+        self._check(self.api.debug_plan_info(self.h, out.ctypes.data_as(C.POINTER(C.c_int32)), 10))
         keys = ("fuse_expand", "frames", "items", "cells", "max_frames_per_cell", "max_items_per_cell", "tree_solver", "m",
-                "all_control_points_observed")
+                "all_control_points_observed", "gather_structured")
         return dict(zip(keys, (int(v) for v in out)))
 
     def comm_init_rccl(self, unique_id, rank, world_size):
diff --git a/calico_amd/csrc/calico_hip.cpp b/calico_amd/csrc/calico_hip.cpp
--- a/calico_amd/csrc/calico_hip.cpp
+++ b/calico_amd/csrc/calico_hip.cpp
@@ -45,6 +45,10 @@
 void launch_gather_lists(const GatherStruct& gs, int n_out, int* cnt, int* out_idx, int64_t* ptr, int* idx, int zero_slot, long long* scratch,
                          hipStream_t s);
 size_t gather_fixed_entries(int n_thin, int n_thin8, int n_thin4, int thin_per_lane);
+bool gather_struct_fits(const GatherStruct& gs);
+void launch_gather_struct(double* R, const double* src, const GatherStruct& gs, int thin_per_lane, const int* out_idx_fat, const int64_t* ptr_fat,
+                          const int* idx_fat, int n_fat, const double* cost_src, int n_cost, const LmState* st, int need_flag,
+                          size_t other_stride, hipStream_t s, const ControlTail* tail);
 void launch_gather_pack_fixed(const int64_t* ptr, const int* idx, int n_thin, int n_thin8, int n_thin4, int thin_per_lane, int zero_slot, int* out,
                               hipStream_t s);
 void launch_post_eval(const SolveArgs& a, const double* x, const BlockDev* blocks, int n_blocks, const LmOptionsDev& o,
@@ -385,6 +389,8 @@
   bool dense_in_lds = true;
   int gather_owner_block = 0;
   bool gs_lists_on_device = false;
+  bool gather_structured = false;
+  GatherStruct gs_struct = {};
 };
 struct PlanDev {
   DevBuf<double> d_knots, d_basis, d_stamp;
@@ -534,6 +540,7 @@
   bool band_split = env_flag("CALICO_BAND_SPLIT", true);
   bool fuse_expand = env_flag("CALICO_FUSE_EXPAND", true);
   bool gather_struct = env_flag("CALICO_GATHER_STRUCT", true);
+  bool gather_lists = env_flag("CALICO_GATHER_LISTS", false);
   int bcr_leaf = env_int("CALICO_BCR_LEAF", 0, 1, kBcrMaxChain);
 };
 
@@ -1098,12 +1105,25 @@
   GatherStruct gsd = {};
   if (gs_ok) {
     const int n_lay = int(layouts.size()), nsg = int(p->valid_knots.size()) - 1;
-    gs_tab.assign(size_t(n_lay) * nsg + size_t(n_lay) * m + size_t(n_lay), -1);
+    gs_tab.assign(size_t(n_lay) * nsg + size_t(n_lay) * m + size_t(n_lay) + size_t(m) + size_t(nsg), -1);
     for (const CellDev& c : p->h_cells) gs_tab[size_t(c.layout) * nsg + size_t(c.seg)] = int(c.partial_off);
     for (int l = 0; l < n_lay; ++l) {
       const std::vector<int>& gmap = layout_gmap[size_t(l)];
       for (size_t q = 0; q < gmap.size(); ++q) gs_tab[size_t(n_lay) * nsg + size_t(l) * m + size_t(gmap[q] - NS)] = 6 * k + int(q);
       gs_tab[size_t(n_lay) * nsg + size_t(n_lay) * m + size_t(l)] = layouts[size_t(l)].ncols + 1;
+    }
+    for (int tc = 0; tc < m; ++tc) {
+      int own = -1, holders = 0;
+      for (int l = 0; l < n_lay; ++l) {
+        const int jc = gs_tab[size_t(n_lay) * nsg + size_t(l) * m + size_t(tc)];
+        if (jc >= 0) { ++holders; own = (l << 16) | jc; }
+      }
+      gs_tab[size_t(n_lay) * (nsg + m + 1) + size_t(tc)] = holders == 1 ? own : -1;
+    }
+    for (int sg = 0; sg < nsg; ++sg) {
+      int full = 1;
+      for (int l = 0; l < n_lay; ++l) full &= gs_tab[size_t(l) * nsg + size_t(sg)] >= 0 ? 1 : 0;
+      gs_tab[size_t(n_lay) * (nsg + m + 1) + size_t(m) + size_t(sg)] = full;
     }
     gsd.n_lay = n_lay; gsd.nseg = nsg; gsd.n_cp = n_cp; gsd.k = k; gsd.m = m;
     {
@@ -1211,15 +1231,10 @@
   DevBuf<long long> d_scan;
   if (comp_base + comp_off + row_store + 2 >= size_t(0x7fffffff)) return p->set_error(CALICO_UNIMPLEMENTED, "problem too large for 32-bit gather indices");
   const int zero_slot = int(comp_base + comp_off + row_store);
+  p->gather_structured = false;
   if (gs_ok) {
     HIP_TRY(p, p->d_gs_tab.upload(gs_tab, s));
     gsd.tab = p->d_gs_tab.p;
-    const int per_out = int(layouts.size()) * k;
-    HIP_TRY(p, p->d_out_thin.alloc(size_t(gs_n_out))); HIP_TRY(p, p->d_ptr_thin.alloc(size_t(gs_n_out) + 1));
-    HIP_TRY(p, p->d_idx_thin.alloc(size_t(gs_n_out) * per_out)); HIP_TRY(p, d_cnt.alloc(size_t(gs_n_out)));
-    HIP_TRY(p, d_scan.alloc(size_t(gs_n_out) / 1024 + 2));
-    launch_gather_lists(gsd, int(gs_n_out), d_cnt.p, p->d_out_thin.p, p->d_ptr_thin.p, p->d_idx_thin.p, zero_slot, d_scan.p, s);
-    p->n_thin = int(gs_n_out);
     bool one_layout = k <= 8;
     for (int tc = 0; one_layout && tc < m; ++tc) {
       int holders = 0;
@@ -1227,16 +1242,36 @@
       one_layout = holders <= 1;
     }
     const int n_border0 = NS + n_cp * k * 36;
-    p->n_thin4 = one_layout ? n_border0 : p->n_thin;
-    const int d4 = gsd.d_split;
-    p->n_thin8 = one_layout ? std::min(n_border0, NS + d4 * n_cp * 36) : p->n_thin;
+    gsd.cls_far = one_layout ? 4 : 8; gsd.cls_border = one_layout ? 1 : 8;
+    gsd.zero_slot = zero_slot;
+    gsd.win = 0;
+    for (int pb = 0, n_wg = struct_workgroups(gsd); pb < n_wg; ++pb) {
+      int o0, o1, base, len;
+      if (struct_workgroup(gsd, pb, o0, o1) < 0) continue;
+      struct_window(gsd, o0, o1, base, len);
+      gsd.win = std::max(gsd.win, len);
+    }
+    p->gather_structured = !sw.gather_lists && gather_struct_fits(gsd);
+    p->gs_struct = gsd;
+    if (p->gather_structured) {
+      p->n_thin = p->n_thin8 = p->n_thin4 = 0;
+    } else {
+      const int per_out = int(layouts.size()) * k;
+      HIP_TRY(p, p->d_out_thin.alloc(size_t(gs_n_out))); HIP_TRY(p, p->d_ptr_thin.alloc(size_t(gs_n_out) + 1));
+      HIP_TRY(p, p->d_idx_thin.alloc(size_t(gs_n_out) * per_out)); HIP_TRY(p, d_cnt.alloc(size_t(gs_n_out)));
+      HIP_TRY(p, d_scan.alloc(size_t(gs_n_out) / 1024 + 2));
+      launch_gather_lists(gsd, int(gs_n_out), d_cnt.p, p->d_out_thin.p, p->d_ptr_thin.p, p->d_idx_thin.p, zero_slot, d_scan.p, s);
+      p->n_thin = int(gs_n_out);
+      p->n_thin4 = one_layout ? n_border0 : p->n_thin;
+      p->n_thin8 = one_layout ? std::min(n_border0, NS + gsd.d_split * n_cp * 36) : p->n_thin;
+    }
   } else {
     HIP_TRY(p, p->d_out_thin.upload(out_thin, s)); HIP_TRY(p, p->d_idx_thin.upload(idx_thin, s));
     HIP_TRY(p, p->d_ptr_thin.upload(ptr_thin, s));
   }
   HIP_TRY(p, p->d_out_fat.upload(out_fat, s)); HIP_TRY(p, p->d_idx_fat.upload(idx_fat, s));
   HIP_TRY(p, p->d_ptr_fat.upload(ptr_fat, s));
-  p->gather_fixed = p->n_thin > 0 && gs_ok;
+  p->gather_fixed = p->n_thin > 0 && gs_ok && !p->gather_structured;
   if (p->gather_fixed) {
     HIP_TRY(p, p->d_idx_fixed.alloc(gather_fixed_entries(p->n_thin, p->n_thin8, p->n_thin4, p->thin_per_lane) + 8));
     launch_gather_pack_fixed(p->d_ptr_thin.p, p->d_idx_thin.p, p->n_thin, p->n_thin8, p->n_thin4, p->thin_per_lane, zero_slot, p->d_idx_fixed.p, s);
@@ -1340,7 +1375,7 @@
     n_obs += s.stamps.size();
   }
   h.word(uint64_t(sw.band_solver) | (uint64_t(sw.speculative) << 1) | (uint64_t(sw.band_split) << 2) | (uint64_t(sw.fuse_expand) << 3) |
-         (uint64_t(sw.gather_struct) << 4) | (uint64_t(sw.bcr_leaf) << 8));
+         (uint64_t(sw.gather_struct) << 4) | (uint64_t(sw.gather_lists) << 5) | (uint64_t(sw.bcr_leaf) << 8));
   PlanKey k; k.h1 = h.a; k.h2 = h.b; k.n_blocks = p->blocks.size(); k.n_obs = n_obs; k.device = p->device;
   return k;
 }
@@ -1654,9 +1689,16 @@
     HIP_TRY(p, hipMemsetAsync(target, 0, p->r_size * sizeof(double), p->stream));
   }
   if (!p->fuse_expand) launch_expand_cells(ea, p->stream);
-  launch_gather(p->d_R.p, p->d_partials.p, p->d_out_thin.p, p->gather_fixed ? nullptr : p->d_ptr_thin.p, p->gather_fixed ? p->d_idx_fixed.p : p->d_idx_thin.p, p->n_thin, p->n_thin8, p->n_thin4, p->thin_per_lane, p->d_out_fat.p,
-                p->d_ptr_fat.p, p->d_idx_fat.p, p->n_fat, p->d_partials.p + p->partial_doubles, p->n_fitems + p->n_jac_items, st, need_flag,
-                spec ? p->r_size : 0, p->stream, tail);
+  if (p->gather_structured) {
+    GatherStruct gs = p->gs_struct;
+    gs.tab = p->d_gs_tab.p;
+    launch_gather_struct(p->d_R.p, p->d_partials.p, gs, p->thin_per_lane, p->d_out_fat.p, p->d_ptr_fat.p, p->d_idx_fat.p, p->n_fat,
+                         p->d_partials.p + p->partial_doubles, p->n_fitems + p->n_jac_items, st, need_flag, spec ? p->r_size : 0, p->stream, tail);
+  } else {
+    launch_gather(p->d_R.p, p->d_partials.p, p->d_out_thin.p, p->gather_fixed ? nullptr : p->d_ptr_thin.p, p->gather_fixed ? p->d_idx_fixed.p : p->d_idx_thin.p, p->n_thin, p->n_thin8, p->n_thin4, p->thin_per_lane, p->d_out_fat.p,
+                  p->d_ptr_fat.p, p->d_idx_fat.p, p->n_fat, p->d_partials.p + p->partial_doubles, p->n_fitems + p->n_jac_items, st, need_flag,
+                  spec ? p->r_size : 0, p->stream, tail);
+  }
   p->timer.end(p->stream);
   if (!p->has_exchange()) return CALICO_OK;
   return do_allreduce(p, target, int64_t(p->r_size));
@@ -2334,8 +2376,36 @@
   return CALICO_OK;
 }
 
+int32_t calico_debug_gather_struct(const int32_t* dims, const int32_t* tab, int32_t o, int32_t* list_out, int32_t* n_list,
+                                   int32_t* slots_out) {
+  if (!dims || !tab || !list_out || !n_list || !slots_out) return CALICO_INVALID_ARGUMENT;
+  cal::GatherStruct gs = {};
+  gs.tab = tab; gs.n_lay = dims[0]; gs.nseg = dims[1]; gs.n_cp = dims[2]; gs.k = dims[3]; gs.m = dims[4]; gs.d_split = dims[5];
+  gs.cls_far = dims[6]; gs.cls_border = dims[7]; gs.zero_slot = dims[8];
+  if (gs.n_lay < 1 || gs.nseg < 1 || gs.n_cp < 1 || gs.k < 1 || gs.k > 8 || gs.m < 1 || gs.n_lay * gs.k > 96 || gs.d_split < 0 || gs.d_split > gs.k)
+    return CALICO_INVALID_ARGUMENT;
+  int begin[5], cls[4];
+  cal::struct_ranges(gs, begin, cls);
+  if (o < 0 || o >= begin[4]) return CALICO_INVALID_ARGUMENT;
+  gs.off_g = 0; gs.off_B = 0; gs.off_E = 0;
+  const cal::StructOut q = cal::struct_output(gs, o);
+  const cal::GsView t = cal::gs_view(gs);
+  int n = 0;
+  cal::struct_sources(gs, t, q, [&](int si) { if (n < 96) list_out[n] = si; ++n; });
+  *n_list = n;
+  const int r = o < begin[1] ? 0 : (o < begin[2] ? 1 : (o < begin[3] ? 2 : 3)), c = cls[r];
+  const int* full = tab + gs.n_lay * (gs.nseg + gs.m + 1) + gs.m;
+  const int own = r == 3 && c == 1 ? tab[gs.n_lay * (gs.nseg + gs.m + 1) + q.tc] : -2;
+  for (int sub = 0; sub < c; ++sub) {
+    int scratch[12], fid[12];
+    cal::struct_lane_slots<12>(gs, t, full, own, q, c, sub, scratch, 1, fid);
+    for (int u = 0; u < 12; ++u) slots_out[sub * 12 + u] = fid[u];
+  }
+  return c;
+}
+
 int32_t calico_debug_plan_info(calico_problem* p, int32_t* out, int32_t n) {
-  if (!p || !out || n < 0 || n > 9) return CALICO_INVALID_ARGUMENT;
+  if (!p || !out || n < 0 || n > 10) return CALICO_INVALID_ARGUMENT;
   int rc = finalize(p);
   if (rc != CALICO_OK) return rc;
   int max_frames = 0, max_items = 0, run = 0, prev_layout = -1, prev_seg = -1;
@@ -2345,8 +2415,8 @@
     prev_layout = it.layout; prev_seg = it.seg;
     max_items = std::max(max_items, run);
   }
-  const int v[9] = {p->fuse_expand ? 1 : 0, p->n_fitems, p->n_jac_items, int(p->h_cells.size()), max_frames, max_items,
-                    p->use_bcr ? 1 : 0, p->m, p->bcr_all_active ? 1 : 0};
+  const int v[10] = {p->fuse_expand ? 1 : 0, p->n_fitems, p->n_jac_items, int(p->h_cells.size()), max_frames, max_items,
+                     p->use_bcr ? 1 : 0, p->m, p->bcr_all_active ? 1 : 0, p->gather_structured ? 1 : 0};
   for (int i = 0; i < n; ++i) out[i] = v[i];
   return CALICO_OK;
 }
diff --git a/calico_amd/csrc/calico_hip_testing.h b/calico_amd/csrc/calico_hip_testing.h
--- a/calico_amd/csrc/calico_hip_testing.h
+++ b/calico_amd/csrc/calico_hip_testing.h
@@ -15,6 +15,9 @@
 
 int32_t calico_debug_roll_table(int32_t spline_order, int32_t lane, uint32_t* out48);
 
+int32_t calico_debug_gather_struct(const int32_t* dims, const int32_t* tab, int32_t o, int32_t* list_out, int32_t* n_list,
+                                   int32_t* slots_out);
+
 #ifdef __cplusplus
 }
 #endif
diff --git a/calico_amd/csrc/problem_dev.hpp b/calico_amd/csrc/problem_dev.hpp
--- a/calico_amd/csrc/problem_dev.hpp
+++ b/calico_amd/csrc/problem_dev.hpp
@@ -164,6 +164,9 @@
   int n_lay, nseg, n_cp, k, m;
   int d_split;
   unsigned long long off_g, off_B, off_E;
+  int cls_far, cls_border;
+  int win;
+  int zero_slot;
 };
 
 struct ControlTail {
@@ -185,6 +188,146 @@
 #endif
 CAL_HD inline int tri_off(int i, int j, int n1) { return i * n1 - ((i * (i - 1)) >> 1) + (j - i); }
 CAL_HD inline int tri_size(int n1) { return (n1 * (n1 + 1)) >> 1; }
+
+struct StructOut { int a, b, r, c, tc, rhs; size_t dst; };
+CAL_HD inline StructOut struct_output(const GatherStruct& gs, int o) {
+  const int NS = 6 * gs.n_cp, n_b = gs.n_cp * gs.k * 36;
+  StructOut q;
+  q.tc = -1; q.rhs = 0; q.c = 0;
+  if (o < NS) {
+    const int ti = o;
+    q.a = q.b = ti / 6; q.r = ti % 6; q.rhs = 1;
+    q.dst = size_t(gs.off_g) + size_t(ti);
+  } else if (o < NS + n_b) {
+    const int e = o - NS, ds = gs.d_split, n_a = gs.n_cp * ds * 36;
+    int bd, d;
+    if (e < n_a) { bd = e / 36; q.a = bd / ds; d = bd - q.a * ds; }
+    else { const int dr = gs.k - ds; bd = (e - n_a) / 36; q.a = bd / dr; d = ds + (bd - q.a * dr); }
+    const int w = e - 36 * (e / 36);
+    q.b = q.a + d;
+    q.r = w / 6; q.c = w % 6;
+    q.dst = size_t(gs.off_B) + size_t(q.a * gs.k + d) * 36 + size_t(w);
+  } else {
+    const int e = o - NS - n_b, ti = e / gs.m;
+    q.tc = e - ti * gs.m;
+    q.a = q.b = ti / 6; q.r = ti % 6;
+    q.dst = size_t(gs.off_E) + size_t(e);
+  }
+  return q;
+}
+struct GsView { const int* poff; int ps, pb; const int* inv; const int* n1s; };
+CAL_HD inline GsView gs_view(const GatherStruct& gs) {
+  const int* inv = gs.tab + gs.n_lay * gs.nseg;
+  return GsView{gs.tab, gs.nseg, 0, inv, inv + gs.n_lay * gs.m};
+}
+template <class F>
+CAL_HD inline int struct_sources(const GatherStruct& gs, const GsView& t, const StructOut& q, F f) {
+  const int n_lay = gs.n_lay, nseg = gs.nseg, m = gs.m, k = gs.k;
+  if (q.b >= gs.n_cp) return 0;
+  const int lo = q.b - (k - 1) > 0 ? q.b - (k - 1) : 0, hi = q.a < nseg - 1 ? q.a : nseg - 1;
+  int n = 0;
+  for (int l = 0; l < n_lay; ++l) {
+    const int n1 = t.n1s[l];
+    const int jc = q.tc >= 0 ? t.inv[l * m + q.tc] : 0;
+    if (jc < 0) continue;
+    for (int s0 = lo; s0 <= hi; s0 += 8) {
+      int po[8];
+#pragma unroll
+      for (int u = 0; u < 8; ++u) po[u] = s0 + u <= hi ? t.poff[l * t.ps + (s0 + u - t.pb)] : -1;
+#pragma unroll
+      for (int u = 0; u < 8; ++u) {
+        if (po[u] < 0) continue;
+        const int sg = s0 + u;
+        int i = 6 * (q.a - sg) + q.r, j;
+        if (q.tc >= 0) j = jc;
+        else if (q.rhs) j = n1 - 1;
+        else { j = 6 * (q.b - sg) + q.c; if (q.a == q.b && i > j) { const int tt = i; i = j; j = tt; } }
+        f(po[u] + tri_off(i, j, n1));
+        ++n;
+      }
+    }
+  }
+  return n;
+}
+template <class P>
+CAL_HD inline void struct_lane_sources(const GatherStruct& gs, const GsView& t, const StructOut& q, int cls, int sub, P put) {
+  const int lg = cls == 8 ? 3 : (cls == 4 ? 2 : 0);
+  int n = 0;
+  struct_sources(gs, t, q, [&](int s) { if ((n & (cls - 1)) == sub) put(n >> lg, s); ++n; });
+}
+template <int SL>
+CAL_HD inline void struct_lane_slots(const GatherStruct& gs, const GsView& t, const int* full, int own, const StructOut& q, int cls,
+                                     int sub, int* slots, int stride, int* fid) {
+  const int k = gs.k, lo = q.b - (k - 1) > 0 ? q.b - (k - 1) : 0, hi = q.a < gs.nseg - 1 ? q.a : gs.nseg - 1;
+  const bool live = q.b < gs.n_cp && k <= 8;
+  if (own >= -1) {
+    const int l = own >= 0 ? own >> 16 : 0, jc = own & 0xffff, n1 = t.n1s[l];
+#pragma unroll
+    for (int u = 0; u < SL; ++u) {
+      const int sg = lo + u;
+      const int po = own >= 0 && live && u < 8 && sg <= hi ? t.poff[l * t.ps + (sg - t.pb)] : -1;
+      fid[u] = po >= 0 ? po + tri_off(6 * (q.a - sg) + q.r, jc, n1) : gs.zero_slot;
+    }
+    return;
+  }
+  bool direct = q.tc < 0 && live;
+#pragma unroll
+  for (int u = 0; u < 8; ++u) if (lo + u <= hi) direct = direct && full[lo + u - t.pb] != 0;
+  if (direct) {
+    const int len_o = hi - lo + 1, n_src = gs.n_lay * len_o;
+#pragma unroll
+    for (int u = 0; u < SL; ++u) {
+      const int n = sub + cls * u;
+      fid[u] = gs.zero_slot;
+      if (n < n_src) {
+        const int l = n / len_o, sg = lo + (n - l * len_o), n1 = t.n1s[l];
+        int i = 6 * (q.a - sg) + q.r, j;
+        if (q.rhs) j = n1 - 1;
+        else { j = 6 * (q.b - sg) + q.c; if (q.a == q.b && i > j) { const int tt = i; i = j; j = tt; } }
+        fid[u] = t.poff[l * t.ps + (sg - t.pb)] + tri_off(i, j, n1);
+      }
+    }
+    return;
+  }
+#pragma unroll
+  for (int u = 0; u < SL; ++u) slots[u * stride] = gs.zero_slot;
+  struct_lane_sources(gs, t, q, cls, sub, [&](int slot, int si) { if (slot < SL) slots[slot * stride] = si; });
+#pragma unroll
+  for (int u = 0; u < SL; ++u) fid[u] = slots[u * stride];
+}
+CAL_HD inline void struct_ranges(const GatherStruct& gs, int* begin, int* cls) {
+  const int NS = 6 * gs.n_cp;
+  begin[0] = 0; begin[1] = NS; begin[2] = NS + gs.n_cp * gs.d_split * 36; begin[3] = NS + gs.n_cp * gs.k * 36; begin[4] = begin[3] + NS * gs.m;
+  cls[0] = 8; cls[1] = 8; cls[2] = gs.cls_far; cls[3] = gs.cls_border;
+}
+CAL_HD inline int struct_workgroup(const GatherStruct& gs, int pb, int& o0, int& o1) {
+  int begin[5], cls[4];
+  struct_ranges(gs, begin, cls);
+  for (int r = 0; r < 4; ++r) {
+    const int per = 256 / cls[r], n = begin[r + 1] - begin[r], nb = (n + per - 1) / per, nbp = (nb + 7) & ~7;
+    if (pb < nbp) {
+      const int j = (pb & 7) * ((nb + 7) >> 3) + (pb >> 3);
+      if (j >= nb) return -1;
+      o0 = begin[r] + j * per;
+      o1 = o0 + per < begin[r + 1] ? o0 + per : begin[r + 1];
+      return r;
+    }
+    pb -= nbp;
+  }
+  return -1;
+}
+CAL_HD inline int struct_workgroups(const GatherStruct& gs) {
+  int begin[5], cls[4], n = 0;
+  struct_ranges(gs, begin, cls);
+  for (int r = 0; r < 4; ++r) { const int per = 256 / cls[r]; n += (((begin[r + 1] - begin[r] + per - 1) / per) + 7) & ~7; }
+  return n;
+}
+CAL_HD inline void struct_window(const GatherStruct& gs, int o0, int o1, int& base, int& len) {
+  const int a0 = struct_output(gs, o0).a, a1 = struct_output(gs, o1 - 1).a;
+  base = a0 - (gs.k - 1) > 0 ? a0 - (gs.k - 1) : 0;
+  const int end = a1 < gs.nseg - 1 ? a1 : gs.nseg - 1;
+  len = end >= base ? end - base + 1 : 0;
+}
 
 struct SolveArgs {
   const double* R;
diff --git a/calico_amd/csrc/solve_kernels.hip b/calico_amd/csrc/solve_kernels.hip
--- a/calico_amd/csrc/solve_kernels.hip
+++ b/calico_amd/csrc/solve_kernels.hip
@@ -13,63 +13,11 @@
                        int log_cap, const double* __restrict__ item_cost, int n_items, const double* Rbase, size_t r_stride,
                        int no_swap, int* progress, int seq, LmState* s_st, const ControlStage* staged = nullptr);
 DEVI void publish(int* word, int value);
-struct StructOut { int a, b, r, c, tc, rhs; size_t dst; };
-DEVI StructOut struct_output(const GatherStruct& gs, int o) {
-  const int NS = 6 * gs.n_cp, n_e = NS * gs.m, n_b = gs.n_cp * gs.k * 36;
-  StructOut q;
-  q.tc = -1; q.rhs = 0; q.c = 0;
-  if (o < NS) {
-    const int ti = o;
-    q.a = q.b = ti / 6; q.r = ti % 6; q.rhs = 1;
-    q.dst = size_t(gs.off_g) + size_t(ti);
-  } else if (o < NS + n_b) {
-    const int e = o - NS, ds = gs.d_split, n_a = gs.n_cp * ds * 36;
-    int bd, d;
-    if (e < n_a) { bd = e / 36; q.a = bd / ds; d = bd - q.a * ds; }
-    else { const int dr = gs.k - ds; bd = (e - n_a) / 36; q.a = bd / dr; d = ds + (bd - q.a * dr); }
-    const int w = e - 36 * (e / 36);
-    q.b = q.a + d;
-    q.r = w / 6; q.c = w % 6;
-    q.dst = size_t(gs.off_B) + size_t(q.a * gs.k + d) * 36 + size_t(w);
-  } else {
-    const int e = o - NS - n_b, ti = e / gs.m;
-    q.tc = e - ti * gs.m;
-    q.a = q.b = ti / 6; q.r = ti % 6;
-    q.dst = size_t(gs.off_E) + size_t(e);
-  }
-  return q;
-}
-template <class F>
-DEVI int struct_sources(const GatherStruct& gs, const StructOut& q, F f) {
-  const int n_lay = gs.n_lay, nseg = gs.nseg, m = gs.m, k = gs.k;
-  const int* poff = gs.tab;
-  const int* inv = gs.tab + n_lay * nseg;
-  const int* n1s = inv + n_lay * m;
-  if (q.b >= gs.n_cp) return 0;
-  const int lo = max(0, q.b - (k - 1)), hi = min(q.a, nseg - 1);
-  int n = 0;
-  for (int l = 0; l < n_lay; ++l) {
-    const int n1 = n1s[l];
-    const int jc = q.tc >= 0 ? inv[l * m + q.tc] : 0;
-    if (jc < 0) continue;
-    for (int sg = lo; sg <= hi; ++sg) {
-      const int po = poff[l * nseg + sg];
-      if (po < 0) continue;
-      int i = 6 * (q.a - sg) + q.r, j;
-      if (q.tc >= 0) j = jc;
-      else if (q.rhs) j = n1 - 1;
-      else { j = 6 * (q.b - sg) + q.c; if (q.a == q.b && i > j) { const int t = i; i = j; j = t; } }
-      f(po + tri_off(i, j, n1));
-      ++n;
-    }
-  }
-  return n;
-}
 __global__ __launch_bounds__(256) void gather_lists_count_kernel(GatherStruct gs, int n_out, int* __restrict__ cnt, int* __restrict__ out_idx) {
   const int o = blockIdx.x * 256 + threadIdx.x;
   if (o >= n_out) return;
   const StructOut q = struct_output(gs, o);
-  const int n = struct_sources(gs, q, [](int) {});
+  const int n = struct_sources(gs, gs_view(gs), q, [](int) {});
   cnt[o] = n > 0 ? n : 1;
   out_idx[o] = int(q.dst);
 }
@@ -134,7 +82,7 @@
   if (o >= n_out) return;
   const StructOut q = struct_output(gs, o);
   int64_t w = ptr[o];
-  const int n = struct_sources(gs, q, [&](int srci) { idx[w++] = srci; });
+  const int n = struct_sources(gs, gs_view(gs), q, [&](int srci) { idx[w++] = srci; });
   if (n == 0) idx[w] = zero_slot;
 }
 void launch_gather_lists(const GatherStruct& gs, int n_out, int* cnt, int* out_idx, int64_t* ptr, int* idx, int zero_slot, long long* scratch,
@@ -145,6 +93,103 @@
   hipLaunchKernelGGL(gather_lists_scan_sums_kernel, dim3(1), dim3(1024), 0, s, scratch, nb, ptr + n_out);
   hipLaunchKernelGGL(gather_lists_block_scan_kernel, dim3(nb), dim3(256), 0, s, cnt, n_out, scratch, ptr);
   hipLaunchKernelGGL(gather_lists_fill_kernel, dim3((n_out + 255) / 256), dim3(256), 0, s, gs, n_out, ptr, idx, zero_slot);
+}
+
+DEVI bool gather_head(double* __restrict__& R, const double* __restrict__ src, const int* __restrict__ out_fat, const int64_t* __restrict__ ptr_fat,
+                      const int* __restrict__ idx_fat, int n_fat, int nb_fat, const double* __restrict__ cost_src, int n_cost,
+                      const LmState* st, size_t other_stride, const ControlTail& tail) {
+  __shared__ LmState s_st;
+  __shared__ double s_c01[2];
+  ControlStage pf;
+  const bool owner = blockIdx.x == 0;
+  if (owner && tail.enabled) { control_prefetch(st, tail.x_cand, tail.n_amb, &s_st, pf); pf.c01 = s_c01; }
+  if (other_stride && st && st->rfill) R += other_stride;
+  if (owner) {
+    const int tid = threadIdx.x;
+    double c = 0.0, v = 0.0;
+    for (int i = tid; i < n_cost; i += 256 * 4) {
+      double cc[4], vv[4];
+#pragma unroll
+      for (int u = 0; u < 4; ++u) { const int j = min(i + 256 * u, n_cost - 1); cc[u] = cost_src[2 * j]; vv[u] = cost_src[2 * j + 1]; }
+#pragma unroll
+      for (int u = 0; u < 4; ++u) if (i + 256 * u < n_cost) { c += cc[u]; v += vv[u]; }
+    }
+    c = wave_sum(c); v = wave_sum(v);
+    __shared__ double s_w[2][4];
+    if ((tid & 63) == 0) { s_w[0][tid >> 6] = c; s_w[1][tid >> 6] = v; }
+    __syncthreads();
+    if (tid == 0) {
+      const double ct = ((s_w[0][0] + s_w[0][1]) + s_w[0][2]) + s_w[0][3], vt = ((s_w[1][0] + s_w[1][1]) + s_w[1][2]) + s_w[1][3];
+      R[0] = ct; R[1] = vt; s_c01[0] = ct; s_c01[1] = vt;
+    }
+    if (tail.enabled) {
+      __syncthreads();
+      control_body(const_cast<LmState*>(st), tail.o, nullptr, tail.x, tail.x_cand, tail.n_amb, tail.log, tail.log_cap, nullptr, 0,
+                   tail.Rbase, tail.r_stride, 0, tail.progress, tail.seq, &s_st, &pf);
+    }
+    return true;
+  }
+  const int bid = int(blockIdx.x) - 1;
+  if (bid >= nb_fat) return false;
+  {
+    const int wave_raw = (bid * blockDim.x + threadIdx.x) >> 6;
+    const int lane = threadIdx.x & 63;
+    const bool live = wave_raw < n_fat;
+    const int wave = live ? wave_raw : n_fat - 1;
+    const int64_t q0 = ptr_fat[wave], q1 = ptr_fat[wave + 1];
+    double s = 0.0;
+    for (int64_t qb = q0; qb < q1; qb += 256) {
+      int id[4];
+#pragma unroll
+      for (int u = 0; u < 4; ++u) { const int64_t q = qb + lane + 64 * u; id[u] = idx_fat[q < q1 ? q : q1 - 1]; }
+      double v[4];
+#pragma unroll
+      for (int u = 0; u < 4; ++u) v[u] = src[id[u]];
+#pragma unroll
+      for (int u = 0; u < 4; ++u) s += qb + lane + 64 * u < q1 ? v[u] : 0.0;
+    }
+    s = wave_sum(s);
+    if (live && lane == 0) R[out_fat[wave]] = s;
+  }
+  return true;
+}
+
+template <int U>
+DEVI void gather_fixed_sum(double* __restrict__ R, const double* __restrict__ src, const int* fid, int cls, bool live, int dst) {
+  if (cls == 1) {
+    double v[8];
+#pragma unroll
+    for (int u = 0; u < 8; ++u) v[u] = src[fid[u]];
+    double s = 0.0;
+#pragma unroll
+    for (int u = 0; u < 8; ++u) s += v[u];
+    if (live) R[dst] = s;
+    return;
+  }
+  if (cls == 4) {
+    const int sub = int(threadIdx.x) & 3;
+    double v[6];
+#pragma unroll
+    for (int u = 0; u < 6; ++u) v[u] = src[fid[u]];
+    double s = 0.0;
+#pragma unroll
+    for (int u = 0; u < 6; ++u) s += v[u];
+    s = row4_sum(s);
+    if (live && sub == 0) R[dst] = s;
+    return;
+  }
+  const int sub = int(threadIdx.x) & 7;
+  double v[U];
+#pragma unroll
+  for (int u = 0; u < U; ++u) v[u] = src[fid[u]];
+  double s = 0.0, s2 = 0.0;
+#pragma unroll
+  for (int u = 0; u < 6; ++u) s += v[u];
+#pragma unroll
+  for (int u = 6; u < U; ++u) s2 += v[u];
+  s += s2;
+  s = row8_sum(s);
+  if (live && sub == 0) R[dst] = s;
 }
 
 template <int U, bool FIXED>
@@ -208,95 +253,11 @@
     return;
   }
   if (idle) return;
-  __shared__ LmState s_st;
-  __shared__ double s_c01[2];
-  ControlStage pf;
-  const bool owner = blockIdx.x == 0;
-  if (owner && tail.enabled) { control_prefetch(st, tail.x_cand, tail.n_amb, &s_st, pf); pf.c01 = s_c01; }
-  if (other_stride && st && st->rfill) R += other_stride;
-  if (owner) {
-    const int tid = threadIdx.x;
-    double c = 0.0, v = 0.0;
-    for (int i = tid; i < n_cost; i += 256 * 4) {
-      double cc[4], vv[4];
-#pragma unroll
-      for (int u = 0; u < 4; ++u) { const int j = min(i + 256 * u, n_cost - 1); cc[u] = cost_src[2 * j]; vv[u] = cost_src[2 * j + 1]; }
-#pragma unroll
-      for (int u = 0; u < 4; ++u) if (i + 256 * u < n_cost) { c += cc[u]; v += vv[u]; }
-    }
-    c = wave_sum(c); v = wave_sum(v);
-    __shared__ double s_w[2][4];
-    if ((tid & 63) == 0) { s_w[0][tid >> 6] = c; s_w[1][tid >> 6] = v; }
-    __syncthreads();
-    if (tid == 0) {
-      const double ct = ((s_w[0][0] + s_w[0][1]) + s_w[0][2]) + s_w[0][3], vt = ((s_w[1][0] + s_w[1][1]) + s_w[1][2]) + s_w[1][3];
-      R[0] = ct; R[1] = vt; s_c01[0] = ct; s_c01[1] = vt;
-    }
-    if (tail.enabled) {
-      __syncthreads();
-      control_body(const_cast<LmState*>(st), tail.o, nullptr, tail.x, tail.x_cand, tail.n_amb, tail.log, tail.log_cap, nullptr, 0,
-                   tail.Rbase, tail.r_stride, 0, tail.progress, tail.seq, &s_st, &pf);
-    }
-    return;
-  }
-  const int bid = int(blockIdx.x) - 1;
-  if (bid < nb_fat) {
-    const int wave_raw = (bid * blockDim.x + threadIdx.x) >> 6;
-    const int lane = threadIdx.x & 63;
-    const bool live = wave_raw < n_fat;
-    const int wave = live ? wave_raw : n_fat - 1;
-    const int64_t q0 = ptr_fat[wave], q1 = ptr_fat[wave + 1];
-    double s = 0.0;
-    for (int64_t qb = q0; qb < q1; qb += 256) {
-      int id[4];
-#pragma unroll
-      for (int u = 0; u < 4; ++u) { const int64_t q = qb + lane + 64 * u; id[u] = idx_fat[q < q1 ? q : q1 - 1]; }
-      double v[4];
-#pragma unroll
-      for (int u = 0; u < 4; ++u) v[u] = src[id[u]];
-#pragma unroll
-      for (int u = 0; u < 4; ++u) s += qb + lane + 64 * u < q1 ? v[u] : 0.0;
-    }
-    s = wave_sum(s);
-    if (live && lane == 0) R[out_fat[wave]] = s;
-  } else {
+  if (gather_head(R, src, out_fat, ptr_fat, idx_fat, n_fat, nb_fat, cost_src, n_cost, st, other_stride, tail)) return;
+  {
     if (FIXED) {
-      if (cls == 1) {
-        const int o = o_thin;
-        const int dst = out_thin[o < n_thin ? o : n_thin - 1];
-        double v[8];
-#pragma unroll
-        for (int u = 0; u < 8; ++u) v[u] = src[fid[u]];
-        double s = 0.0;
-#pragma unroll
-        for (int u = 0; u < 8; ++u) s += v[u];
-        if (o < n_thin) R[dst] = s;
-        return;
-      }
-      if (cls == 4) {
-        const int o = o_thin, sub = int(threadIdx.x) & 3;
-        double v[6];
-#pragma unroll
-        for (int u = 0; u < 6; ++u) v[u] = src[fid[u]];
-        double s = 0.0;
-#pragma unroll
-        for (int u = 0; u < 6; ++u) s += v[u];
-        s = row4_sum(s);
-        if (o < n_thin4 && sub == 0) R[out_thin[o]] = s;
-        return;
-      }
-      const int o = o_thin, sub = int(threadIdx.x) & 7;
-      double v[U];
-#pragma unroll
-      for (int u = 0; u < U; ++u) v[u] = src[fid[u]];
-      double s = 0.0, s2 = 0.0;
-#pragma unroll
-      for (int u = 0; u < 6; ++u) s += v[u];
-#pragma unroll
-      for (int u = 6; u < U; ++u) s2 += v[u];
-      s += s2;
-      s = row8_sum(s);
-      if (o < n_thin8 && sub == 0) R[out_thin[o]] = s;
+      const int o = o_thin, n_cls = cls == 1 ? n_thin : (cls == 4 ? n_thin4 : n_thin8);
+      gather_fixed_sum<U>(R, src, fid, cls, o < n_cls, out_thin[o < n_cls ? o : n_cls - 1]);
       return;
     }
     if (cls == 1) {
@@ -360,6 +321,80 @@
     s = row8_sum(s);
     if (live && sub == 0) R[out_thin[o]] = s;
   }
+}
+
+constexpr int kGsSlots(int U) { return U > 8 ? U : 8; }
+constexpr int kGsStageCells = 8, kGsStageCols = 16;
+template <int U>
+__global__ __launch_bounds__(256) void gather_struct_kernel(double* __restrict__ R, const double* __restrict__ src, GatherStruct gs,
+                                                            const int* __restrict__ out_fat, const int64_t* __restrict__ ptr_fat,
+                                                            const int* __restrict__ idx_fat, int n_fat, int nb_fat,
+                                                            const double* __restrict__ cost_src, int n_cost,
+                                                            const LmState* st, int need_flag, size_t other_stride, ControlTail tail) {
+  constexpr int SL = kGsSlots(U);
+  extern __shared__ int s_gs[];
+  const int tid = int(threadIdx.x), n_lay = gs.n_lay, m = gs.m;
+  int rg = -1, o0 = 0, o1 = 0, base = 0, len = 0;
+  bool idle = false;
+  if (int(blockIdx.x) - 1 >= nb_fat) {
+    const int pb = int(blockIdx.x) - ((1 + nb_fat + 7) & ~7);
+    rg = pb < 0 ? -1 : struct_workgroup(gs, pb, o0, o1);
+    idle = rg < 0;
+  }
+  int cw[kGsStageCells], iw[kGsStageCols], nw = 0, own = -1, fw = 0;
+  const int* inv_g = gs.tab + n_lay * gs.nseg;
+  const bool one_lane = rg == 3 && gs.cls_border == 1;
+  if (rg >= 0) {
+    struct_window(gs, o0, o1, base, len);
+    const int n_c = n_lay * len;
+#pragma unroll
+    for (int u = 0; u < kGsStageCells; ++u) {
+      const int t = tid + 256 * u, l = t < n_c ? t / len : 0;
+      cw[u] = t < n_c ? gs.tab[l * gs.nseg + base + (t - l * len)] : 0;
+    }
+    if (one_lane) {
+      const int oc = o0 + tid < o1 ? o0 + tid : o1 - 1;
+      own = gs.tab[n_lay * (gs.nseg + m + 1) + struct_output(gs, oc).tc];
+    } else if (rg == 3) {
+#pragma unroll
+      for (int u = 0; u < kGsStageCols; ++u) { const int t = tid + 256 * u; iw[u] = t < n_lay * m ? inv_g[t] : 0; }
+    }
+    nw = tid < n_lay ? inv_g[n_lay * m + tid] : 0;
+    fw = tid < len ? gs.tab[n_lay * (gs.nseg + m + 1) + m + base + tid] : 0;
+  }
+  if (st && (st->terminated || (need_flag && !st->need_jacobian))) {
+    if (tail.enabled && tail.progress && st->terminated && blockIdx.x == 0 && threadIdx.x == 0) publish_progress(tail.progress, st, tail.seq);
+    return;
+  }
+  if (idle) return;
+  if (gather_head(R, src, out_fat, ptr_fat, idx_fat, n_fat, nb_fat, cost_src, n_cost, st, other_stride, tail)) return;
+  int* s_slot = s_gs;
+  int* s_n1 = s_slot + SL * 256;
+  int* s_cell = s_n1 + n_lay;
+  int* s_col = s_cell + n_lay * gs.win;
+  int* s_full = s_col + n_lay * m;
+  {
+    const int n_c = n_lay * len;
+#pragma unroll
+    for (int u = 0; u < kGsStageCells; ++u) { const int t = tid + 256 * u; if (t < n_c) s_cell[t] = cw[u]; }
+    if (rg == 3 && !one_lane) {
+#pragma unroll
+      for (int u = 0; u < kGsStageCols; ++u) { const int t = tid + 256 * u; if (t < n_lay * m) s_col[t] = iw[u]; }
+    }
+    if (tid < n_lay) s_n1[tid] = nw;
+    if (tid < len) s_full[tid] = fw;
+  }
+  __syncthreads();
+  int begin[5], clss[4];
+  struct_ranges(gs, begin, clss);
+  const int cls = clss[rg], lg = cls == 8 ? 3 : (cls == 4 ? 2 : 0);
+  const int o = o0 + (tid >> lg), sub = tid & (cls - 1);
+  const bool live = o < o1;
+  const StructOut q = struct_output(gs, live ? o : o1 - 1);
+  const GsView view{s_cell, len, base, s_col, s_n1};
+  int fid[SL];
+  struct_lane_slots<SL>(gs, view, s_full, one_lane ? own : -2, q, cls, sub, s_slot + tid, 256, fid);
+  gather_fixed_sum<U>(R, src, fid, cls, live, int(q.dst));
 }
 
 __global__ __launch_bounds__(256) void post_eval_kernel(SolveArgs a, const double* __restrict__ x,
@@ -1349,6 +1384,27 @@
   else { if (ptr_thin) LAUNCH_GATHER(12, false); else LAUNCH_GATHER(12, true); }
 #undef LAUNCH_GATHER
 }
+size_t gather_struct_lds_bytes(const GatherStruct& gs, int thin_per_lane) {
+  return sizeof(int) * (size_t(kGsSlots(thin_per_lane <= 6 ? 6 : 12)) * 256 + size_t(gs.n_lay) * (1 + gs.win + gs.m) + size_t(gs.win));
+}
+bool gather_struct_fits(const GatherStruct& gs) {
+  return gs.n_lay * gs.win <= 256 * kGsStageCells && gs.n_lay * gs.m <= 256 * kGsStageCols && gs.n_lay <= 256;
+}
+void launch_gather_struct(double* R, const double* src, const GatherStruct& gs, int thin_per_lane, const int* out_idx_fat, const int64_t* ptr_fat,
+                          const int* idx_fat, int n_fat, const double* cost_src, int n_cost, const LmState* st, int need_flag,
+                          size_t other_stride, hipStream_t s, const ControlTail* tail) {
+  const int nb_fat = (n_fat + 3) / 4;
+  const int n_blocks = ((1 + nb_fat + 7) & ~7) + struct_workgroups(gs);
+  const size_t lds = gather_struct_lds_bytes(gs, thin_per_lane);
+  ControlTail t;
+  if (tail) t = *tail; else { t = ControlTail(); t.enabled = 0; }
+  if (thin_per_lane <= 6)
+    hipLaunchKernelGGL((gather_struct_kernel<6>), dim3(n_blocks), dim3(256), lds, s, R, src, gs, out_idx_fat, ptr_fat, idx_fat, n_fat, nb_fat,
+                       cost_src, n_cost, st, need_flag, other_stride, t);
+  else
+    hipLaunchKernelGGL((gather_struct_kernel<12>), dim3(n_blocks), dim3(256), lds, s, R, src, gs, out_idx_fat, ptr_fat, idx_fat, n_fat, nb_fat,
+                       cost_src, n_cost, st, need_flag, other_stride, t);
+}
 __global__ __launch_bounds__(256) void gather_pack_fixed_kernel(const int64_t* __restrict__ ptr, const int* __restrict__ idx, int n_thin, int n_thin8,
                                                                int n_thin4, int s8, int zero_slot, int* __restrict__ out) {
   const int o = int(blockIdx.x) * 256 + int(threadIdx.x);
```

After: 10280, median of 4. About the same (+0.1%).
